# AI-Application-and-Integration-Lab/RDPN6D

Hardware: AMD Instinct MI355X
Metric: RGB-D crops/sec (fwd+PnP) at 256x256 (higher is better)
Workload: dtype f32

## Files before the change

include/rdpn6d.h:

```cpp
#ifndef RDPN6D_H
#define RDPN6D_H

#ifdef __cplusplus
extern "C" {
#endif

#define RDPN6D_OK 0
#define RDPN6D_EINVAL -1
#define RDPN6D_EHIP -2
#define RDPN6D_ENOMEM -3

const char* rdpn6d_last_error(void);
int rdpn6d_version(void);
int rdpn6d_device_count(void);

void farthest_point_sampling(float* pts, int* idxs, int pn, int sn);
void farthest_point_sampling_init_center(float* pts, int* idxs, int pn, int sn);
int rdpn6d_fps_host(const float* pts, int* idxs, int pn, int sn, int start);
int rdpn6d_fps_device(const float* d_pts, const int* d_offsets, int nobj, int max_pn, int sn, int start,
                      int* d_idxs, float* d_mindist, void* stream);
long long rdpn6d_fps_workspace_bytes(int nobj);
int rdpn6d_fps_device_ws(const float* d_pts, const int* d_offsets, int nobj, int max_pn, int sn, int start, int* d_idxs,
                         float* d_mindist, void* workspace, long long workspace_bytes, void* stream);

typedef struct {
    const float* x;
    const float* w;
    const float* scale;
    const float* shift;
    const float* res;
    float* y;
    int B, H, W;
    int Cin;
    int in_cs, in_co;
    int Ho, Wo;
    int stride;
    int ntaps;
    int dy[9], dx[9];
    int N, Npad;
    int OH, OW;
    int osy, osx, ooy, oox;
    int out_cs, out_co;
    int res_cs, res_co;
    int act;
    float slope;
} rdpn6d_conv_desc;
int rdpn6d_conv2d_f32(const rdpn6d_conv_desc* d, void* stream);
long long rdpn6d_conv_splitk_ws_floats(const rdpn6d_conv_desc* d, int ksplit);
int rdpn6d_conv2d_splitk_f32(const rdpn6d_conv_desc* d, int ksplit, float* workspace, void* stream);
int rdpn6d_conv_tile_for(const rdpn6d_conv_desc* d, int* bm, int* bn);
void rdpn6d_conv_force_tile(int bm, int bn);
void rdpn6d_conv_set_tap_inner(int v);

int rdpn6d_conv2d_bf16(const rdpn6d_conv_desc* d, int out_f32, void* stream);
int rdpn6d_conv2d_splitk_bf16(const rdpn6d_conv_desc* d, int out_f32, int ksplit, float* workspace, void* stream);
int rdpn6d_conv2d_bf16_bnstats(const rdpn6d_conv_desc* d, double* stats, int stats_row0, int* stats_rows, void* stream);
int rdpn6d_conv2d_bf16_bnbwd(const rdpn6d_conv_desc* d, const void* bn_x, int bn_cs, int bn_co, const float* mean, const float* invstd,
                             const float* gamma, const float* beta, double* partial, int* rows, void* stream);
int rdpn6d_bn_relu_backward_apply_bf16(const void* x, int xcs, int xco, const void* dy, int dcs, int dco, const float* mean,
                                       const float* invstd, const float* gamma, const float* beta, float* dgamma, float* dbeta, void* dx,
                                       int xgcs, int xgco, long long M, int C, const double* partial, int S, void* stream);
int rdpn6d_conv2d_bf16_bnbwd_y(const rdpn6d_conv_desc* d, const void* bn_x, int bn_cs, int bn_co, const void* bn_y, int y_cs, int y_co,
                               const float* mean, const float* invstd, double* partial, int* rows, void* stream);
int rdpn6d_bn_backward_apply_bf16(const void* x, int xcs, int xco, const void* dy, int dcs, int dco, const void* y, int ycs, int yco,
                                  const float* mean, const float* invstd, const float* gamma, float* dgamma, float* dbeta, void* dx,
                                  int xgcs, int xgco, void* dres, int rcs, int rco, long long M, int C, const double* partial, int S,
                                  void* stream);
void rdpn6d_conv_bf16_force_tile(int bm, int bn);
void rdpn6d_conv_bf16_force_stages(int nst);
int rdpn6d_conv_bf16_tile_for(const rdpn6d_conv_desc* d, int* bm, int* bn);
int rdpn6d_conv_bf16_uses_pingpong(const rdpn6d_conv_desc* d, int out_f32);
int rdpn6d_split_bf16x3(const float* x, long long n, void* planes, long long plane_elems, void* stream);
int rdpn6d_conv_bf16x3_eligible(const rdpn6d_conv_desc* d);
int rdpn6d_conv_bf16x3_kernel_for(const rdpn6d_conv_desc* d);
int rdpn6d_conv2d_bf16x3(const rdpn6d_conv_desc* d, long long x_plane_elems, long long w_plane_elems, void* y_planes,
                         long long y_plane_elems, void* stream);
int rdpn6d_conv2d_bf16x3_ex(const rdpn6d_conv_desc* d, long long x_plane_elems, long long w_plane_elems, void* y_planes,
                            long long y_plane_elems, const void* res_planes, long long res_plane_elems, void* stream);
int rdpn6d_split_h2(const float* x, int src_cs, int src_co, int C, void* dst, long long npix, int* overflow_flag, void* stream);
int rdpn6d_conv_h2_kernel_for(const rdpn6d_conv_desc* d);
int rdpn6d_conv2d_h2(const rdpn6d_conv_desc* d, void* y_h2, const void* res_h2, int* overflow_flag, void* stream);
int rdpn6d_conv2d_h2_cb(const rdpn6d_conv_desc* d, void* y_h2, const void* res_h2, int* overflow_flag, const float* crop_bias,
                        void* stream);
long long rdpn6d_conv_h2_workspace_bytes(const rdpn6d_conv_desc* d);
void rdpn6d_conv_h2_set_clock_probe(unsigned long long* buf);
void rdpn6d_conv_h2_set_wfrag(int mode);
int rdpn6d_conv_h2_colmax_ok(const rdpn6d_conv_desc* d, int rows_per_group);
int rdpn6d_conv2d_h2_colmax(const rdpn6d_conv_desc* d, unsigned long long* keys, int rows_per_group, int* overflow_flag, void* stream);
int rdpn6d_h2_colmax_decode(unsigned long long* keys, int groups, int N, int Npad, void* out_h2, void* stream);
int rdpn6d_conv_h2_wfrag_wanted(const rdpn6d_conv_desc* d);
int rdpn6d_h2_weight_frag(const void* w_h2, int Npad, int ntaps, int cchunks, void* w_frag, void* stream);
int rdpn6d_conv2d_h2_wf(const rdpn6d_conv_desc* d, void* y_h2, const void* res_h2, int* overflow_flag, const void* w_frag, void* stream);
int rdpn6d_conv2d_h2_ws(const rdpn6d_conv_desc* d, void* y_h2, const void* res_h2, int* overflow_flag, const float* crop_bias,
                        void* workspace, long long workspace_bytes, void* stream);
int rdpn6d_conv_h2_fuse1x1_ok(const rdpn6d_conv_desc* d);
int rdpn6d_conv2d_h2_fuse1x1(const rdpn6d_conv_desc* d, const void* res_h2, int* overflow_flag, const float* crop_bias,
                             const void* w1_h2, const float* scale1, const float* bias1, float* out, int out_cs, int n_out,
                             void* stream);
int rdpn6d_upsample_bilinear_h2(const void* x, int B, int H, int W, int C, int factor, void* y, int* overflow_flag, void* stream);
int rdpn6d_upsample_bilinear_h2_ex(const void* x, int B, int H, int W, int C, int factor, void* y, int out_cs, int out_co, int relu,
                                   int* overflow_flag, void* stream);
int rdpn6d_xyz_subsample_h2(const float* x, int B, int xc, int R, int step, void* y, int out_cs, int out_co, int* overflow_flag,
                            void* stream);
int rdpn6d_global_max_concat_h2(void* buf, int B, int HW, int C, int cs, void* stream);
int rdpn6d_global_max_h2(const void* x_h2, int B, int HW, int C, int cs, void* gmax_h2, void* stream);
int rdpn6d_convt3x3s2_const_bias_f32(const float* V, const float* scale, int B, int F, float* out , void* stream);
int rdpn6d_stem_pool_h2(const float* x, int B, int xc, int R, const void* w_h2, const float* scale, const float* shift, void* y,
                        int* overflow_flag, void* stream);
int rdpn6d_stem_pool_h2_ex(const float* x, int B, int xc, int R, const void* w_h2, const float* scale, const float* shift, void* y,
                           int out_fmt, int* overflow_flag, void* stream);
int rdpn6d_stem_pack_h2(const float* w_oihw, void* w_h2, float* inv_scale, void* stream);
void rdpn6d_conv_bf16_force_chunk(int row_bytes);
int rdpn6d_stem_conv7x7_bf16(const float* x, int B, int xc, int R, const float* w, const float* scale,
                             const float* shift, void* y, void* stream);
int rdpn6d_maxpool3x3s2_bf16(const void* x, int B, int H, int W, int C, void* y, void* stream);
int rdpn6d_upsample_bilinear_bf16(const void* x, int B, int H, int W, int C, int factor, void* y, void* stream);
int rdpn6d_xyz_subsample_bf16(const float* x, int B, int xc, int R, int step, void* y, int out_cs, int out_co,
                              void* stream);
int rdpn6d_global_max_concat_bf16(void* buf, int B, int HW, int C, int cs, void* stream);
int rdpn6d_cast_f32_bf16(const float* src, int src_cs, int src_co, int C, void* dst, int dst_cs, long long npix,
                         void* stream);

int rdpn6d_stem_conv7x7_f32(const float* x, int B, int xc, int R, const float* w, const float* scale,
                            const float* shift, float* y, void* stream);
int rdpn6d_maxpool3x3s2_f32(const float* x, int B, int H, int W, int C, float* y, void* stream);
int rdpn6d_upsample_bilinear_f32(const float* x, int B, int H, int W, int C, int factor, float* y, void* stream);
int rdpn6d_xyz_subsample_f32(const float* x, int B, int xc, int R, int step, float* y, int out_cs, int out_co,
                             void* stream);
int rdpn6d_global_max_concat_f32(float* buf, int B, int HW, int C, int cs, void* stream);
int rdpn6d_groupnorm_relu_f32(float* x, int B, int HW, int C, int G, const float* gamma, const float* beta,
                              void* stream);
int rdpn6d_groupnorm_relu_h2(const float* x, int B, int HW, int C, int G, const float* gamma, const float* beta, void* y_h2,
                             int* overflow_flag, void* stream);

int rdpn6d_dense_glue_f32(const float* head, int head_cs, const float* coord2d, const float* fps, int B, int HW,
                          int K, int mask_attention, float* minmax_scratch, float* out_nchw, float* pnp_in,
                          int pnp_cs, int* argmax_out, void* stream);
int rdpn6d_dense_glue_h2(const float* head, int head_cs, const float* coord2d, const float* fps, int B, int HW, int K,
                         int mask_attention, float* minmax_scratch, float* out_nchw, void* pnp_in_h2, int pnp_cs,
                         int* argmax_out, int* overflow_flag, void* stream);
int rdpn6d_dense_glue_mt_f32(const float* head, int head_cs, const float* coord2d, const float* fps, int B, int HW, int K,
                             int mask_attention, int mask_type, float* minmax_scratch, float* out_nchw, float* pnp_in, int pnp_cs,
                             int* argmax_out, void* stream);
int rdpn6d_dense_glue_mt_h2(const float* head, int head_cs, const float* coord2d, const float* fps, int B, int HW, int K,
                            int mask_attention, int mask_type, float* minmax_scratch, float* out_nchw, void* pnp_in_h2, int pnp_cs,
                            int* argmax_out, int* overflow_flag, void* stream);

int rdpn6d_pose_decode_f32(const float* rt, int rt_stride, const float* roi_cams, const float* roi_centers,
                           const float* roi_whs, const float* resize_ratios, int B, int is_allo, int train_variant,
                           float* rot, float* trans, void* stream);

int rdpn6d_ransac_kabsch_f32(const float* out_nchw, const float* coord2d, const float* fps, const float* extents,
                             const float* resize_ratios, const int* region_argmax, int B, int HW, int K,
                             float mask_thr, float inlier_thr, int iters, float confidence, unsigned seed,
                             float* pose_out, int* n_inliers, unsigned char* inlier_mask, void* stream);
int rdpn6d_ransac_kabsch_ex(const float* out_nchw, const float* coord2d, const float* fps, const float* extents,
                            const float* resize_ratios, const int* region_argmax, int B, int HW, int K,
                            float mask_thr, float inlier_thr, int iters, float confidence, unsigned seed,
                            float* pose_out, int* n_inliers, unsigned char* inlier_mask, int* best_hyp, void* stream);
int rdpn6d_ransac_kabsch_net_f32(const float* out_nchw, const float* coord2d, const float* fps, const float* extents,
                                 const float* resize_ratios, const int* region_argmax, const float* net_pose, int B,
                                 int HW, int K, float mask_thr, float inlier_thr, int iters, float confidence,
                                 unsigned seed, int mode, float max_t_diff, float* pose_out, int* n_inliers,
                                 unsigned char* inlier_mask, int* best_hyp, void* stream);
long long rdpn6d_ransac_workspace_bytes(int B);
int rdpn6d_ransac_kabsch_ws(const float* out_nchw, const float* coord2d, const float* fps, const float* extents,
                            const float* resize_ratios, const int* region_argmax, const float* net_pose, int B, int HW, int K,
                            float mask_thr, float inlier_thr, int iters, float confidence, unsigned seed, int mode,
                            float max_t_diff, float* pose_out, int* n_inliers, unsigned char* inlier_mask, int* best_hyp,
                            void* workspace, long long workspace_bytes, void* stream);
int rdpn6d_ransac_kabsch_ws_mt(const float* out_nchw, const float* coord2d, const float* fps, const float* extents,
                               const float* resize_ratios, const int* region_argmax, const float* net_pose, int B, int HW, int K,
                               float mask_thr, int mask_type, float inlier_thr, int iters, float confidence, unsigned seed, int mode,
                               float max_t_diff, float* pose_out, int* n_inliers, unsigned char* inlier_mask, int* best_hyp,
                               void* workspace, long long workspace_bytes, void* stream);



int rdpn6d_stem_conv7x7_raw_f32(const float* x, int B, int xc, int R, const float* w, float* y, void* stream);
int rdpn6d_bn_train_stats_f32(const float* x, long long M, int C, int cs, int co, float eps, float momentum, float* mean,
                              float* invstd, float* running_mean, float* running_var, double* scratch, void* stream);
int rdpn6d_bn_stats_finalize(const double* partial, int S, int C, long long M, float eps, float momentum, float* mean, float* invstd,
                             float* running_mean, float* running_var, void* stream);
int rdpn6d_bn_apply_f32(const float* x, int xcs, int xco, const float* mean, const float* invstd, const float* gamma,
                        const float* beta, const float* res, int rcs, int rco, float* y, int ycs, int yco, long long M, int C,
                        int relu, void* stream);
int rdpn6d_bn_backward_f32(const float* x, int xcs, int xco, const float* dy, int dcs, int dco, const float* y, int ycs,
                           int yco, const float* mean, const float* invstd, const float* gamma, float* dgamma, float* dbeta,
                           float* dx, int xgcs, int xgco, float* dres, int rcs, int rco, long long M, int C, int relu,
                           double* scratch, void* stream);
int rdpn6d_bn_relu_backward_f32(const float* x, int xcs, int xco, const float* dy, int dcs, int dco, const float* mean,
                                const float* invstd, const float* gamma, const float* beta, float* dgamma, float* dbeta, float* dx,
                                int xgcs, int xgco, long long M, int C, double* scratch, void* stream);
int rdpn6d_channel_sum_f32(const float* x, long long M, int C, int cs, int co, float* out, int accumulate, double* scratch,
                           void* stream);
int rdpn6d_groupnorm_relu_train_f32(const float* x, float* y, int B, int HW, int C, int G, const float* gamma,
                                    const float* beta, float* stats, void* stream);
int rdpn6d_groupnorm_relu_backward_f32(const float* x, const float* y, const float* dy, const float* gamma, const float* stats,
                                       float* dx, float* dgamma, float* dbeta, float* dgb_scratch, double* scratch, int B,
                                       int HW, int C, int G, void* stream);
long long rdpn6d_wgrad_scratch_floats(int Bn, int Ha, int Wa, int Ca, int Cb, int ntaps);
int rdpn6d_wgrad_f32(const float* A, int a_cs, int a_co, int Ca, const float* Bg, int b_cs, int b_co, int Cb, int Bn, int Ha,
                     int Wa, int Hb, int Wb, int stride, int ntaps, const int* dy, const int* dx, float* out, float* partial,
                     void* stream);
int rdpn6d_wgrad_bf16(const void* A, int a_cs, int a_co, int Ca, int Ca_ld, const void* Bg, int b_cs, int b_co, int Cb,
                      int Cb_ld, int Bn, int Ha, int Wa, int Hb, int Wb, int stride, int ntaps, const int* dy, const int* dx,
                      float* out, float* partial, void* stream);
int rdpn6d_wgrad_f32_strided(const float* A, int a_cs, int a_co, int Ca, const float* Bg, int b_cs, int b_co, int Cb, int Bn,
                             int Ha, int Wa, int Hb, int Wb, int stride, int ntaps, const int* dy, const int* dx, float* out,
                             long long sa, long long st, long long sb, int Ca_out, int Cb_out, float* partial, void* stream);
int rdpn6d_wgrad_bf16_strided(const void* A, int a_cs, int a_co, int Ca, int Ca_ld, const void* Bg, int b_cs, int b_co, int Cb,
                              int Cb_ld, int Bn, int Ha, int Wa, int Hb, int Wb, int stride, int ntaps, const int* dy,
                              const int* dx, float* out, long long sa, long long st, long long sb, int Ca_out, int Cb_out,
                              float* partial, void* stream);
long long rdpn6d_wgrad_group_scratch_floats(int G, int Bn, int Ha, int Wa, int Ca, int Cb, int ntaps);
int rdpn6d_wgrad_bf16_group(int G, const void* const* A_list, int a_cs, int a_co, int Ca, int Ca_ld, const void* const* B_list, int b_cs,
                            int b_co, int Cb, int Cb_ld, int Bn, int Ha, int Wa, int Hb, int Wb, int stride, int ntaps, const int* dy,
                            const int* dx, float* const* out_list, long long sa, long long st, long long sb, int Ca_out, int Cb_out,
                            float* partial, long long partial_floats, void* stream);
int rdpn6d_wgrad_bf16x3_strided(const void* A, long long a_plane_elems, int a_cs, int a_co, int Ca, int Ca_ld, const void* Bg,
                                long long b_plane_elems, int b_cs, int b_co, int Cb, int Cb_ld, int Bn, int Ha, int Wa, int Hb,
                                int Wb, int stride, int ntaps, const int* dy, const int* dx, float* out, long long sa,
                                long long st, long long sb, int Ca_out, int Cb_out, float* partial, void* stream);
int rdpn6d_maxpool3x3s2_backward_f32(const float* x, const float* dy, int B, int H, int W, int C, float* dx, void* stream);
int rdpn6d_upsample_bilinear_backward_f32(const float* dy, int B, int H, int W, int C, int factor, float* dx, void* stream);
int rdpn6d_global_max_concat_backward_f32(const float* feat, const float* dfeat, int B, int HW, int C, int cs, float* dl3,
                                          void* stream);
int rdpn6d_dense_losses_f32(const float* head, int head_cs, const float* gt_xyz, const float* mask_visib,
                            const float* mask_trunc, const long long* gt_region, int B, int HW, int K, float xyz_lw,
                            float mask_lw, float region_lw, float* dhead, float* losses, double* scratch, void* stream);
int rdpn6d_dense_glue_backward_f32(const float* head, int head_cs, const float* coord2d, const float* fps, const int* argmax,
                                   const float* dpnp, int pnp_cs, int B, int HW, int K, int mask_attention,
                                   const float* minmax, float* dhead, float* datt_scratch, void* stream);
int rdpn6d_dense_losses_mt_f32(const float* head, int head_cs, const float* gt_xyz, const float* mask_visib, const float* mask_trunc,
                               const long long* gt_region, int B, int HW, int K, float xyz_lw, float mask_lw, float region_lw,
                               int mask_type, float* dhead, float* losses, double* scratch, void* stream);
int rdpn6d_dense_glue_backward_mt_f32(const float* head, int head_cs, const float* coord2d, const float* fps, const int* argmax,
                                      const float* dpnp, int pnp_cs, int B, int HW, int K, int mask_attention, int mask_type,
                                      const float* minmax, float* dhead, float* datt_scratch, void* stream);
int rdpn6d_pose_train_f32(const float* rt, int rt_stride, const float* roi_cams, const float* roi_centers,
                          const float* roi_whs, const float* resize_ratios, const float* roi_extents, const float* gt_rot,
                          const float* gt_trans_ratio, const float* points, int npts, int B, int is_allo, float pm_lw,
                          int pm_norm_by_extent, float centroid_lw, float z_lw, float* rot, float* trans, float* d_rt,
// ... 156 lines not shown
```

rdpn6d_amd/_lib.py:

```python
import ctypes
import os

HERE = os.path.dirname(os.path.abspath(__file__))
LIB_PATH = os.environ.get("RDPN6D_LIB") or os.path.join(HERE, "librdpn6d_hip.so")

_ll = ctypes.c_longlong
c_float_p = ctypes.c_void_p
c_int_p = ctypes.c_void_p
_vp, _i, _f, _u = ctypes.c_void_p, ctypes.c_int, ctypes.c_float, ctypes.c_uint


class ConvDesc(ctypes.Structure):

    _fields_ = [
        ("x", _vp), ("w", _vp), ("scale", _vp), ("shift", _vp), ("res", _vp), ("y", _vp),
        ("B", _i), ("H", _i), ("W", _i), ("Cin", _i), ("in_cs", _i), ("in_co", _i), ("Ho", _i), ("Wo", _i),
        ("stride", _i), ("ntaps", _i), ("dy", _i * 9), ("dx", _i * 9), ("N", _i), ("Npad", _i), ("OH", _i), ("OW", _i),
        ("osy", _i), ("osx", _i), ("ooy", _i), ("oox", _i), ("out_cs", _i), ("out_co", _i), ("res_cs", _i),
        ("res_co", _i), ("act", _i), ("slope", _f),
    ]


SIGNATURES = {
    "rdpn6d_last_error": (ctypes.c_char_p, []),
    "rdpn6d_version": (_i, []),
    "rdpn6d_device_count": (_i, []),
    "farthest_point_sampling": (None, [_vp, _vp, _i, _i]),
    "farthest_point_sampling_init_center": (None, [_vp, _vp, _i, _i]),
    "rdpn6d_fps_host": (_i, [_vp, _vp, _i, _i, _i]),
    "rdpn6d_fps_device": (_i, [_vp, _vp, _i, _i, _i, _i, _vp, _vp, _vp]),
    "rdpn6d_fps_workspace_bytes": (_ll, [_i]),
    "rdpn6d_fps_device_ws": (_i, [_vp, _vp, _i, _i, _i, _i, _vp, _vp, _vp, _ll, _vp]),
    "rdpn6d_conv2d_f32": (_i, [ctypes.POINTER(ConvDesc), _vp]),
    "rdpn6d_conv_tile_for": (_i, [ctypes.POINTER(ConvDesc), _vp, _vp]),
    "rdpn6d_conv_force_tile": (None, [_i, _i]),
    "rdpn6d_conv_set_tap_inner": (None, [_i]),
    "rdpn6d_conv_splitk_ws_floats": (ctypes.c_longlong, [ctypes.POINTER(ConvDesc), _i]),
    "rdpn6d_conv2d_splitk_f32": (_i, [ctypes.POINTER(ConvDesc), _i, _vp, _vp]),
    "rdpn6d_conv2d_bf16": (_i, [ctypes.POINTER(ConvDesc), _i, _vp]),
    "rdpn6d_conv2d_splitk_bf16": (_i, [ctypes.POINTER(ConvDesc), _i, _i, _vp, _vp]),
    "rdpn6d_conv_bf16_force_tile": (None, [_i, _i]),
    "rdpn6d_conv_bf16_uses_pingpong": (_i, [ctypes.POINTER(ConvDesc), _i]),
    "rdpn6d_conv2d_bf16_bnstats": (_i, [ctypes.POINTER(ConvDesc), _vp, _i, _vp, _vp]),
    "rdpn6d_conv2d_bf16_bnbwd": (_i, [ctypes.POINTER(ConvDesc), _vp, _i, _i, _vp, _vp, _vp, _vp, _vp, _vp, _vp]),
    "rdpn6d_bn_relu_backward_apply_bf16": (_i, [_vp, _i, _i, _vp, _i, _i, _vp, _vp, _vp, _vp, _vp, _vp, _vp, _i, _i, _ll, _i, _vp, _i, _vp]),
    "rdpn6d_conv2d_bf16_bnbwd_y": (_i, [ctypes.POINTER(ConvDesc), _vp, _i, _i, _vp, _i, _i, _vp, _vp, _vp, _vp, _vp]),
    "rdpn6d_bn_backward_apply_bf16": (_i, [_vp, _i, _i, _vp, _i, _i, _vp, _i, _i, _vp, _vp, _vp, _vp, _vp, _vp, _i, _i, _vp, _i, _i, _ll, _i,
                                           _vp, _i, _vp]),
    "rdpn6d_bn_stats_finalize": (_i, [_vp, _i, _i, _ll, _f, _f, _vp, _vp, _vp, _vp, _vp]),
    "rdpn6d_conv_bf16_tile_for": (_i, [ctypes.POINTER(ConvDesc), _vp, _vp]),
    "rdpn6d_split_bf16x3": (_i, [_vp, _ll, _vp, _ll, _vp]),
    "rdpn6d_conv_bf16x3_eligible": (_i, [ctypes.POINTER(ConvDesc)]),
    "rdpn6d_conv2d_bf16x3": (_i, [ctypes.POINTER(ConvDesc), _ll, _ll, _vp, _ll, _vp]),
    "rdpn6d_conv_bf16x3_kernel_for": (_i, [ctypes.POINTER(ConvDesc)]),
    "rdpn6d_conv2d_bf16x3_ex": (_i, [ctypes.POINTER(ConvDesc), _ll, _ll, _vp, _ll, _vp, _ll, _vp]),
    "rdpn6d_conv_bf16_force_chunk": (None, [_i]),
    "rdpn6d_conv_bf16_force_stages": (None, [_i]),
    "rdpn6d_stem_conv7x7_bf16": (_i, [_vp, _i, _i, _i, _vp, _vp, _vp, _vp, _vp]),
    "rdpn6d_maxpool3x3s2_bf16": (_i, [_vp, _i, _i, _i, _i, _vp, _vp]),
    "rdpn6d_upsample_bilinear_bf16": (_i, [_vp, _i, _i, _i, _i, _i, _vp, _vp]),
    "rdpn6d_xyz_subsample_bf16": (_i, [_vp, _i, _i, _i, _i, _vp, _i, _i, _vp]),
    "rdpn6d_global_max_concat_bf16": (_i, [_vp, _i, _i, _i, _i, _vp]),
    "rdpn6d_cast_f32_bf16": (_i, [_vp, _i, _i, _i, _vp, _i, ctypes.c_longlong, _vp]),
    "rdpn6d_stem_conv7x7_f32": (_i, [_vp, _i, _i, _i, _vp, _vp, _vp, _vp, _vp]),
    "rdpn6d_maxpool3x3s2_f32": (_i, [_vp, _i, _i, _i, _i, _vp, _vp]),
    "rdpn6d_upsample_bilinear_f32": (_i, [_vp, _i, _i, _i, _i, _i, _vp, _vp]),
    "rdpn6d_xyz_subsample_f32": (_i, [_vp, _i, _i, _i, _i, _vp, _i, _i, _vp]),
    "rdpn6d_global_max_concat_f32": (_i, [_vp, _i, _i, _i, _i, _vp]),
    "rdpn6d_groupnorm_relu_f32": (_i, [_vp, _i, _i, _i, _i, _vp, _vp, _vp]),
    "rdpn6d_groupnorm_relu_h2": (_i, [_vp, _i, _i, _i, _i, _vp, _vp, _vp, _vp, _vp]),
    "rdpn6d_dense_glue_f32": (_i, [_vp, _i, _vp, _vp, _i, _i, _i, _i, _vp, _vp, _vp, _i, _vp, _vp]),
    "rdpn6d_dense_glue_h2": (_i, [_vp, _i, _vp, _vp, _i, _i, _i, _i, _vp, _vp, _vp, _i, _vp, _vp, _vp]),
    "rdpn6d_dense_glue_mt_f32": (_i, [_vp, _i, _vp, _vp, _i, _i, _i, _i, _i, _vp, _vp, _vp, _i, _vp, _vp]),
    "rdpn6d_dense_glue_mt_h2": (_i, [_vp, _i, _vp, _vp, _i, _i, _i, _i, _i, _vp, _vp, _vp, _i, _vp, _vp, _vp]),
    "rdpn6d_pose_decode_f32": (_i, [_vp, _i, _vp, _vp, _vp, _vp, _i, _i, _i, _vp, _vp, _vp]),
    "rdpn6d_ransac_kabsch_f32": (_i, [_vp, _vp, _vp, _vp, _vp, _vp, _i, _i, _i, _f, _f, _i, _f, _u, _vp, _vp, _vp, _vp]),
    "rdpn6d_ransac_kabsch_ex": (_i, [_vp, _vp, _vp, _vp, _vp, _vp, _i, _i, _i, _f, _f, _i, _f, _u, _vp, _vp, _vp, _vp, _vp]),
    "rdpn6d_ransac_kabsch_net_f32": (_i, [_vp, _vp, _vp, _vp, _vp, _vp, _vp, _i, _i, _i, _f, _f, _i, _f, _u, _i, _f, _vp, _vp, _vp,
                                          _vp, _vp]),
    "rdpn6d_ransac_workspace_bytes": (ctypes.c_longlong, [_i]),
    "rdpn6d_ransac_kabsch_ws": (_i, [_vp, _vp, _vp, _vp, _vp, _vp, _vp, _i, _i, _i, _f, _f, _i, _f, _u, _i, _f, _vp, _vp, _vp, _vp, _vp, _ll, _vp]),
    "rdpn6d_ransac_kabsch_ws_mt": (_i, [_vp, _vp, _vp, _vp, _vp, _vp, _vp, _i, _i, _i, _f, _i, _f, _i, _f, _u, _i, _f, _vp, _vp, _vp, _vp, _vp, _ll, _vp]),
    "rdpn6d_stem_conv7x7_raw_f32": (_i, [_vp, _i, _i, _i, _vp, _vp, _vp]),
    "rdpn6d_bn_train_stats_f32": (_i, [_vp, _ll, _i, _i, _i, _f, _f, _vp, _vp, _vp, _vp, _vp, _vp]),
    "rdpn6d_bn_apply_f32": (_i, [_vp, _i, _i, _vp, _vp, _vp, _vp, _vp, _i, _i, _vp, _i, _i, _ll, _i, _i, _vp]),
    "rdpn6d_bn_backward_f32": (_i, [_vp, _i, _i, _vp, _i, _i, _vp, _i, _i, _vp, _vp, _vp, _vp, _vp, _vp, _i, _i, _vp, _i, _i,
                                    _ll, _i, _i, _vp, _vp]),
    "rdpn6d_bn_relu_backward_f32": (_i, [_vp, _i, _i, _vp, _i, _i, _vp, _vp, _vp, _vp, _vp, _vp, _vp, _i, _i, _ll, _i, _vp, _vp]),
    "rdpn6d_channel_sum_f32": (_i, [_vp, _ll, _i, _i, _i, _vp, _i, _vp, _vp]),
    "rdpn6d_groupnorm_relu_train_f32": (_i, [_vp, _vp, _i, _i, _i, _i, _vp, _vp, _vp, _vp]),
    "rdpn6d_groupnorm_relu_backward_f32": (_i, [_vp, _vp, _vp, _vp, _vp, _vp, _vp, _vp, _vp, _vp, _i, _i, _i, _i, _vp]),
    "rdpn6d_wgrad_scratch_floats": (_ll, [_i, _i, _i, _i, _i, _i]),
    "rdpn6d_wgrad_f32": (_i, [_vp, _i, _i, _i, _vp, _i, _i, _i, _i, _i, _i, _i, _i, _i, _i, _vp, _vp, _vp, _vp, _vp]),
    "rdpn6d_wgrad_bf16": (_i, [_vp, _i, _i, _i, _i, _vp, _i, _i, _i, _i, _i, _i, _i, _i, _i, _i, _i, _vp, _vp, _vp, _vp, _vp]),
    "rdpn6d_wgrad_f32_strided": (_i, [_vp, _i, _i, _i, _vp, _i, _i, _i, _i, _i, _i, _i, _i, _i, _i, _vp, _vp, _vp, _ll, _ll, _ll, _i, _i,
                                      _vp, _vp]),
    "rdpn6d_wgrad_bf16_strided": (_i, [_vp, _i, _i, _i, _i, _vp, _i, _i, _i, _i, _i, _i, _i, _i, _i, _i, _i, _vp, _vp, _vp, _ll, _ll, _ll,
                                       _i, _i, _vp, _vp]),
    "rdpn6d_wgrad_group_scratch_floats": (_ll, [_i, _i, _i, _i, _i, _i, _i]),
    "rdpn6d_wgrad_bf16_group": (_i, [_i, _vp, _i, _i, _i, _i, _vp, _i, _i, _i, _i, _i, _i, _i, _i, _i, _i, _i, _vp, _vp, _vp, _ll, _ll, _ll,
                                     _i, _i, _vp, _ll, _vp]),
    "rdpn6d_wgrad_bf16x3_strided": (_i, [_vp, _ll, _i, _i, _i, _i, _vp, _ll, _i, _i, _i, _i, _i, _i, _i, _i, _i, _i, _i, _vp, _vp, _vp,
                                         _ll, _ll, _ll, _i, _i, _vp, _vp]),
    "rdpn6d_maxpool3x3s2_backward_f32": (_i, [_vp, _vp, _i, _i, _i, _i, _vp, _vp]),
    "rdpn6d_upsample_bilinear_backward_f32": (_i, [_vp, _i, _i, _i, _i, _i, _vp, _vp]),
    "rdpn6d_global_max_concat_backward_f32": (_i, [_vp, _vp, _i, _i, _i, _i, _vp, _vp]),
    "rdpn6d_dense_losses_f32": (_i, [_vp, _i, _vp, _vp, _vp, _vp, _i, _i, _i, _f, _f, _f, _vp, _vp, _vp, _vp]),
    "rdpn6d_dense_glue_backward_f32": (_i, [_vp, _i, _vp, _vp, _vp, _vp, _i, _i, _i, _i, _i, _vp, _vp, _vp, _vp]),
    "rdpn6d_dense_losses_mt_f32": (_i, [_vp, _i, _vp, _vp, _vp, _vp, _i, _i, _i, _f, _f, _f, _i, _vp, _vp, _vp, _vp]),
    "rdpn6d_dense_glue_backward_mt_f32": (_i, [_vp, _i, _vp, _vp, _vp, _vp, _i, _i, _i, _i, _i, _i, _vp, _vp, _vp, _vp]),
    "rdpn6d_pose_train_f32": (_i, [_vp, _i, _vp, _vp, _vp, _vp, _vp, _vp, _vp, _vp, _i, _i, _i, _f, _i, _f, _f, _vp, _vp, _vp,
                                   _vp, _vp, _vp]),
    "rdpn6d_pose_train_sym_f32": (_i, [_vp, _i, _vp, _vp, _vp, _vp, _vp, _vp, _vp, _vp, _i, _i, _i, _f, _i, _f, _f, _vp, _vp, _i,
                                       _vp, _vp, _vp, _vp, _vp, _vp, _vp]),
    "rdpn6d_ranger_step_f32": (_i, [_vp, _vp, _vp, _vp, _vp, _vp, _i, _vp, _vp, _i, _vp, _f, _f, _f, _f, _f, _i, _i, _f, _vp]),
    "rdpn6d_ranger_step_scaled_f32": (_i, [_vp, _vp, _vp, _vp, _vp, _vp, _i, _vp, _vp, _i, _vp, _f, _f, _f, _f, _f, _i, _i, _f, _f, _vp, _vp]),
    "rdpn6d_grad_nonfinite_f32": (_i, [_vp, _ll, _vp, _vp]),
    "rdpn6d_region_targets_f32": (_i, [_vp, _vp, _vp, _vp, _i, _i, _i, _vp, _vp, _vp]),
    "rdpn6d_pose_errors_f64": (_i, [_vp, _vp, _vp, _i, _i, _i, _vp, _vp, _vp]),
    "rdpn6d_crop_builder_f32": (_i, [_vp, _vp, _i, _i, _i, _vp, _vp, _vp, _vp, _vp, _i, _i, _vp, _vp, _vp]),
    "rdpn6d_act_backward_f32": (_i, [_vp, _vp, _ll, _f, _vp]),
    "rdpn6d_transpose_rc_f32": (_i, [_vp, _i, _i, _i, _vp, _vp]),
    "rdpn6d_train_vis_scalars_f32": (_i, [_vp, _vp, _vp, _vp, _vp, _i, _vp, _i, _vp, _vp]),
    "rdpn6d_rgb_to_nhwc4_f32": (_i, [_vp, _i, _i, _i, _vp, _vp]),
    "rdpn6d_stem_im2col_f32": (_i, [_vp, _i, _i, _i, _vp, _vp]),
    "rdpn6d_stem_rowpatch_f32": (_i, [_vp, _i, _i, _i, _vp, _vp]),
    "rdpn6d_stem_conv7x7_raw_bf16": (_i, [_vp, _i, _i, _i, _vp, _vp, _vp]),
    "rdpn6d_bn_train_stats_bf16": (_i, [_vp, _ll, _i, _i, _i, _f, _f, _vp, _vp, _vp, _vp, _vp, _vp]),
    "rdpn6d_bn_apply_bf16": (_i, [_vp, _i, _i, _vp, _vp, _vp, _vp, _vp, _i, _i, _vp, _i, _i, _ll, _i, _i, _vp]),
    "rdpn6d_bn_backward_bf16": (_i, [_vp, _i, _i, _vp, _i, _i, _vp, _i, _i, _vp, _vp, _vp, _vp, _vp, _vp, _i, _i, _vp, _i, _i,
                                     _ll, _i, _i, _vp, _vp]),
    "rdpn6d_bn_relu_backward_bf16": (_i, [_vp, _i, _i, _vp, _i, _i, _vp, _vp, _vp, _vp, _vp, _vp, _vp, _i, _i, _ll, _i, _vp, _vp]),
    "rdpn6d_channel_sum_bf16": (_i, [_vp, _ll, _i, _i, _i, _vp, _i, _vp, _vp]),
    "rdpn6d_maxpool3x3s2_backward_bf16": (_i, [_vp, _vp, _i, _i, _i, _i, _vp, _vp]),
    "rdpn6d_upsample_bilinear_backward_bf16": (_i, [_vp, _i, _i, _i, _i, _i, _vp, _vp]),
    "rdpn6d_global_max_concat_backward_bf16": (_i, [_vp, _vp, _i, _i, _i, _i, _vp, _vp]),
    "rdpn6d_stem_im2col_bf16": (_i, [_vp, _i, _i, _i, _vp, _vp]),
    "rdpn6d_stem_rowpatch_bf16": (_i, [_vp, _i, _i, _i, _vp, _vp]),
    "rdpn6d_repack_f32": (_i, [_vp, _vp, _vp, _i, _vp]),
    "rdpn6d_split_h2": (_i, [_vp, _i, _i, _i, _vp, _ll, _vp, _vp]),
    "rdpn6d_conv_h2_kernel_for": (_i, [_vp]),
    "rdpn6d_conv2d_h2": (_i, [_vp, _vp, _vp, _vp, _vp]),
    "rdpn6d_upsample_bilinear_h2": (_i, [_vp, _i, _i, _i, _i, _i, _vp, _vp, _vp]),
    "rdpn6d_xyz_subsample_h2": (_i, [_vp, _i, _i, _i, _i, _vp, _i, _i, _vp, _vp]),
    "rdpn6d_stem_pool_h2": (_i, [_vp, _i, _i, _i, _vp, _vp, _vp, _vp, _vp, _vp]),
    "rdpn6d_stem_pool_h2_ex": (_i, [_vp, _i, _i, _i, _vp, _vp, _vp, _vp, _i, _vp, _vp]),
    "rdpn6d_stem_pack_h2": (_i, [_vp, _vp, _vp, _vp]),
    "rdpn6d_global_max_concat_h2": (_i, [_vp, _i, _i, _i, _i, _vp]),
    "rdpn6d_upsample_bilinear_h2_ex": (_i, [_vp, _i, _i, _i, _i, _i, _vp, _i, _i, _i, _vp, _vp]),
    "rdpn6d_global_max_h2": (_i, [_vp, _i, _i, _i, _i, _vp, _vp]),
    "rdpn6d_convt3x3s2_const_bias_f32": (_i, [_vp, _vp, _i, _i, _vp, _vp]),
    "rdpn6d_conv2d_h2_cb": (_i, [_vp, _vp, _vp, _vp, _vp, _vp]),
    "rdpn6d_conv2d_h2_ws": (_i, [_vp, _vp, _vp, _vp, _vp, _vp, ctypes.c_longlong, _vp]),
    "rdpn6d_conv_h2_fuse1x1_ok": (_i, [ctypes.POINTER(ConvDesc)]),
    "rdpn6d_conv2d_h2_fuse1x1": (_i, [ctypes.POINTER(ConvDesc), _vp, _vp, _vp, _vp, _vp, _vp, _vp, _i, _i, _vp]),
    "rdpn6d_conv_h2_workspace_bytes": (ctypes.c_longlong, [_vp]),
    "rdpn6d_conv_h2_colmax_ok": (_i, [ctypes.POINTER(ConvDesc), _i]),
    "rdpn6d_conv2d_h2_colmax": (_i, [ctypes.POINTER(ConvDesc), _vp, _i, _vp, _vp]),
    "rdpn6d_h2_colmax_decode": (_i, [_vp, _i, _i, _i, _vp, _vp]),
    "rdpn6d_conv_h2_set_wfrag": (None, [_i]),
    "rdpn6d_conv_h2_set_clock_probe": (None, [_vp]),
    "rdpn6d_conv_h2_wfrag_wanted": (_i, [ctypes.POINTER(ConvDesc)]),
    "rdpn6d_h2_weight_frag": (_i, [_vp, _i, _i, _i, _vp, _vp]),
    "rdpn6d_conv2d_h2_wf": (_i, [ctypes.POINTER(ConvDesc), _vp, _vp, _vp, _vp, _vp]),
    "rdpn6d_ransac_pnp_f32": (_i, [_vp, _vp, _vp, _vp, _vp, _i, _i, _f, _i, _f, ctypes.c_uint, _i, _f, _vp, _vp, _vp, _vp, _vp]),
    "rdpn6d_ransac_pnp_ex": (_i, [_vp, _vp, _vp, _vp, _vp, _i, _i, _f, _i, _f, ctypes.c_uint, _i, _f, _i, _vp, _vp, _vp, _vp, _vp]),
    "rdpn6d_ransac_pnp_workspace_bytes": (_ll, [_i]),
    "rdpn6d_ransac_pnp_ws": (_i, [_vp, _vp, _vp, _vp, _vp, _i, _i, _f, _i, _f, ctypes.c_uint, _i, _f, _i, _vp, _vp, _vp, _vp, _vp, _ll, _vp]),
    "rdpn6d_select_correspondences_f32": (_i, [_vp, _i, _vp, _i, _i, _i, _vp, _vp, _i, _i, _i, _i, _f, _vp, _vp, _vp, _vp, _vp, _vp]),
    "rdpn6d_select_correspondences_mt_f32": (_i, [_vp, _i, _vp, _i, _i, _i, _vp, _vp, _i, _i, _i, _i, _f, _i, _vp, _vp, _vp, _vp, _vp, _vp]),
}

for _k in [k for k in list(SIGNATURES) if "_bf16" in k and "bf16x3" not in k]:
    SIGNATURES[_k.replace("_bf16", "_fp16")] = SIGNATURES[_k]
SIGNATURES["rdpn6d_repack_fp16"] = SIGNATURES["rdpn6d_repack_f32"]

_lib = None


def load():
    global _lib
    if _lib is None:
        if not os.path.exists(LIB_PATH):
            raise RuntimeError(
                f"{LIB_PATH} is missing: build the HIP extension first (python -m rdpn6d_amd.build). "
                "rdpn6d_amd has no CPU fallback."
            )
        import torch

        if torch.cuda.device_count() > 0:
            torch.cuda.init()
        lib = ctypes.CDLL(LIB_PATH)
        for name, (res, args) in SIGNATURES.items():
            fn = getattr(lib, name)
            fn.restype = res
            fn.argtypes = args
        _lib = lib
    return _lib


def check(rc, what=""):
    if rc != 0:
        msg = load().rdpn6d_last_error()
        raise RuntimeError(f"rdpn6d HIP call failed ({what}, rc={rc}): {msg.decode() if msg else '?'}")
```

rdpn6d_amd/csrc/conv_igemm_h2.hip:

```cpp
#include "conv_h2_common.h"

#include <cstdio>
#include <cstdlib>

#ifdef RDPN6D_PROBE
__device__ unsigned long long* g_h2_probe = nullptr;
extern "C" int rdpn6d_debug_h2_probe(void* buf)
{
    RD_CHECK_HIP(hipMemcpyToSymbol(HIP_SYMBOL(g_h2_probe), &buf, sizeof(buf)));
    return RDPN6D_OK;
}
#endif

namespace {

constexpr int HT_BYTES = 16384;
constexpr int LDS_8PH = 2 * 4 * HT_BYTES;
constexpr int LDS_8PH_FUSED = 8 * (32 * 72 * 4 + 32 * 272);
static_assert(LDS_8PH_FUSED >= LDS_8PH && LDS_8PH_FUSED <= 160 * 1024, "LDS");

template <bool FUSE, bool CMAX>
__device__ __forceinline__ void conv_h2_8ph_body(const ConvH2Args& ax)
{
    extern __shared__ __attribute__((aligned(1024))) unsigned char smem[];
// ... 292 lines not shown
            f32x16 oacc[2];
#pragma unroll
            for (int jn = 0; jn < 2; ++jn)
#pragma unroll
                for (int e = 0; e < 16; ++e) oacc[jn][e] = 0.f;
            {
                H2_PAIRS;
#pragma unroll
                for (int cch = 0; cch < 2; ++cch) {
                    u32x4 af[4];
#pragma unroll
                    for (int j = 0; j < 4; ++j) af[j] = *reinterpret_cast<const u32x4*>(ast + frow * AST + cch * 128 + ((2 * j + half) << 4));
#pragma unroll
                    for (int pr = 0; pr < 6; ++pr)
#pragma unroll
                        for (int jn = 0; jn < 2; ++jn) oacc[jn] = h2_mfma(af[H2_PA[pr]], fw[jn][cch][H2_PB[pr]], oacc[jn]);
                }
            }
#pragma unroll
            for (int jn = 0; jn < 2; ++jn)
#pragma unroll
                for (int e = 0; e < 16; ++e) cst[((e & 3) + 8 * (e >> 2) + 4 * hi) * CS + jn * 32 + frow] = oacc[jn][e];
            asm volatile("s_waitcnt lgkmcnt(0)" ::: "memory");
            __builtin_amdgcn_s_barrier();
            asm volatile("" ::: "memory");
            {
                const int row = lane >> 1, n8 = wc * 16 + (lane & 1) * 8;
                float r[8] = {0.f, 0.f, 0.f, 0.f, 0.f, 0.f, 0.f, 0.f};
#pragma unroll
                for (int w4 = 0; w4 < 4; ++w4) {
                    const float* ps = reinterpret_cast<const float*>(smem + (wr * 4 + w4) * SLICE) + row * CS + n8;
                    const f32x4 p0 = *reinterpret_cast<const f32x4*>(ps), p1 = *reinterpret_cast<const f32x4*>(ps + 4);
#pragma unroll
                    for (int q = 0; q < 4; ++q) {
                        r[q] += p0[q];
                        r[4 + q] += p1[q];
                    }
                }
                const long long mrow = m0 + wr * 128 + i * 32 + row;
                if (mrow < a.M && n8 < ax.fuse_cs) {
                    float* op = ax.fuse_out + h2_pixel_of(a, mrow) * ax.fuse_cs + n8;
                    f32x4 o0, o1;
#pragma unroll
                    for (int q = 0; q < 4; ++q) {
                        o0[q] = r[q] * ax.fuse_scale[n8 + q] + ax.fuse_bias[n8 + q];
                        o1[q] = r[4 + q] * ax.fuse_scale[n8 + 4 + q] + ax.fuse_bias[n8 + 4 + q];
                    }
                    *reinterpret_cast<f32x4*>(op) = o0;
                    *reinterpret_cast<f32x4*>(op + 4) = o1;
                }
            }
            asm volatile("s_waitcnt lgkmcnt(0)" ::: "memory");
            __builtin_amdgcn_s_barrier();
            asm volatile("" ::: "memory");
        }
        return;
    }
    if constexpr (CMAX) {
        unsigned long long* keys = reinterpret_cast<unsigned long long*>(ax.fuse_out);
        const int hi = lane >> 5;
        const long long rbase = m0 + wr * 128 + 4 * hi;
        const bool full = m0 + 256 <= a.M;
        unsigned mbits = 0;
#pragma unroll
        for (int j = 0; j < 2; ++j) {
            float vmax = -__builtin_huge_valf();
#pragma unroll
            for (int i = 0; i < 4; ++i)
#pragma unroll
                for (int e = 0; e < 16; ++e) {
                    const float v = acc[i][j][e] * scj[j] + shj[j];
                    const bool valid = full || rbase + i * 32 + (e & 3) + 8 * (e >> 2) < a.M;
                    const unsigned ub = __float_as_uint(v) & 0x7fffffffu;
                    mbits = (valid && ub > mbits) ? ub : mbits;
                    vmax = valid ? __builtin_fmaxf(vmax, v) : vmax;
                }
            const float vo = __shfl_xor(vmax, 32, 64);
            vmax = __builtin_fmaxf(vmax, vo);
            const int n = nb + j * 32 + frow;
            if (hi == 0 && n < d.N && vmax > -__builtin_huge_valf()) {
                _Float16 hq, lq;
                h2_split(vmax * H2_SCALE, hq, lq);
                const float r = (float)hq + (float)lq;
                const unsigned u = __float_as_uint(r);
                const unsigned ord = (u & 0x80000000u) ? ~u : (u | 0x80000000u);
                const unsigned pay = ((unsigned)__builtin_bit_cast(unsigned short, hq) << 16) | (unsigned)__builtin_bit_cast(unsigned short, lq);
                atomicMax(keys + (m0 / ax.fuse_cs) * d.Npad + n, ((unsigned long long)ord << 32) | pay);
            }
        }
        if (mbits > 0x457fe000u && ax.overflow_flag) *ax.overflow_flag = 1;
        return;
    }
    {
        const int hi = lane >> 5;
        constexpr int CS = 64 + 8;
        __builtin_amdgcn_s_barrier();
        asm volatile("" ::: "memory");
        float* cst = reinterpret_cast<float*>(smem) + wave * (32 * CS);
        const int rrow = lane >> 3, c8 = (lane & 7) * 8;
#pragma unroll
        for (int i = 0; i < 4; ++i) {
#pragma unroll
            for (int j = 0; j < 2; ++j)
#pragma unroll
                for (int e = 0; e < 16; ++e)
                    cst[((e & 3) + 8 * (e >> 2) + 4 * hi) * CS + j * 32 + frow] = acc[i][j][e] * scj[j] + shj[j];
#pragma unroll
            for (int rr = 0; rr < 4; ++rr) {
                const int row = rr * 8 + rrow;
                const long long mrow = m0 + wr * 128 + i * 32 + row;
                if (mrow >= a.M) continue;
                const f32x4 lo = *reinterpret_cast<const f32x4*>(cst + row * CS + c8);
                const f32x4 hi4 = *reinterpret_cast<const f32x4*>(cst + row * CS + c8 + 4);
                float v[8] = {lo[0], lo[1], lo[2], lo[3], hi4[0], hi4[1], hi4[2], hi4[3]};
                h2_finish_row8(ax, v, h2_pixel_of(a, mrow), nb + c8);
            }
        }
    }
#ifdef RDPN6D_PROBE
    {
        const unsigned long long t_issued = __builtin_readcyclecounter();
        asm volatile("s_waitcnt vmcnt(0)" ::: "memory");
        const unsigned long long t_done = __builtin_readcyclecounter();
        if (g_h2_probe && lane == 0) {
            unsigned long long* o = g_h2_probe + ((size_t)blockIdx.x * 8 + wave) * 8;
            o[0] = pq_loop0 - pq_start;
            o[1] = pq_loop1 - pq_loop0;
            o[2] = t_issued - pq_loop1;
            o[3] = t_done - t_issued;
            o[4] = pq_rt0;
            o[5] = __builtin_amdgcn_s_memrealtime();
            o[6] = (unsigned long long)nk;
        }
    }
#endif
}

template <bool FUSE>
__global__ __launch_bounds__(512) void conv_h2_8ph_kernel_t(const ConvH2Args ax)
{
    const bool probe = ax.clk_probe != nullptr && blockIdx.x == 0 && blockIdx.y == 0;
    unsigned long long t0 = 0, r0 = 0;
    if (probe) { t0 = __builtin_readcyclecounter(); r0 = __builtin_amdgcn_s_memrealtime(); }
    conv_h2_8ph_body<FUSE, false>(ax);
    if (probe && threadIdx.x == 0) {
        ax.clk_probe[0] = t0; ax.clk_probe[1] = r0;
        ax.clk_probe[2] = __builtin_readcyclecounter(); ax.clk_probe[3] = __builtin_amdgcn_s_memrealtime();
    }
}
__global__ __launch_bounds__(512) void conv_h2_8ph_colmax_kernel(const ConvH2Args ax) { conv_h2_8ph_body<false, true>(ax); }

constexpr auto conv_h2_8ph_kernel = conv_h2_8ph_kernel_t<false>;

template <int BM, int BN, int NST, int SCHED = 0>
__global__ __launch_bounds__(256, 2) void conv_h2_tile_kernel(const ConvH2Args ax)
{
    constexpr int NW = 4, RB = 128;
    constexpr int RPP = 1024 / RB;
    constexpr int WGN = 2, WTM = BM / 2, WTN = BN / 2;
    constexpr int TM = WTM / 32, TN = WTN / 32;
    constexpr int AG = BM / RPP / NW, BG = BN / RPP / NW;
    constexpr int NDMA = AG + BG;
    static_assert(TM >= 1 && TN >= 1 && AG >= 1 && BG >= 1, "tile / wave layout");
    extern __shared__ __attribute__((aligned(1024))) unsigned char smem[];
    unsigned char* As = smem;
    unsigned char* Bs = smem + NST * BM * RB;

    const ConvBArgs& a = ax.b;
    const rdpn6d_conv_desc& d = a.d;
    const int nblk = a.mtiles * a.ntiles;
    const int bid = blockIdx.x;
    const int q8 = nblk >> 3, r8 = nblk & 7, xcd = bid & 7, kk = bid >> 3;
    const int logical = (xcd < r8 ? xcd * (q8 + 1) : r8 * (q8 + 1) + (xcd - r8) * q8) + kk;
    const int nt = logical % a.ntiles;
    const int mt = logical / a.ntiles;
    const long long m0 = (long long)mt * BM;
    const int n0 = nt * BN;

    const int tid = threadIdx.x;
    const int lane = tid & 63;
    const int wave = __builtin_amdgcn_readfirstlane(tid >> 6);

    const int prow = lane >> 3, pslot = lane & 7;
    const unsigned px_bytes = (unsigned)d.in_cs * 4u;
    unsigned a_base[AG], a_mask[AG];
#pragma unroll
    for (int i = 0; i < AG; ++i) {
        const int row = (wave + NW * i) * RPP + prow;
        const long long m = m0 + row;
        const bool ok = m < a.M;
        const int mm = ok ? (int)m : 0;
        const int b = mm / a.HoWo;
        const int rem = mm - b * a.HoWo;
        const int oy = rem / d.Wo;
        const int ox = rem - oy * d.Wo;
        const int iy = oy * d.stride, ix = ox * d.stride;
        const int lslot = pslot ^ ((row >> 1) & 7);
        a_base[i] = (unsigned)((b * d.H + iy) * d.W + ix) * px_bytes + (unsigned)d.in_co * 4u + (unsigned)lslot * 16u;
        unsigned mask = 0;
        for (int t = 0; t < d.ntaps; ++t) {
            const int dy = (int)((a.dy_pack >> (4 * t)) & 15ull) - 8, dx = (int)((a.dx_pack >> (4 * t)) & 15ull) - 8;
            mask |= (ok && (unsigned)(iy + dy) < (unsigned)d.H && (unsigned)(ix + dx) < (unsigned)d.W) ? (1u << t) : 0u;
        }
        a_mask[i] = mask;
    }
    unsigned w_off[BG];
#pragma unroll
    for (int i = 0; i < BG; ++i) {
        const int row = (wave + NW * i) * RPP + prow;
        const int lslot = pslot ^ ((row >> 1) & 7);
        w_off[i] = (unsigned)(n0 + row) * (unsigned)a.Ktot * 4u + (unsigned)lslot * 16u;
    }
    const __amdgpu_buffer_rsrc_t xsrc = __builtin_amdgcn_make_buffer_rsrc(const_cast<float*>(d.x), 0, a.x_bytes, 0x00020000);
    const __amdgpu_buffer_rsrc_t wsrc = __builtin_amdgcn_make_buffer_rsrc(const_cast<float*>(d.w), 0, a.w_bytes, 0x00020000);

    auto stage_chunk = [&](const int tap, const int cc, const int st) {
        const int dy = (int)((a.dy_pack >> (4 * tap)) & 15ull) - 8, dx = (int)((a.dx_pack >> (4 * tap)) & 15ull) - 8;
        const unsigned toff = (unsigned)((dy * d.W + dx) * (int)px_bytes + cc * RB);
#pragma unroll
        for (int i = 0; i < AG; ++i) {
            const unsigned kill = ((a_mask[i] >> tap) & 1u) - 1u;
            unsigned char* dst = As + ((st * BM) + (wave + NW * i) * RPP) * RB;
            __builtin_amdgcn_raw_ptr_buffer_load_lds(xsrc, (lds_ptr_t)dst, 16, (int)((a_base[i] + toff) | kill), 0, 0, 0);
        }
        const unsigned wk = (unsigned)tap * (unsigned)d.Cin * 4u + (unsigned)cc * (unsigned)RB;
#pragma unroll
        for (int i = 0; i < BG; ++i) {
            unsigned char* dst = Bs + ((st * BN) + (wave + NW * i) * RPP) * RB;
            __builtin_amdgcn_raw_ptr_buffer_load_lds(wsrc, (lds_ptr_t)dst, 16, (int)(w_off[i] + wk), 0, 0, 0);
        }
    };
    const int nk = a.kper;
    const int kt0 = (int)blockIdx.y * a.kper;
    int ld_cc = kt0 / d.ntaps, ld_tap = kt0 - (kt0 / d.ntaps) * d.ntaps, ld_left = nk - 1;
    auto next_chunk = [](int& tap, int& cc, int& left, const int ntaps) {
        const int go = left > 0 ? 1 : 0;
        left -= go;
        tap += go;
        const int wrap = tap == ntaps ? 1 : 0;
        tap = wrap ? 0 : tap;
        cc += wrap;
    };

    const int wm = wave / WGN, wn = wave % WGN;
    const int frow = lane & 31;
    const int half = lane >> 5;

    auto read_frags = [&](int st, u32x4 (&fa)[TM][4], u32x4 (&fb)[TN][4]) {
#pragma unroll
        for (int i = 0; i < TM; ++i) {
            const int R = wm * WTM + i * 32 + frow;
            const int sw = (R >> 1) & 7;
            const unsigned char* q = As + ((st * BM) + R) * RB;
#pragma unroll
            for (int j = 0; j < 4; ++j) fa[i][j] = *reinterpret_cast<const u32x4*>(q + (((2 * j + half) ^ sw) << 4));
        }
#pragma unroll
        for (int jn = 0; jn < TN; ++jn) {
            const int R = wn * WTN + jn * 32 + frow;
            const int sw = (R >> 1) & 7;
            const unsigned char* q = Bs + ((st * BN) + R) * RB;
#pragma unroll
            for (int j = 0; j < 4; ++j) fb[jn][j] = *reinterpret_cast<const u32x4*>(q + (((2 * j + half) ^ sw) << 4));
        }
    };

    constexpr int WC = WTN, CS = WC + 8, LPR = WC / 8, RPI = 64 / LPR, NRR = 32 / RPI;
    const int nb = n0 + wn * WC;
    const int rrow = lane / LPR, c8 = (lane % LPR) * 8;
    f16x8 rh[TM][NRR], rl[TM][NRR];
    long long pixs[TM][NRR];
    const bool res_pre = ax.res_h2 != nullptr && d.res == nullptr && ax.partial == nullptr;
#pragma unroll
    for (int i = 0; i < TM; ++i)
#pragma unroll
        for (int rr = 0; rr < NRR; ++rr) {
            const long long mrow = m0 + wm * WTM + i * 32 + rr * RPI + rrow;
            const bool ok = mrow < a.M && nb + c8 < d.N;
            pixs[i][rr] = ok ? h2_pixel_of(a, mrow) : -1;
            if (res_pre && ok) {
                const int c = d.res_co + nb + c8;
                const _Float16* rp = reinterpret_cast<const _Float16*>(ax.res_h2) + pixs[i][rr] * (2 * d.res_cs) + (c >> 5) * 64 + (c & 31);
                rh[i][rr] = *reinterpret_cast<const f16x8*>(rp);
                rl[i][rr] = *reinterpret_cast<const f16x8*>(rp + 32);
            } else {
                rh[i][rr] = f16x8{};
                rl[i][rr] = f16x8{};
            }
        }
    float scj[TN], shj[TN];
#pragma unroll
    for (int j = 0; j < TN; ++j) {
        const int n = nb + j * 32 + frow;
        scj[j] = (d.scale && !ax.partial) ? d.scale[n] : 1.f;
        shj[j] = (d.shift && !ax.partial) ? d.shift[n] : 0.f;
    }

    f32x16 acc[TM][TN];
#pragma unroll
    for (int i = 0; i < TM; ++i)
#pragma unroll
        for (int j = 0; j < TN; ++j)
#pragma unroll
            for (int e = 0; e < 16; ++e) acc[i][j][e] = 0.f;

    auto mma = [&](const u32x4 (&fa)[TM][4], const u32x4 (&fb)[TN][4]) {
        H2_PAIRS;
#pragma unroll
        for (int pr = 0; pr < 6; ++pr)
#pragma unroll
            for (int i = 0; i < TM; ++i)
#pragma unroll
                for (int jn = 0; jn < TN; ++jn) acc[i][jn] = h2_mfma(fa[i][H2_PA[pr]], fb[jn][H2_PB[pr]], acc[i][jn]);
    };

    u32x4 fa0[TM][4], fb0[TN][4], fa1[TM][4], fb1[TN][4];
    [[maybe_unused]] unsigned long long pr_sum[5] = {0, 0, 0, 0, 0};
    [[maybe_unused]] const unsigned long long pr_start = SCHED == 9 ? __builtin_readcyclecounter() : 0ull;
    [[maybe_unused]] const unsigned long long pr_rt0 = SCHED == 9 ? (__builtin_amdgcn_s_memrealtime() & 0xffffffffull) : 0ull;
    if constexpr (NST == 2) {
        stage_chunk(ld_tap, ld_cc, 0);
        next_chunk(ld_tap, ld_cc, ld_left, d.ntaps);
        stage_chunk(ld_tap, ld_cc, 1);
        next_chunk(ld_tap, ld_cc, ld_left, d.ntaps);
        __syncthreads();
        read_frags(0, fa0, fb0);
        __syncthreads();
        const int npairs = nk >> 1;
        for (int pr = 0; pr < npairs; ++pr) {
            stage_chunk(ld_tap, ld_cc, 0);
            next_chunk(ld_tap, ld_cc, ld_left, d.ntaps);
            read_frags(1, fa1, fb1);
            mma(fa0, fb0);
            __syncthreads();

            stage_chunk(ld_tap, ld_cc, 1);
            next_chunk(ld_tap, ld_cc, ld_left, d.ntaps);
            read_frags(0, fa0, fb0);
            mma(fa1, fb1);
            __syncthreads();
        }
        if (nk & 1) mma(fa0, fb0);
    } else {
        auto publish = [&]() {
            asm volatile("s_waitcnt vmcnt(%0) lgkmcnt(0)" ::"n"(NDMA) : "memory");
            __builtin_amdgcn_s_barrier();
            asm volatile("" ::: "memory");
        };
        stage_chunk(ld_tap, ld_cc, 0);
        next_chunk(ld_tap, ld_cc, ld_left, d.ntaps);
        stage_chunk(ld_tap, ld_cc, 1);
        next_chunk(ld_tap, ld_cc, ld_left, d.ntaps);
        stage_chunk(ld_tap, ld_cc, 2);
        next_chunk(ld_tap, ld_cc, ld_left, d.ntaps);
        asm volatile("s_waitcnt vmcnt(%0)" ::"n"(2 * NDMA) : "memory");
        __builtin_amdgcn_s_barrier();
        asm volatile("" ::: "memory");
        read_frags(0, fa0, fb0);
        publish();
        int st_free = 0, st_next = 1;
        const int npairs = nk >> 1;
        auto step = [&](const int stf, const int stn, u32x4 (&fcur_a)[TM][4], u32x4 (&fcur_b)[TN][4], u32x4 (&fnxt_a)[TM][4], u32x4 (&fnxt_b)[TN][4]) {
            if constexpr (SCHED == 0) {
                stage_chunk(ld_tap, ld_cc, stf);
                next_chunk(ld_tap, ld_cc, ld_left, d.ntaps);
                read_frags(stn, fnxt_a, fnxt_b);
                mma(fcur_a, fcur_b);
                publish();
            } else if constexpr (SCHED == 9) {
#ifdef RDPN6D_PROBE
                const unsigned long long t0 = __builtin_readcyclecounter();
                __builtin_amdgcn_sched_barrier(0);
                read_frags(stn, fnxt_a, fnxt_b);
                __builtin_amdgcn_sched_barrier(0);
                const unsigned long long t1 = __builtin_readcyclecounter();
                __builtin_amdgcn_sched_barrier(0);
                stage_chunk(ld_tap, ld_cc, stf);
                next_chunk(ld_tap, ld_cc, ld_left, d.ntaps);
                __builtin_amdgcn_sched_barrier(0);
                const unsigned long long t2 = __builtin_readcyclecounter();
                __builtin_amdgcn_sched_barrier(0);
                mma(fcur_a, fcur_b);
                __builtin_amdgcn_sched_barrier(0);
                const unsigned long long t3 = __builtin_readcyclecounter();
                __builtin_amdgcn_sched_barrier(0);
                asm volatile("s_waitcnt vmcnt(%0) lgkmcnt(0)" ::"n"(NDMA) : "memory");
                const unsigned long long t4 = __builtin_readcyclecounter();
                __builtin_amdgcn_sched_barrier(0);
                __builtin_amdgcn_s_barrier();
                asm volatile("" ::: "memory");
                const unsigned long long t5 = __builtin_readcyclecounter();
                pr_sum[0] += t1 - t0;
                pr_sum[1] += t2 - t1;
                pr_sum[2] += t3 - t2;
                pr_sum[3] += t4 - t3;
                pr_sum[4] += t5 - t4;
#endif
            }
        };
        for (int pr = 0; pr < npairs; ++pr) {
            step(st_free, st_next, fa0, fb0, fa1, fb1);
            st_free = st_next;
            st_next = st_next == 2 ? 0 : st_next + 1;
            step(st_free, st_next, fa1, fb1, fa0, fb0);
            st_free = st_next;
            st_next = st_next == 2 ? 0 : st_next + 1;
        }
        if (nk & 1) mma(fa0, fb0);
        asm volatile("s_waitcnt vmcnt(0)" ::: "memory");
    }
#ifdef RDPN6D_PROBE
    [[maybe_unused]] const unsigned long long pr_loop_end = SCHED == 9 ? __builtin_readcyclecounter() : 0ull;
#endif

    {
        const int hi = lane >> 5;
        asm volatile("s_waitcnt vmcnt(0) lgkmcnt(0)" ::: "memory");
        __builtin_amdgcn_s_barrier();
        asm volatile("" ::: "memory");
        float* cst = reinterpret_cast<float*>(smem) + wave * (32 * CS);
        if (ax.partial) {
            float* part = ax.partial + ((size_t)blockIdx.y * ax.mpad + (size_t)m0 + wm * WTM) * d.Npad + nb + c8;
#pragma unroll
            for (int i = 0; i < TM; ++i) {
#pragma unroll
                for (int j = 0; j < TN; ++j)
#pragma unroll
                    for (int e = 0; e < 16; ++e) cst[((e & 3) + 8 * (e >> 2) + 4 * hi) * CS + j * 32 + frow] = acc[i][j][e];
#pragma unroll
                for (int rr = 0; rr < 32 / RPI; ++rr) {
                    const int row = rr * RPI + rrow;
                    float* pp = part + (size_t)(i * 32 + row) * d.Npad;
                    *reinterpret_cast<f32x4*>(pp) = *reinterpret_cast<const f32x4*>(cst + row * CS + c8);
                    *reinterpret_cast<f32x4*>(pp + 4) = *reinterpret_cast<const f32x4*>(cst + row * CS + c8 + 4);
                }
            }
            return;
        }
#pragma unroll
        for (int i = 0; i < TM; ++i) {
#pragma unroll
            for (int j = 0; j < TN; ++j)
#pragma unroll
                for (int e = 0; e < 16; ++e)
                    cst[((e & 3) + 8 * (e >> 2) + 4 * hi) * CS + j * 32 + frow] = acc[i][j][e] * scj[j] + shj[j];
#pragma unroll
            for (int rr = 0; rr < NRR; ++rr) {
                const int row = rr * RPI + rrow;
                if (pixs[i][rr] >= 0) {
                    const f32x4 lo = *reinterpret_cast<const f32x4*>(cst + row * CS + c8);
                    const f32x4 hi4 = *reinterpret_cast<const f32x4*>(cst + row * CS + c8 + 4);
                    float v[8] = {lo[0], lo[1], lo[2], lo[3], hi4[0], hi4[1], hi4[2], hi4[3]};
                    if (res_pre) h2_finish_row8_t<true>(ax, v, pixs[i][rr], nb + c8, rh[i][rr], rl[i][rr]);
                    else h2_finish_row8_t<false>(ax, v, pixs[i][rr], nb + c8, rh[i][rr], rl[i][rr]);
                }
            }
        }
    }
#ifdef RDPN6D_PROBE
    if constexpr (SCHED == 9) {
        if (g_h2_probe && lane == 0) {
            const unsigned long long t_end = __builtin_readcyclecounter();
            unsigned long long* o = g_h2_probe + ((size_t)blockIdx.x * 4 + wave) * 8;
            for (int i = 0; i < 5; ++i) o[i] = pr_sum[i];
            o[5] = pr_loop_end - pr_start;
            o[6] = t_end - pr_loop_end;
            o[7] = pr_rt0 | (__builtin_amdgcn_s_memrealtime() << 32);
        }
    }
#endif
}

__global__ __launch_bounds__(256) void h2_splitk_reduce_kernel(const ConvH2Args ax)
{
    const ConvBArgs& a = ax.b;
    const rdpn6d_conv_desc& d = a.d;
    const int n8 = d.Npad >> 3;
    const long long total = a.M * n8;
    const size_t sstride = (size_t)ax.mpad * d.Npad;
    for (long long i = (long long)blockIdx.x * 256 + threadIdx.x; i < total; i += (long long)gridDim.x * 256) {
        const long long m = i / n8;
        const int ch = (int)(i - m * n8) * 8;
        if (ch >= d.N) continue;
        const float* pp = ax.partial + (size_t)m * d.Npad + ch;
        f32x4 s0 = *reinterpret_cast<const f32x4*>(pp), s1 = *reinterpret_cast<const f32x4*>(pp + 4);
        int sl = 1;
        for (; sl + 3 <= ax.nsplit; sl += 3) {
            const float* q = pp + sl * sstride;
            const f32x4 t0 = *reinterpret_cast<const f32x4*>(q), t1 = *reinterpret_cast<const f32x4*>(q + 4);
            const f32x4 u0 = *reinterpret_cast<const f32x4*>(q + sstride), u1 = *reinterpret_cast<const f32x4*>(q + sstride + 4);
            const f32x4 w0 = *reinterpret_cast<const f32x4*>(q + 2 * sstride), w1 = *reinterpret_cast<const f32x4*>(q + 2 * sstride + 4);
            s0 = ((s0 + t0) + u0) + w0;
            s1 = ((s1 + t1) + u1) + w1;
        }
        for (; sl < ax.nsplit; ++sl) {
            const float* q = pp + sl * sstride;
            s0 += *reinterpret_cast<const f32x4*>(q);
            s1 += *reinterpret_cast<const f32x4*>(q + 4);
        }
        float v[8];
#pragma unroll
        for (int q = 0; q < 4; ++q) {
            v[q] = s0[q] * (d.scale ? d.scale[ch + q] : 1.f) + (d.shift ? d.shift[ch + q] : 0.f);
            v[4 + q] = s1[q] * (d.scale ? d.scale[ch + 4 + q] : 1.f) + (d.shift ? d.shift[ch + 4 + q] : 0.f);
        }
        h2_finish_row8(ax, v, h2_pixel_of(a, m), ch);
    }
}

template <int BM, int BN, int NST, int SCHED = 0>
int launch_h2_tile_s(const ConvH2Args& ax, hipStream_t s);
template <int BM, int BN, int NST>
int launch_h2_tile(const ConvH2Args& ax, hipStream_t s)
{
#ifdef RDPN6D_PROBE
    static const int sched = getenv("RDPN6D_H2_SCHED") ? atoi(getenv("RDPN6D_H2_SCHED")) : 0;
    if (sched == 9) return launch_h2_tile_s<BM, BN, NST, 9>(ax, s);
#endif
    return launch_h2_tile_s<BM, BN, NST, 0>(ax, s);
}
template <int BM, int BN, int NST, int SCHED>
int launch_h2_tile_s(const ConvH2Args& ax, hipStream_t s)
{
    constexpr int lds_stage = NST * (BM + BN) * 128;
    constexpr int lds_epi = 4 * 32 * (BN / 2 + 8) * 4;
    constexpr int lds = lds_stage > lds_epi ? lds_stage : lds_epi;
    static_assert(lds <= 80 * 1024 || (BM == 128 && BN == 128 && NST == 3), "two workgroups per CU (128x128 with three stages: one)");
    auto kern = conv_h2_tile_kernel<BM, BN, NST, SCHED>;
    if (lds > 64 * 1024) {
        RD_LDS_OPT_IN(kern, lds);
    }
    hipLaunchKernelGGL(kern, dim3((unsigned)(ax.b.mtiles * ax.b.ntiles), (unsigned)ax.nsplit), dim3(256), lds, s, ax);
    return RDPN6D_OK;
}

__global__ void split_h2_kernel(const float* __restrict__ x, int src_cs, int src_co, int C, _Float16* __restrict__ dst, long long npix,
                                int* __restrict__ overflow_flag)
{
    const int c8n = C >> 3;
    const long long total = npix * c8n;
    bool over = false;
    for (long long i = (long long)blockIdx.x * blockDim.x + threadIdx.x; i < total; i += (long long)gridDim.x * blockDim.x) {
        const long long p = i / c8n;
        const int c = (int)(i - p * c8n) * 8;
        const float* sp = x + p * src_cs + src_co + c;
        const f32x4 v0 = *reinterpret_cast<const f32x4*>(sp), v1 = *reinterpret_cast<const f32x4*>(sp + 4);
        const float v[8] = {v0[0], v0[1], v0[2], v0[3], v1[0], v1[1], v1[2], v1[3]};
        f16x8 hi, lo;
        float sv[8];
#pragma unroll
        for (int q = 0; q < 8; ++q) sv[q] = v[q] * H2_SCALE;
        over |= h2_split8(sv, hi, lo);
        _Float16* pp = dst + p * (2 * (long long)C) + (c >> 5) * 64 + (c & 31);
        *reinterpret_cast<f16x8*>(pp) = hi;
        *reinterpret_cast<f16x8*>(pp + 32) = lo;
    }
    if (over && overflow_flag) *overflow_flag = 1;
}

bool h2_common_ok(const rdpn6d_conv_desc* d)
{
    return d->Cin % 32 == 0 && d->in_cs % 32 == 0 && d->in_co % 32 == 0 && d->out_cs % 8 == 0 && d->out_co % 8 == 0 && d->N % 8 == 0 &&
           d->Npad % 64 == 0 && (!d->res || (d->res_cs % 4 == 0 && d->res_co % 4 == 0));
}
bool h2_big_ok(const rdpn6d_conv_desc* d)
{
    const int nk = d->ntaps * (d->Cin / 32);
    return h2_common_ok(d) && d->Npad % 256 == 0 && d->N == d->Npad && nk >= 2 && (nk & 1) == 0;
}
bool h2_big_pays(const rdpn6d_conv_desc* d, long long M)
{
    const long long tiles = (long long)rd_cdiv(M, 256) * (d->Npad / 256);
    const long long rounds = (tiles + 255) / 256;
    return tiles >= 160 && (double)tiles >= 0.62 * 256.0 * (double)rounds;
}
void h2_pick_tile(const rdpn6d_conv_desc* d, long long M, int* pbm, int* pbn)
{
    int bn = (d->Npad % 128 == 0) ? 128 : 64;
    int bm = 128;
    if ((long long)rd_cdiv(M, 128) * (d->Npad / bn) < 512) bm = 64;
    if (bm == 64 && bn == 128 && (long long)rd_cdiv(M, 64) * (d->Npad / 128) < 512) bn = 64;
    if (const char* f = getenv("RDPN6D_H2_TILE")) {
        int fbm = 0, fbn = 0;
        if (sscanf(f, "%d,%d", &fbm, &fbn) == 2 && (fbm == 64 || fbm == 128) && (fbn == 64 || fbn == 128) && d->Npad % fbn == 0) {
            bm = fbm;
            bn = fbn;
        }
    }
    *pbm = bm;
    *pbn = bn;
}

}

extern "C" int rdpn6d_split_h2(const float* x, int src_cs, int src_co, int C, void* dst, long long npix, int* overflow_flag, void* stream)
{
    RD_REQUIRE(x && dst && npix > 0 && C > 0 && C % 32 == 0 && src_cs % 4 == 0 && src_co % 4 == 0 && src_co + C <= src_cs, "h2 split: C % 32, aligned slice");
    const long long blocks = (npix * (C / 8) + 255) / 256;
    hipLaunchKernelGGL(split_h2_kernel, dim3((unsigned)(blocks > 16384 ? 16384 : blocks)), dim3(256), 0, (hipStream_t)stream, x, src_cs,
                       src_co, C, (_Float16*)dst, npix, overflow_flag);
    RD_LAUNCH_CHECK();
    return RDPN6D_OK;
}

int conv_h2_launch_pp(ConvH2Args& ax, int shape, hipStream_t s);

static int h2_pp_plan(const rdpn6d_conv_desc* d, long long M, int* pbm, int* pbn)
{
    static const int on = getenv("RDPN6D_H2_PP") ? atoi(getenv("RDPN6D_H2_PP")) : 1;
    static const int force = getenv("RDPN6D_H2_PP_SHAPE") ? atoi(getenv("RDPN6D_H2_PP_SHAPE")) : -1;
    if (!on || d->Npad % 128 != 0 || d->ntaps * (d->Cin / 32) < 8) return -1;
    int shape = 0;
    if ((long long)rd_cdiv(M, 256) * (d->Npad / 128) >= 224 && (long long)rd_cdiv(M, 128) * (d->Npad / 128) > 288) shape = 2;
    if (force == 0 || force == 2) shape = force;
    const int bm = shape == 0 ? 128 : 256;
    if ((long long)rd_cdiv(M, bm) * (d->Npad / 128) < 224) return -1;
    *pbm = bm;
    *pbn = 128;
    return shape;
}

static int h2_tile_ksplit(const rdpn6d_conv_desc* d, long long M, int bm, int bn)
{
    static const int off = getenv("RDPN6D_H2_NO_SPLITK") ? 1 : 0;
    const long long tiles = (long long)rd_cdiv(M, bm) * (d->Npad / bn);
    static const int tmax = getenv("RDPN6D_H2_SPLIT_TILES") ? atoi(getenv("RDPN6D_H2_SPLIT_TILES")) : 128;
    if (off || tiles >= tmax) return 0;
    const int nk = d->ntaps * (d->Cin / 32);
    int best = 0;
    for (int sl = 2; sl <= 32; sl *= 2)
        if (tiles * sl <= 512 && nk % sl == 0 && nk / sl >= 4) best = sl;
    return best;
}

static int g_h2_wfrag_mode = getenv("RDPN6D_H2_BFG") ? atoi(getenv("RDPN6D_H2_BFG")) : 0;
extern "C" void rdpn6d_conv_h2_set_wfrag(int mode) { g_h2_wfrag_mode = mode; }
static unsigned long long* g_h2_clk_probe = nullptr;
extern "C" void rdpn6d_conv_h2_set_clock_probe(unsigned long long* buf) { g_h2_clk_probe = buf; }
static bool h2_wfrag_shape_ok(int shape)
{
    const int mode = g_h2_wfrag_mode;
    return mode >= 1 && (shape == 0 || (mode >= 2 && shape == 2));
}

extern "C" int rdpn6d_conv_h2_kernel_for(const rdpn6d_conv_desc* d)
{
    if (!d || !h2_common_ok(d)) return 0;
    const long long M = (long long)d->B * d->Ho * d->Wo;
    return (h2_big_ok(d) && h2_big_pays(d, M)) ? 2 : 1;
}

extern "C" int rdpn6d_conv2d_h2_cb(const rdpn6d_conv_desc* d, void* y_h2, const void* res_h2, int* overflow_flag, const float* crop_bias,
                                   void* stream);
extern "C" int rdpn6d_conv2d_h2(const rdpn6d_conv_desc* d, void* y_h2, const void* res_h2, int* overflow_flag, void* stream)
{
    return rdpn6d_conv2d_h2_cb(d, y_h2, res_h2, overflow_flag, nullptr, stream);
}

extern "C" long long rdpn6d_conv_h2_workspace_bytes(const rdpn6d_conv_desc* d)
{
    if (!d || rdpn6d_conv_h2_kernel_for(d) != 1) return 0;
    const long long M = (long long)d->B * d->Ho * d->Wo;
    int bm, bn;
    if (h2_pp_plan(d, M, &bm, &bn) >= 0) return 0;
    h2_pick_tile(d, M, &bm, &bn);
    return (long long)h2_tile_ksplit(d, M, bm, bn) * rd_cdiv(M, bm) * bm * d->Npad * 4;
}

extern "C" int rdpn6d_conv2d_h2_ws(const rdpn6d_conv_desc* d, void* y_h2, const void* res_h2, int* overflow_flag, const float* crop_bias,
                                   void* workspace, long long workspace_bytes, void* stream);
extern "C" int rdpn6d_conv2d_h2_cb(const rdpn6d_conv_desc* d, void* y_h2, const void* res_h2, int* overflow_flag, const float* crop_bias,
                                   void* stream)
{
    return rdpn6d_conv2d_h2_ws(d, y_h2, res_h2, overflow_flag, crop_bias, nullptr, 0, stream);
}

struct H2Fuse {
    const void* w;
    const float *scale, *bias;
    float* out;
    int cs, n;
};
static int conv2d_h2_impl(const rdpn6d_conv_desc* d, void* y_h2, const void* res_h2, int* overflow_flag, const float* crop_bias,
                          void* workspace, long long workspace_bytes, const H2Fuse* fuse, void* stream, const void* w_frag = nullptr);

extern "C" int rdpn6d_conv2d_h2_ws(const rdpn6d_conv_desc* d, void* y_h2, const void* res_h2, int* overflow_flag, const float* crop_bias,
                                   void* workspace, long long workspace_bytes, void* stream)
{
    return conv2d_h2_impl(d, y_h2, res_h2, overflow_flag, crop_bias, workspace, workspace_bytes, nullptr, stream);
}

extern "C" int rdpn6d_conv_h2_wfrag_wanted(const rdpn6d_conv_desc* d)
{
    if (!d || rdpn6d_conv_h2_kernel_for(d) != 1) return 0;
    int bm, bn;
    const int shape = h2_pp_plan(d, (long long)d->B * d->Ho * d->Wo, &bm, &bn);
    return shape >= 0 && h2_wfrag_shape_ok(shape) ? 1 : 0;
}

extern "C" int rdpn6d_conv2d_h2_wf(const rdpn6d_conv_desc* d, void* y_h2, const void* res_h2, int* overflow_flag, const void* w_frag,
                                   void* stream)
{
    return conv2d_h2_impl(d, y_h2, res_h2, overflow_flag, nullptr, nullptr, 0, nullptr, stream, w_frag);
}

__global__ void h2_weight_frag_kernel(const uint4* __restrict__ w, uint4* __restrict__ out, int ntaps, int cchunks, long long nslots)
{
    const long long i = (long long)blockIdx.x * blockDim.x + threadIdx.x;
    if (i >= nslots) return;
    const int r = (int)(i & 31), sl = (int)((i >> 5) & 7);
    const long long blk = i >> 8;
    const int cc = (int)(blk % cchunks);
    const long long t2 = blk / cchunks;
    const int tap = (int)(t2 % ntaps);
    const long long n32 = t2 / ntaps;
    out[i] = w[(((n32 * 32 + r) * ntaps + tap) * cchunks + cc) * 8 + sl];
}

extern "C" int rdpn6d_h2_weight_frag(const void* w_h2, int Npad, int ntaps, int cchunks, void* w_frag, void* stream)
{
    RD_REQUIRE(w_h2 && w_frag && w_h2 != w_frag, "null pointer / in place");
    RD_REQUIRE(Npad > 0 && Npad % 32 == 0 && ntaps >= 1 && cchunks >= 1, "shape (Npad % 32)");
    const long long nslots = (long long)Npad * ntaps * cchunks * 8;
    hipLaunchKernelGGL(h2_weight_frag_kernel, dim3((unsigned)((nslots + 255) / 256)), dim3(256), 0, (hipStream_t)stream,
                       (const uint4*)w_h2, (uint4*)w_frag, ntaps, cchunks, nslots);
    RD_LAUNCH_CHECK();
    return RDPN6D_OK;
}

extern "C" int rdpn6d_conv_h2_fuse1x1_ok(const rdpn6d_conv_desc* d)
{
    return d && rdpn6d_conv_h2_kernel_for(d) == 2 && d->Npad == 256 && d->N == 256;
}
extern "C" int rdpn6d_conv2d_h2_fuse1x1(const rdpn6d_conv_desc* d, const void* res_h2, int* overflow_flag, const float* crop_bias,
                                        const void* w1_h2, const float* scale1, const float* bias1, float* out, int out_cs, int n_out,
                                        void* stream)
{
    RD_REQUIRE(d && w1_h2 && scale1 && bias1 && out, "null pointer");
    RD_REQUIRE(rdpn6d_conv_h2_fuse1x1_ok(d), "fused 1x1 output convolution: needs the 256x256 kernel with N == Npad == 256");
    RD_REQUIRE(n_out >= 1 && n_out <= out_cs && out_cs <= 64 && out_cs % 8 == 0, "n_out <= out_cs <= 64, out_cs % 8 == 0");
    RD_REQUIRE(d->y == nullptr, "the fused form does not write the activation (desc.y must be null)");
    RD_REQUIRE(!res_h2 && !crop_bias && !d->res, "the fused 1x1 form takes no residual and no per-crop bias");
    const H2Fuse f = {w1_h2, scale1, bias1, out, out_cs, n_out};
    return conv2d_h2_impl(d, nullptr, res_h2, overflow_flag, crop_bias, nullptr, 0, &f, stream);
}

extern "C" int rdpn6d_conv_h2_colmax_ok(const rdpn6d_conv_desc* d, int rows_per_group)
{
    return d && rdpn6d_conv_h2_kernel_for(d) == 2 && rows_per_group > 0 && rows_per_group % 256 == 0 && d->act == 0 && !d->res &&
           ((long long)d->B * d->Ho * d->Wo) % rows_per_group == 0 && d->osy == 1 && d->osx == 1 && d->ooy == 0 && d->oox == 0 && d->OH == d->Ho && d->OW == d->Wo;
}
extern "C" int rdpn6d_conv2d_h2_colmax(const rdpn6d_conv_desc* d, unsigned long long* keys, int rows_per_group, int* overflow_flag,
                                       void* stream)
{
    RD_REQUIRE(d && keys, "null pointer");
    RD_REQUIRE(rdpn6d_conv_h2_colmax_ok(d, rows_per_group), "column-max form: 256x256 kernel, rows_per_group % 256 == 0, linear output, no activation / residual");
    RD_REQUIRE(d->y == nullptr, "the column-max form does not write the activation (desc.y must be null)");
    const long long groups = (long long)d->B * d->Ho * d->Wo / rows_per_group;
    RD_CHECK_HIP(hipMemsetAsync(keys, 0, (size_t)groups * d->Npad * sizeof(unsigned long long), (hipStream_t)stream));
    const H2Fuse f = {nullptr, nullptr, nullptr, reinterpret_cast<float*>(keys), rows_per_group, 0};
    return conv2d_h2_impl(d, nullptr, nullptr, overflow_flag, nullptr, nullptr, 0, &f, stream);
}

__global__ void h2_colmax_decode_kernel(unsigned long long* __restrict__ keys, int groups, int N, int Npad, _Float16* __restrict__ out)
{
    const int i = blockIdx.x * blockDim.x + threadIdx.x;
    if (i >= groups * N) return;
    const int g = i / N, n = i - g * N;
    const unsigned long long k = keys[(size_t)g * Npad + n];
    keys[(size_t)g * Npad + n] = 0ull;
    const unsigned pay = (unsigned)(k & 0xffffffffull);
    _Float16* o = out + ((size_t)g * (N / 32) + (n >> 5)) * 64 + (n & 31);
    o[0] = __builtin_bit_cast(_Float16, (unsigned short)(pay >> 16));
    o[32] = __builtin_bit_cast(_Float16, (unsigned short)(pay & 0xffffu));
}
extern "C" int rdpn6d_h2_colmax_decode(unsigned long long* keys, int groups, int N, int Npad, void* out_h2, void* stream)
{
    RD_REQUIRE(keys && out_h2 && groups > 0 && N > 0 && N % 32 == 0 && Npad >= N, "shape (N % 32)");
    hipLaunchKernelGGL(h2_colmax_decode_kernel, dim3((unsigned)((groups * N + 255) / 256)), dim3(256), 0, (hipStream_t)stream, keys, groups, N,
                       Npad, (_Float16*)out_h2);
    RD_LAUNCH_CHECK();
    return RDPN6D_OK;
}

static int conv2d_h2_impl(const rdpn6d_conv_desc* d, void* y_h2, const void* res_h2, int* overflow_flag, const float* crop_bias,
                          void* workspace, long long workspace_bytes, const H2Fuse* fuse, void* stream, const void* w_frag)
{
    RD_REQUIRE(d && d->x && d->w && (d->y || y_h2 || fuse), "null pointer");
    const int which = rdpn6d_conv_h2_kernel_for(d);
    RD_REQUIRE(which != 0, "h2 needs Cin, in_cs, in_co % 32 == 0, N % 8 == 0, Npad % 64 == 0, 16-byte aligned output slices");
    RD_REQUIRE(d->B > 0 && d->H > 0 && d->W > 0 && d->Ho > 0 && d->Wo > 0 && d->ntaps >= 1 && d->ntaps <= 9, "shape");
    RD_REQUIRE(d->in_co + d->Cin <= d->in_cs && d->out_co + d->N <= d->out_cs, "channel slices");
    RD_REQUIRE((d->Ho - 1) * d->osy + d->ooy < d->OH && (d->Wo - 1) * d->osx + d->oox < d->OW, "output geometry");
    RD_REQUIRE(!(d->res && res_h2), "residual either as an fp32 tensor or as an h2 tensor");
    RD_REQUIRE(!res_h2 || (d->res_cs % 32 == 0 && d->res_co % 8 == 0 && d->res_co + d->N <= d->res_cs), "h2 residual slice");
    RD_REQUIRE(!y_h2 || (d->out_cs % 32 == 0), "h2 output: channel stride % 32");
    ConvH2Args ax;
    ConvBArgs& a = ax.b;
    a.d = *d;
    a.M = (long long)d->B * d->Ho * d->Wo;
    RD_REQUIRE(a.M < (1LL << 31), "B*Ho*Wo must fit 31 bits");
    a.HoWo = d->Ho * d->Wo;
    a.cchunks = d->Cin / 32;
    a.nk = d->ntaps * a.cchunks;
    a.Ktot = d->ntaps * d->Cin;
    a.linear_out = (d->osy == 1 && d->osx == 1 && d->ooy == 0 && d->oox == 0 && d->OH == d->Ho && d->OW == d->Wo);
    a.out_f32 = 1;
    a.vec_out = 1;
    const long long x_bytes = (long long)d->B * d->H * d->W * d->in_cs * 4, w_bytes = (long long)d->Npad * d->ntaps * d->Cin * 4;
    RD_REQUIRE(x_bytes < (1LL << 32) - 64 && w_bytes < (1LL << 32) - 64, "h2 tensors are addressed with 32-bit offsets (< 4 GiB each)");
    a.x_bytes = (unsigned)x_bytes;
    a.w_bytes = (unsigned)w_bytes;
    ax.y_h2 = y_h2;
    ax.res_h2 = res_h2;
    ax.overflow_flag = overflow_flag;
    ax.crop_bias = crop_bias;
    ax.partial = nullptr;
    ax.fuse_w = fuse ? fuse->w : nullptr;
    ax.fuse_scale = fuse ? fuse->scale : nullptr;
    ax.fuse_bias = fuse ? fuse->bias : nullptr;
    ax.fuse_out = fuse ? fuse->out : nullptr;
    ax.fuse_cs = fuse ? fuse->cs : 0;
    ax.fuse_n = fuse ? fuse->n : 0;
    ax.w_frag = nullptr;
    ax.clk_probe = g_h2_clk_probe;
    ax.nsplit = 1;
    ax.mpad = 0;
    a.dy_pack = a.dx_pack = 0;
    for (int t = 0; t < d->ntaps; ++t) {
        RD_REQUIRE(d->dy[t] >= -8 && d->dy[t] <= 7 && d->dx[t] >= -8 && d->dx[t] <= 7, "tap offsets must be in -8..7");
        a.dy_pack |= (unsigned long long)(d->dy[t] + 8) << (4 * t);
        a.dx_pack |= (unsigned long long)(d->dx[t] + 8) << (4 * t);
    }
    a.kper = a.nk;
    a.partial = nullptr;
    hipStream_t s = (hipStream_t)stream;
    if (which == 1) {
        int bm, bn;
        const int shape = h2_pp_plan(d, a.M, &bm, &bn);
        if (shape >= 0) {
            a.mtiles = rd_cdiv(a.M, bm);
            a.ntiles = d->Npad / bn;
            ax.w_frag = h2_wfrag_shape_ok(shape) ? w_frag : nullptr;
            const int rc = conv_h2_launch_pp(ax, shape, s);
            if (rc != RDPN6D_OK) return rc;
            RD_LAUNCH_CHECK();
            return RDPN6D_OK;
        }
        h2_pick_tile(d, a.M, &bm, &bn);
        a.mtiles = rd_cdiv(a.M, bm);
        a.ntiles = d->Npad / bn;
        const int ks = h2_tile_ksplit(d, a.M, bm, bn);
        if (ks && workspace && workspace_bytes >= (long long)ks * a.mtiles * bm * d->Npad * 4) {
            ax.nsplit = ks;
            ax.mpad = a.mtiles * bm;
            ax.partial = reinterpret_cast<float*>(workspace);
            a.kper = a.nk / ks;
        }
        int rc;
        static const int nst_env = getenv("RDPN6D_H2_NST") ? atoi(getenv("RDPN6D_H2_NST")) : 0;
        const bool three = nst_env ? nst_env == 3 : a.kper >= 32;
        if (bm == 128 && bn == 128) rc = (nst_env == 3) ? launch_h2_tile<128, 128, 3>(ax, s) : launch_h2_tile<128, 128, 2>(ax, s);
        else if (bm == 128) rc = three ? launch_h2_tile<128, 64, 3>(ax, s) : launch_h2_tile<128, 64, 2>(ax, s);
        else if (bn == 128) rc = three ? launch_h2_tile<64, 128, 3>(ax, s) : launch_h2_tile<64, 128, 2>(ax, s);
        else rc = three ? launch_h2_tile<64, 64, 3>(ax, s) : launch_h2_tile<64, 64, 2>(ax, s);
        if (rc != RDPN6D_OK) return rc;
        RD_LAUNCH_CHECK();
        if (ax.partial) {
            const long long items = a.M * (d->Npad / 8);
            hipLaunchKernelGGL(h2_splitk_reduce_kernel, dim3((unsigned)((items + 255) / 256 < 4096 ? (items + 255) / 256 : 4096)), dim3(256), 0, s, ax);
            RD_LAUNCH_CHECK();
        }
        return RDPN6D_OK;
    }
    a.mtiles = rd_cdiv(a.M, 256);
    a.ntiles = d->Npad / 256;
    if (fuse && !fuse->w) {
        RD_LDS_OPT_IN(conv_h2_8ph_colmax_kernel, LDS_8PH);
        hipLaunchKernelGGL(conv_h2_8ph_colmax_kernel, dim3((unsigned)(a.mtiles * a.ntiles)), dim3(512), LDS_8PH, s, ax);
        RD_LAUNCH_CHECK();
        return RDPN6D_OK;
    }
    if (fuse) {
        RD_LDS_OPT_IN(conv_h2_8ph_kernel_t<true>, LDS_8PH_FUSED);
        hipLaunchKernelGGL(conv_h2_8ph_kernel_t<true>, dim3((unsigned)(a.mtiles * a.ntiles)), dim3(512), LDS_8PH_FUSED, s, ax);
        RD_LAUNCH_CHECK();
        return RDPN6D_OK;
    }
    RD_LDS_OPT_IN(conv_h2_8ph_kernel, LDS_8PH);
#ifdef RDPN6D_PROBE
    if (const char* e = getenv("RDPN6D_H2_ABL_A")) ax.nsplit = 100 + atoi(e);
#endif
    hipLaunchKernelGGL(conv_h2_8ph_kernel, dim3((unsigned)(a.mtiles * a.ntiles)), dim3(512), LDS_8PH, s, ax);
    RD_LAUNCH_CHECK();
    return RDPN6D_OK;
}
```

rdpn6d_amd/csrc/conv_igemm_h2_pp.hip:

```cpp
#include "conv_h2_common.h"

#include <cstdio>
#include <cstdlib>

#ifdef RDPN6D_PROBE
__device__ unsigned long long* g_h2pp_probe = nullptr;
extern "C" int rdpn6d_debug_h2pp_probe(void* buf)
{
    RD_CHECK_HIP(hipMemcpyToSymbol(HIP_SYMBOL(g_h2pp_probe), &buf, sizeof(buf)));
    return RDPN6D_OK;
}
#define PP_T(i) const unsigned long long pt##i = __builtin_readcyclecounter(); __builtin_amdgcn_sched_barrier(0)
#define PP_ACC(j, a, b) pp_sum[j] += pt##b - pt##a
#else
#define PP_T(i)
#define PP_ACC(j, a, b)
#endif

namespace {

template <int BM, int BN, int WM, int WN, int NST, int PM, bool BFG = false>
__global__ __launch_bounds__(512) void conv_h2_pp_kernel(const ConvH2Args ax)
{
    constexpr int RB = 128, RPP = 8, NW = 8;
    constexpr int WTM = BM / WM, WTN = BN / WN, TM = WTM / 32, TN = WTN / 32;
    constexpr int AG = BM / RPP / NW, BG = BFG ? 0 : BN / RPP / NW;
    constexpr int NB = BFG ? 4 * TN : 0;
    constexpr int P = AG + BG, PL = P - PM, D = NST - 1;
    constexpr int Q = P + NB;
    static_assert(WM * WN == NW && WM == 2 && TM >= 1 && TN >= 1 && AG >= 1 && (BFG || BG >= 1), "wave grid / tile");
    static_assert(PM >= 0 && PM <= 2 && PL >= 1 && D >= 2, "pieces in the MFMA part; at least three stages");
    extern __shared__ __attribute__((aligned(1024))) unsigned char smem[];
    unsigned char* As = smem;
    unsigned char* Bs = smem + NST * BM * RB;
#ifdef RDPN6D_PROBE
    const unsigned long long pp_start = __builtin_readcyclecounter();
    unsigned long long pp_e[6] = {0, 0, 0, 0, 0, 0};
#endif

    const ConvBArgs& a = ax.b;
    const rdpn6d_conv_desc& d = a.d;
    const int nblk = a.mtiles * a.ntiles;
    const int bid = blockIdx.x;
    const int q8 = nblk >> 3, r8 = nblk & 7, xcd = bid & 7, kk = bid >> 3;
    const int logical = (xcd < r8 ? xcd * (q8 + 1) : r8 * (q8 + 1) + (xcd - r8) * q8) + kk;
    const int nt = logical % a.ntiles;
    const int mt = logical / a.ntiles;
    const long long m0 = (long long)mt * BM;
    const int n0 = nt * BN;

    const int tid = threadIdx.x;
    const int lane = tid & 63;
    const int wave = __builtin_amdgcn_readfirstlane(tid >> 6);
    const int grp = wave >> 2, wq = wave & 3;
    const int wm = grp, wn = wq;

    const int prow = lane >> 3, pslot = lane & 7;
    const unsigned px_bytes = (unsigned)d.in_cs * 4u;
    unsigned a_base[AG], a_mask[AG];
#pragma unroll
    for (int i = 0; i < AG; ++i) {
        const int row = (wave + NW * i) * RPP + prow;
        const long long m = m0 + row;
        const bool ok = m < a.M;
        const int mm = ok ? (int)m : 0;
        const int b = mm / a.HoWo;
        const int rem = mm - b * a.HoWo;
        const int oy = rem / d.Wo;
        const int ox = rem - oy * d.Wo;
        const int iy = oy * d.stride, ix = ox * d.stride;
        const int lslot = pslot ^ ((row >> 1) & 7);
        a_base[i] = (unsigned)((b * d.H + iy) * d.W + ix) * px_bytes + (unsigned)d.in_co * 4u + (unsigned)lslot * 16u;
        unsigned mask = 0;
        for (int t = 0; t < d.ntaps; ++t) {
            const int dy = (int)((a.dy_pack >> (4 * t)) & 15ull) - 8, dx = (int)((a.dx_pack >> (4 * t)) & 15ull) - 8;
            mask |= (ok && (unsigned)(iy + dy) < (unsigned)d.H && (unsigned)(ix + dx) < (unsigned)d.W) ? (1u << t) : 0u;
        }
        a_mask[i] = mask;
    }
    unsigned w_off[BG > 0 ? BG : 1];
#pragma unroll
    for (int i = 0; i < BG; ++i) {
        const int row = (wave + NW * i) * RPP + prow;
        const int lslot = pslot ^ ((row >> 1) & 7);
        w_off[i] = (unsigned)(n0 + row) * (unsigned)a.Ktot * 4u + (unsigned)lslot * 16u;
    }
    const __amdgpu_buffer_rsrc_t xsrc = __builtin_amdgcn_make_buffer_rsrc(const_cast<float*>(d.x), 0, a.x_bytes, 0x00020000);
    const __amdgpu_buffer_rsrc_t wsrc = __builtin_amdgcn_make_buffer_rsrc(const_cast<void*>(BFG ? ax.w_frag : (const void*)d.w), 0, a.w_bytes, 0x00020000);

    unsigned dma_off[P];
    auto stage_addr = [&](const int tap, const int cc, const bool valid) {
        const int dy = (int)((a.dy_pack >> (4 * tap)) & 15ull) - 8, dx = (int)((a.dx_pack >> (4 * tap)) & 15ull) - 8;
        const unsigned toff = (unsigned)((dy * d.W + dx) * (int)px_bytes + cc * RB);
        const unsigned sel = valid ? 0u : 0xFFFFFFFFu;
#pragma unroll
        for (int i = 0; i < AG; ++i) dma_off[i] = (a_base[i] + toff) | (((a_mask[i] >> tap) & 1u) - 1u) | sel;
        const unsigned wk = (unsigned)tap * (unsigned)d.Cin * 4u + (unsigned)cc * (unsigned)RB;
#pragma unroll
        for (int i = 0; i < BG; ++i) dma_off[AG + i] = (w_off[i] + wk) | sel;
    };
    auto stage_piece = [&](auto ic_, const int st) {
        constexpr int i = decltype(ic_)::value;
        if constexpr (i < AG) {
            unsigned char* dst = As + ((st * BM) + (wave + NW * i) * RPP) * RB;
            __builtin_amdgcn_raw_ptr_buffer_load_lds(xsrc, (lds_ptr_t)dst, 16, (int)dma_off[i], 0, 0, 0);
        } else {
            unsigned char* dst = Bs + ((st * BN) + (wave + NW * (i - AG)) * RPP) * RB;
            __builtin_amdgcn_raw_ptr_buffer_load_lds(wsrc, (lds_ptr_t)dst, 16, (int)dma_off[i], 0, 0, 0);
        }
    };
    auto stage_pieces = [&](auto firstc, auto lastc, const int st) {
        constexpr int first = decltype(firstc)::value, last = decltype(lastc)::value;
        if constexpr (first + 0 < last) stage_piece(ic<first + 0>{}, st);
        if constexpr (first + 1 < last) stage_piece(ic<first + 1>{}, st);
        if constexpr (first + 2 < last) stage_piece(ic<first + 2>{}, st);
        if constexpr (first + 3 < last) stage_piece(ic<first + 3>{}, st);
        if constexpr (first + 4 < last) stage_piece(ic<first + 4>{}, st);
        if constexpr (first + 5 < last) stage_piece(ic<first + 5>{}, st);
        if constexpr (first + 6 < last) stage_piece(ic<first + 6>{}, st);
        if constexpr (first + 7 < last) stage_piece(ic<first + 7>{}, st);
        static_assert(last - first <= 8, "pieces per wave and chunk");
    };

    constexpr int CS = WTN + 8, LPR = WTN / 8, RPI = 64 / LPR, NRR = 32 / RPI;
    const int frow = lane & 31;
    const int nb = n0 + wn * WTN;
    const int rrow = lane / LPR, c8 = (lane % LPR) * 8;
    const long long mbase = m0 + wm * WTM;
    f16x8 rh[TM][NRR], rl[TM][NRR];
    long long pixs[TM][NRR];
    const bool res_pre = ax.res_h2 != nullptr && d.res == nullptr;
#pragma unroll
    for (int i = 0; i < TM; ++i)
#pragma unroll
        for (int rr = 0; rr < NRR; ++rr) {
            const long long mrow = mbase + i * 32 + rr * RPI + rrow;
            const bool ok = mrow < a.M && nb + c8 < d.N;
            pixs[i][rr] = ok ? h2_pixel_of(a, mrow) : -1;
            if (res_pre && ok) {
                const int c = d.res_co + nb + c8;
                const _Float16* rp = reinterpret_cast<const _Float16*>(ax.res_h2) + pixs[i][rr] * (2 * d.res_cs) + (c >> 5) * 64 + (c & 31);
                rh[i][rr] = *reinterpret_cast<const f16x8*>(rp);
                rl[i][rr] = *reinterpret_cast<const f16x8*>(rp + 32);
            } else {
                rh[i][rr] = f16x8{};
                rl[i][rr] = f16x8{};
            }
        }
    float scj[TN], shj[TN];
#pragma unroll
    for (int j = 0; j < TN; ++j) {
        const int n = nb + j * 32 + frow;
        scj[j] = d.scale ? d.scale[n] : 1.f;
        shj[j] = d.shift ? d.shift[n] : 0.f;
    }

    const int nk = a.nk;
    int ld_cc = 0, ld_tap = 0, ld_idx = 0;
    auto next_chunk = [&]() {
        ++ld_idx;
        ++ld_tap;
        const int wrap = ld_tap == d.ntaps ? 1 : 0;
        ld_tap = wrap ? 0 : ld_tap;
        ld_cc += wrap;
    };

    const int half = lane >> 5;
    u32x4 fa[TM][4], fb[BFG ? 3 * TN : TN][4];
    const unsigned wf_lane = (unsigned)lane * 16u;
    const unsigned wf_n32 = (unsigned)(n0 + wn * WTN) / 32u;
    auto load_bfrags = [&](auto slotc, const int tap, const int cc, const bool valid) {
        constexpr int slot = decltype(slotc)::value;
        if constexpr (BFG) {
#pragma unroll
            for (int jn = 0; jn < TN; ++jn) {
                const unsigned base = (((wf_n32 + (unsigned)jn) * (unsigned)d.ntaps + (unsigned)tap) * (unsigned)a.cchunks + (unsigned)cc) * 4096u;
                const unsigned so = valid ? base : 0xFFFFF000u;
#pragma unroll
                for (int j = 0; j < 4; ++j)
                    fb[slot * TN + jn][j] = __builtin_bit_cast(u32x4, __builtin_amdgcn_raw_buffer_load_b128(wsrc, (int)wf_lane, (int)(so + j * 1024u), 0));
            }
        }
    };
    auto read_frags = [&](const int st) {
#pragma unroll
        for (int i = 0; i < TM; ++i) {
            const int R = wm * WTM + i * 32 + frow;
            const int sw = (R >> 1) & 7;
            const unsigned char* q = As + ((st * BM) + R) * RB;
#pragma unroll
            for (int j = 0; j < 4; ++j) fa[i][j] = *reinterpret_cast<const u32x4*>(q + (((2 * j + half) ^ sw) << 4));
        }
        if constexpr (!BFG) {
#pragma unroll
            for (int jn = 0; jn < TN; ++jn) {
                const int R = wn * WTN + jn * 32 + frow;
                const int sw = (R >> 1) & 7;
                const unsigned char* q = Bs + ((st * BN) + R) * RB;
#pragma unroll
                for (int j = 0; j < 4; ++j) fb[jn][j] = *reinterpret_cast<const u32x4*>(q + (((2 * j + half) ^ sw) << 4));
            }
        }
    };

    f32x16 acc[TM][TN];
#pragma unroll
    for (int i = 0; i < TM; ++i)
#pragma unroll
        for (int j = 0; j < TN; ++j)
#pragma unroll
            for (int e = 0; e < 16; ++e) acc[i][j][e] = 0.f;

    auto mma_group = [&](auto prc, auto slotc) {
        constexpr int pr = decltype(prc)::value, slot = decltype(slotc)::value;
        H2_PAIRS;
#pragma unroll
        for (int i = 0; i < TM; ++i)
#pragma unroll
            for (int jn = 0; jn < TN; ++jn) acc[i][jn] = h2_mfma(fa[i][H2_PA[pr]], fb[slot * TN + jn][H2_PB[pr]], acc[i][jn]);
    };

    int lb_cc = 0, lb_tap = 0, lb_idx = 0;
    auto next_b = [&]() {
        ++lb_idx;
        ++lb_tap;
        const int wrap = lb_tap == d.ntaps ? 1 : 0;
        lb_tap = wrap ? 0 : lb_tap;
        lb_cc += wrap;
    };
    static_assert(!BFG || D <= 3, "BFG: the counted waits below assume the weight stream (2 chunks ahead) is not behind the DMA ring");

    auto pro_step = [&](auto cc_) {
        constexpr int c = decltype(cc_)::value;
        if constexpr (c < D) {
            stage_addr(ld_tap, ld_cc, ld_idx < nk);
            stage_pieces(ic<0>{}, ic<PL>{}, c);
            if constexpr (BFG && c - D + 2 >= 0) {
                load_bfrags(ic<c - D + 2>{}, lb_tap, lb_cc, lb_idx < nk);
                next_b();
            }
            stage_pieces(ic<PL>{}, ic<P>{}, c);
            next_chunk();
        }
    };
    pro_step(ic<0>{});
    pro_step(ic<1>{});
    pro_step(ic<2>{});
    pro_step(ic<3>{});
    static_assert(D <= 4, "prologue steps");
    stage_addr(ld_tap, ld_cc, ld_idx < nk);
    asm volatile("s_waitcnt vmcnt(%0)" ::"n"((D - 1) * Q) : "memory");
    __builtin_amdgcn_s_barrier();
    asm volatile("" ::: "memory");
    if (grp == 1) __builtin_amdgcn_s_barrier();

    int st_rd = 0, st_wr = D;
#ifdef RDPN6D_PROBE
    unsigned long long pp_sum[6] = {0, 0, 0, 0, 0, 0};
    const unsigned long long pp_t0 = __builtin_readcyclecounter();
#endif
    constexpr int N1a = (D - 2) * Q + PL + NB, N1 = (BFG && N1a > 2 * Q) ? 2 * Q : N1a, N3 = (D - 1) * Q;
    static_assert(N1 <= 63 && N3 <= 63, "vmcnt is a 6-bit counter");
    auto step = [&](auto slotc) {
        constexpr int slot = decltype(slotc)::value;
        __builtin_amdgcn_sched_barrier(0);
        PP_T(0);
        read_frags(st_rd);
        __builtin_amdgcn_sched_barrier(0);
        stage_pieces(ic<0>{}, ic<PL>{}, st_wr);
        if constexpr (BFG) {
            load_bfrags(ic<(slot + 2) % 3>{}, lb_tap, lb_cc, lb_idx < nk);
            next_b();
        }
        __builtin_amdgcn_sched_barrier(0);
        PP_T(1);
        asm volatile("s_waitcnt vmcnt(%0) lgkmcnt(0)" ::"n"(N1) : "memory");
        PP_T(2);
        __builtin_amdgcn_s_barrier();
        asm volatile("" ::: "memory");
        __builtin_amdgcn_sched_barrier(0);
        PP_T(3);
        __builtin_amdgcn_s_setprio(1);
        mma_group(ic<0>{}, slotc);
        mma_group(ic<1>{}, slotc);
        __builtin_amdgcn_sched_barrier(0);
        if constexpr (PM >= 1) stage_piece(ic<PL>{}, st_wr);
        __builtin_amdgcn_sched_barrier(0);
        mma_group(ic<2>{}, slotc);
        mma_group(ic<3>{}, slotc);
        __builtin_amdgcn_sched_barrier(0);
        if constexpr (PM >= 2) stage_piece(ic<PL + 1>{}, st_wr);
        __builtin_amdgcn_sched_barrier(0);
        next_chunk();
        stage_addr(ld_tap, ld_cc, ld_idx < nk);
        mma_group(ic<4>{}, slotc);
        mma_group(ic<5>{}, slotc);
        __builtin_amdgcn_s_setprio(0);
        __builtin_amdgcn_sched_barrier(0);
        PP_T(4);
        st_rd = st_rd == NST - 1 ? 0 : st_rd + 1;
        st_wr = st_wr == NST - 1 ? 0 : st_wr + 1;
        asm volatile("s_waitcnt vmcnt(%0)" ::"n"(N3) : "memory");
        PP_T(5);
        __builtin_amdgcn_s_barrier();
        asm volatile("" ::: "memory");
        PP_T(6);
        PP_ACC(0, 0, 1);
        PP_ACC(1, 1, 2);
        PP_ACC(2, 2, 3);
        PP_ACC(3, 3, 4);
        PP_ACC(4, 4, 5);
        PP_ACC(5, 5, 6);
    };
    if constexpr (BFG) {
        int k = 0;
        for (; k + 3 <= nk; k += 3) {
            step(ic<0>{});
            step(ic<1>{});
            step(ic<2>{});
        }
        if (k < nk) step(ic<0>{});
        if (k + 1 < nk) step(ic<1>{});
    } else {
        for (int k = 0; k < nk; ++k) step(ic<0>{});
    }
#ifdef RDPN6D_PROBE
    const unsigned long long pp_loop_end = __builtin_readcyclecounter();
#endif
    asm volatile("s_waitcnt vmcnt(0)" ::: "memory");
    if (grp == 0) __builtin_amdgcn_s_barrier();
#ifdef RDPN6D_PROBE
    pp_e[0] = __builtin_readcyclecounter();
#endif

    {
        const int hi = lane >> 5;
        __builtin_amdgcn_s_barrier();
        asm volatile("" ::: "memory");
#ifdef RDPN6D_PROBE
        pp_e[1] = __builtin_readcyclecounter();
#endif
        float* cst = reinterpret_cast<float*>(smem) + wave * (32 * CS);
#pragma unroll
        for (int i = 0; i < TM; ++i) {
#pragma unroll
            for (int j = 0; j < TN; ++j)
#pragma unroll
                for (int e = 0; e < 16; ++e)
                    cst[((e & 3) + 8 * (e >> 2) + 4 * hi) * CS + j * 32 + frow] = acc[i][j][e] * scj[j] + shj[j];
#pragma unroll
            for (int rr = 0; rr < NRR; ++rr) {
                const int row = rr * RPI + rrow;
                if (pixs[i][rr] >= 0) {
                    const f32x4 lo = *reinterpret_cast<const f32x4*>(cst + row * CS + c8);
                    const f32x4 hi4 = *reinterpret_cast<const f32x4*>(cst + row * CS + c8 + 4);
                    float v[8] = {lo[0], lo[1], lo[2], lo[3], hi4[0], hi4[1], hi4[2], hi4[3]};
                    if (res_pre) h2_finish_row8_t<true>(ax, v, pixs[i][rr], nb + c8, rh[i][rr], rl[i][rr]);
                    else h2_finish_row8_t<false>(ax, v, pixs[i][rr], nb + c8, rh[i][rr], rl[i][rr]);
                }
            }
        }
    }
#ifdef RDPN6D_PROBE
    pp_e[2] = __builtin_readcyclecounter();
    asm volatile("s_waitcnt vmcnt(0)" ::: "memory");
    pp_e[3] = __builtin_readcyclecounter();
    if (g_h2pp_probe && lane == 0) {
        unsigned long long* o = g_h2pp_probe + ((size_t)blockIdx.x * 8 + wave) * 16;
        for (int i = 0; i < 6; ++i) o[i] = pp_sum[i];
        o[6] = pp_loop_end - pp_t0;
        o[7] = (unsigned long long)nk;
        o[8] = pp_t0 - pp_start;
        o[9] = pp_e[0] - pp_loop_end;
        o[10] = pp_e[1] - pp_e[0];
        o[11] = pp_e[2] - pp_e[1];
        o[12] = pp_e[3] - pp_e[2];
    }
#endif
}

template <int BM, int BN, int WM, int WN, int NST, int PM, bool BFG = false>
int launch_pp(const ConvH2Args& ax, hipStream_t s)
{
    constexpr int lds_stage = NST * (BM + (BFG ? 0 : BN)) * 128;
    constexpr int lds_epi = 8 * 32 * (BN / WN + 8) * 4;
    constexpr int lds = lds_stage > lds_epi ? lds_stage : lds_epi;
    static_assert(lds <= 160 * 1024, "LDS");
    auto kern = conv_h2_pp_kernel<BM, BN, WM, WN, NST, PM, BFG>;
    RD_LDS_OPT_IN(kern, lds);
    hipLaunchKernelGGL(kern, dim3((unsigned)(ax.b.mtiles * ax.b.ntiles)), dim3(512), lds, s, ax);
    return RDPN6D_OK;
}

}

int conv_h2_launch_pp(ConvH2Args& ax, int shape, hipStream_t s)
{
    static const int pm = getenv("RDPN6D_H2_PP_PM") ? atoi(getenv("RDPN6D_H2_PP_PM")) : 2;
    if (ax.w_frag) {
        static const int bpm = getenv("RDPN6D_H2_BFG_PM") ? atoi(getenv("RDPN6D_H2_BFG_PM")) : 1;
        if (shape == 0) return bpm == 0 ? launch_pp<128, 128, 2, 4, 4, 0, true>(ax, s) : launch_pp<128, 128, 2, 4, 4, 1, true>(ax, s);
        if (shape == 2) return bpm == 0 ? launch_pp<256, 128, 2, 4, 4, 0, true>(ax, s) : bpm == 1 ? launch_pp<256, 128, 2, 4, 4, 1, true>(ax, s) : launch_pp<256, 128, 2, 4, 4, 2, true>(ax, s);
    }
    if (shape == 0) return pm == 0 ? launch_pp<128, 128, 2, 4, 4, 0>(ax, s) : pm == 1 ? launch_pp<128, 128, 2, 4, 4, 1>(ax, s) : launch_pp<128, 128, 2, 4, 4, 2>(ax, s);
    if (shape == 2) return pm == 0 ? launch_pp<256, 128, 2, 4, 3, 0>(ax, s) : pm == 1 ? launch_pp<256, 128, 2, 4, 3, 1>(ax, s) : launch_pp<256, 128, 2, 4, 3, 2>(ax, s);
    rdpn6d_set_error("conv_h2_launch_pp: unknown tile shape %d", shape);
    return RDPN6D_EINVAL;
}
```

rdpn6d_amd/gdrn.py:

```python
import ctypes
import os

import torch
import torch.nn as nn

from . import _lib

import weakref

_MODELS = weakref.WeakSet()


def bump_weights_epoch(tensors=None):
    if isinstance(tensors, nn.Module):
        tensors._weights_epoch += 1
        return
    ids = None if tensors is None else {id(t) for t in tensors}
    for m in list(_MODELS):
        if ids is None or not ids.isdisjoint(m._tensor_ids()):
            m._weights_epoch += 1


RESNET_SPEC = {18: (1, (2, 2, 2, 2)), 34: (1, (3, 4, 6, 3)), 50: (4, (3, 4, 6, 3)), 101: (4, (3, 4, 23, 3)),
               152: (4, (3, 8, 36, 3))}
# ... 144 lines not shown
                ds = bi == 0 and (s != 1 or cin != cout)
                blocks.append(BlockP(cin, planes, s, ds) if exp == 1 else BottleneckP(cin, planes, s, ds))
                cin = cout
            setattr(self, f"layer{li + 1}", _HolderSeq(*blocks))


class RotHeadP(_Holder):
    def __init__(self, num_regions, num_filters=256, num_layers=3, in_channels=1024, mask_out_dim=1):
        super().__init__()
        f = [ConvP(in_channels, num_filters, 3, 2, 1, transposed=True), BNP(num_filters), Slot()]
        for _ in range(2 * num_layers):
            f += [ConvP(num_filters, num_filters, 3, 1, 1), BNP(num_filters), Slot()]
        f.append(ConvP(num_filters, mask_out_dim + 3 + num_regions + 1, 1, bias=True))
        self.features = _HolderList(f)


class ConvPnPP(_Holder):
    def __init__(self, n_in, featdim=128, rot_dim=6, out_res=64):
        super().__init__()
        f = []
        for i in range(3):
            f += [ConvP(n_in if i == 0 else featdim, featdim, 3, 2, 1), GNP(32, featdim), Slot()]
        self.features = _HolderList(f)
        self.fc1 = LinearP(featdim * (out_res // 8) ** 2, 1024)
        self.fc2 = LinearP(1024, 256)
        self.fc_r = LinearP(256, rot_dim, std=0.01)
        self.fc_t = LinearP(256, 3, std=0.01)


def _pad_to(n, m):
    return (n + m - 1) // m * m


def _ptr(t):
    return ctypes.c_void_p(t.data_ptr()) if t is not None else None


def pack_conv_weight(w, cin_pad=None, perm=None):
    cout, cin, kh, kw = w.shape
    if perm is not None:
        w = w[:, perm]
    cin_pad = cin_pad or _pad_to(cin, 16)
    npad = _pad_to(cout, 64)
    out = torch.zeros(npad, kh * kw, cin_pad, dtype=torch.float32, device=w.device)
    out[:cout, :, :cin] = w.permute(0, 2, 3, 1).reshape(cout, kh * kw, cin)
    return out.contiguous()


H2_ACT_SCALE = 16.0


def pack_h2_weight(w32):
    npad, taps, cin = w32.shape
    assert cin % 32 == 0, cin
    mx = w32.abs().amax(dim=(1, 2))
    e = torch.floor(13.0 - torch.log2(mx.clamp_min(1e-30)))
    sw = torch.where(mx > 0, torch.exp2(e), torch.ones_like(mx))
    ws = w32 * sw[:, None, None]
    hi = ws.half()
    lo = (ws - hi.float()).half()
    out = torch.stack([hi.view(npad, taps, cin // 32, 32), lo.view(npad, taps, cin // 32, 32)], dim=3).contiguous()
    assert torch.isfinite(out.float()).all()
    return out, (1.0 / (sw * H2_ACT_SCALE)).float().contiguous()


def pack_stem_h2_weight(w_oihw):
    w = w_oihw.detach().float()
    wk = torch.zeros(64, 24, 8, dtype=torch.float32, device=w.device)
    wk[:, :21, :7] = w.reshape(64, 21, 7)
    return pack_h2_weight(wk.reshape(64, 1, 192))


def fold_bn(bn, conv_bias=None, npad=None):
    g, b = bn.weight.detach().double(), bn.bias.detach().double()
    m, v = bn.running_mean.double(), bn.running_var.double()
    scale = g / torch.sqrt(v + bn.eps)
    shift = b - m * scale
    if conv_bias is not None:
        shift = shift + conv_bias.detach().double() * scale
    return _pad_vec(scale.float(), npad, 1.0), _pad_vec(shift.float(), npad, 0.0)


def _pad_vec(v, npad, fill):
    npad = npad or _pad_to(v.numel(), 64)
    out = torch.full((npad,), fill, dtype=torch.float32, device=v.device)
    out[: v.numel()] = v
    return out


def pick_ksplit(M, npad, nk):
    blocks = ((M + 63) // 64) * (npad // 64)
    ks = min(nk // 8, max(1, 768 // blocks))
    return ks if ks >= 2 else 1


class _Launch:

    __slots__ = ("fn", "args", "name", "keep")

    def __init__(self, name, fn, args, keep=()):
        self.name, self.fn, self.args, self.keep = name, fn, args, keep


_SIGMA_MAX_CACHE = {}


def _sigma_max_upper_bound(w):
    import hashlib
    import math

    wh = w.detach().to("cpu", torch.float32).contiguous()
    key = (tuple(wh.shape), hashlib.blake2b(wh.numpy().tobytes(), digest_size=16).hexdigest())
    hit = _SIGMA_MAX_CACHE.get(key)
    if hit is not None:
        return hit
    a = wh.double()
    g = a @ a.t() if a.shape[0] <= a.shape[1] else a.t() @ a
    if not bool(torch.isfinite(g).all()):
        return float("inf")
    log_scale, k = 0.0, 1
    for _ in range(7):
        tr = float(g.diagonal().sum())
        if tr <= 0.0:
            return 0.0
        g = g / tr
        g = g @ g
        log_scale, k = 2.0 * (log_scale + math.log(tr)), 2 * k
    lam = math.exp((log_scale + math.log(max(float(g.diagonal().sum()), 1e-300))) / k)
    out = math.sqrt(lam) * (1.0 + 1e-9)
    if len(_SIGMA_MAX_CACHE) > 64:
        _SIGMA_MAX_CACHE.clear()
    _SIGMA_MAX_CACHE[key] = out
    return out


class InferencePlan:

    def __init__(self, model, B, device, bf16=False):
        self.lib = _lib.load()
        self.lp = None if not bf16 else ("bf16" if bf16 is True else str(bf16))
        if self.lp not in (None, "bf16", "fp16"):
            raise ValueError(f"16-bit format {self.lp!r}: bf16 | fp16")
        self.lp_dtype = torch.float16 if self.lp == "fp16" else torch.bfloat16
        self.B, self.device, self.bf16 = B, device, self.lp is not None
        self.launches = []
        self._graphs = {}
        self.bufs = {}
        self.keep = []
        cfg = model.cfg
        self.fused_gmax = False
        self.h2_wfrag = bool(cfg.get("TEST", {}).get("H2_WFRAG", False))
        if self.h2_wfrag:
            self.lib.rdpn6d_conv_h2_set_wfrag(1)
        self.R = int(cfg.MODEL.CDPN.BACKBONE.INPUT_RES)
        self.K = int(cfg.MODEL.CDPN.ROT_HEAD.NUM_REGIONS)
        self.mask_attention = cfg.MODEL.CDPN.PNP_NET.MASK_ATTENTION
        if self.mask_attention not in ("none", "mul"):
            raise ValueError(f"MASK_ATTENTION={self.mask_attention!r} is not implemented (none | mul)")
        self.mask_type = MASK_TYPES[str(cfg.MODEL.CDPN.ROT_HEAD.MASK_LOSS_TYPE)]
        self.mask_channels = 2 if self.mask_type == 2 else 1
        if self.mask_attention != "none" and self.mask_type == 2:
            raise NotImplementedError("MASK_ATTENTION with ROT_HEAD.MASK_LOSS_TYPE='CE': get_mask_prob's CE branch raises in the reference "
                                      "itself (torch.softmax has no keepdim argument, models/model_utils.py:39)")
        tcfg = cfg.get("TEST", {})
        self.fast = None if (self.bf16 or not tcfg.get("BF16X3", True)) else ("h2" if tcfg.get("FP16X2", True) else "x3")
        self.x3 = self.fast is not None
        self.x3_launches = 0
        self.h2_flag = model.h2_range_flag(device)
        self._exp_table = dict(model.h2_exponents(device))
        self._slots, self._texp, self._tvar = [], {}, {}
        self._h2_out, self._probe = {}, None
        self._tile_min_rows = int(os.environ.get("RDPN6D_TILE_MIN_ROWS", 1024 if self.fast == "h2" else 8192))
        self._side_stream = None
        self._build(model)

    def exp(self, var):
        return int(self._exp_table.get(var, 4)) if var is not None else 4

    def flag_ptr(self, var):
        n = self.h2_flag.numel()
        if len(self._slots) >= n - 1:
            if len(self._slots) == n - 1:
                self._slots.append(None)
            return ctypes.c_void_p(self.h2_flag.data_ptr() + 4 * (n - 1))
        self._slots.append(var)
        return ctypes.c_void_p(self.h2_flag.data_ptr() + 4 * (len(self._slots) - 1))

    def tag(self, t, e, var):
        if t is not None:
            self._texp[t.data_ptr()], self._tvar[t.data_ptr()] = int(e), var

    def exp_of(self, t):
        return self._texp.get(t.data_ptr(), 4) if t is not None else 4

    def buf(self, name, *shape, dtype=torch.float32, zero=False):
        if name not in self.bufs:
            fn = torch.zeros if zero else torch.empty
            self.bufs[name] = fn(*shape, dtype=dtype, device=self.device)
        return self.bufs[name]

    def conv(self, name, x, xshape, w, scale, shift, y, yshape, *, cin, in_cs, in_co=0, k=1, stride=1, pad=0, N,
             out_cs, out_co=0, res=None, res_cs=0, res_co=0, act=0, slope=0.0, taps=None, phase=None, lowp=False,
             out_f32=False, ksplit=False):
        d = _lib.ConvDesc()
        d.x, d.w, d.scale, d.shift, d.res, d.y = _ptr(x), _ptr(w), _ptr(scale), _ptr(shift), _ptr(res), _ptr(y)
        d.B, d.H, d.W = self.B, xshape[0], xshape[1]
        d.Cin, d.in_cs, d.in_co = cin, in_cs, in_co
        if taps is None:
            taps = [(ky - pad, kx - pad) for ky in range(k) for kx in range(k)]
        d.ntaps = len(taps)
        for t, (dy, dx) in enumerate(taps):
            d.dy[t], d.dx[t] = dy, dx
        d.stride = stride
        d.N, d.Npad = N, w.shape[0]
        d.OH, d.OW = yshape
        if phase is None:
            d.Ho, d.Wo, d.osy, d.osx, d.ooy, d.oox = yshape[0], yshape[1], 1, 1, 0, 0
        else:
            d.Ho, d.Wo, d.osy, d.osx, d.ooy, d.oox = phase
        d.out_cs, d.out_co, d.res_cs, d.res_co = out_cs, out_co, res_cs, res_co
        d.act, d.slope = act, slope
        assert w.shape[1] == d.ntaps and w.shape[2] == cin, (name, tuple(w.shape), d.ntaps, cin)
        self.keep += [w, scale, shift]
        nk = d.ntaps * cin // (64 if (lowp and cin % 64 == 0) else (32 if lowp else 16))
        ks = pick_ksplit(self.B * d.Ho * d.Wo, d.Npad, nk) if phase is None else 1
        if ks > 1:
            ws = self.buf("splitk_ws:" + name, int(self.lib.rdpn6d_conv_splitk_ws_floats(ctypes.byref(d), ks)))
            if lowp:
                self.launches.append(_Launch(name, getattr(self.lib, f"rdpn6d_conv2d_splitk_{self.lp}"), (ctypes.byref(d), 1 if out_f32 else 0, ks, _ptr(ws)),
                                             keep=(d,)))
            else:
                self.launches.append(_Launch(name, self.lib.rdpn6d_conv2d_splitk_f32, (ctypes.byref(d), ks, _ptr(ws)), keep=(d,)))
        elif lowp:
            assert w.dtype == self.lp_dtype, name
            self.launches.append(_Launch(name, getattr(self.lib, f"rdpn6d_conv2d_{self.lp}"), (ctypes.byref(d), 1 if out_f32 else 0), keep=(d,)))
        else:
            assert w.dtype == torch.float32, name
            self.launches.append(_Launch(name, self.lib.rdpn6d_conv2d_f32, (ctypes.byref(d),), keep=(d,)))

    def x3_ok(self, M, N, cin, ntaps):
        kc = 32 if self.fast == "h2" else 16
        if not self.x3 or N % 256 or cin % kc or (ntaps * (cin // kc)) % 2:
            return False
        if self._fast_bytes(M, max(N, cin)) >= (1 << 32) - 64:
            self._x3_limit_warning(M, max(N, cin))
            return False
        tiles = ((M + 255) // 256) * (N // 256)
        rounds = (tiles + 255) // 256
        return tiles >= 160 and tiles / (256.0 * rounds) >= 0.62

    def x3_tile_ok(self, M, N, cin):
        if self.x3 and N % 64 == 0 and cin % 32 == 0 and M >= self._tile_min_rows and self._fast_bytes(M, max(N, cin)) >= (1 << 32) - 64:
            self._x3_limit_warning(M, max(N, cin))
        return self.x3 and N % 64 == 0 and cin % 32 == 0 and M >= self._tile_min_rows and self._fast_bytes(M, max(N, cin)) < (1 << 32) - 64

    def _fast_bytes(self, M, C):
        return (4 if self.fast == "h2" else 6) * M * C

    def planes_buf(self, name, npix, C):
        if self.fast == "h2":
            return self.buf(name, npix * C * 2, dtype=torch.float16)
        return self.buf(name, 3, npix * C, dtype=torch.bfloat16)

    def _x3_limit_warning(self, M, C):
        if not getattr(self, "_x3_warned", False):
            self._x3_warned = True
            import warnings

            warnings.warn(f"rdpn6d_amd: batch {self.B}: an activation of {M} x {C} elements needs {self._fast_bytes(M, C) / 2**30:.1f} GiB in "
                          "plane form (> 4 GiB buffer-descriptor range): those layers run on the fp32 MFMA kernel instead "
                          "(about 1.5x slower per layer); split the batch (<= 256 crops per call at 256x256) to stay on the fast path",
                          RuntimeWarning, stacklevel=3)

    def split3(self, name, x, planes):
        if self.fast == "h2":
            C = x.shape[-1]
            self.launches.append(_Launch(name, self.lib.rdpn6d_split_h2, (_ptr(x), C, 0, C, _ptr(planes), x.numel() // C, self.flag_ptr(None))))
            return
        self.launches.append(_Launch(name, self.lib.rdpn6d_split_bf16x3, (_ptr(x), x.numel(), _ptr(planes), planes.shape[1])))

    def weight_planes(self, w32):
        n = w32.numel()
        wp = torch.empty(3, _pad_to(n, 8), dtype=torch.bfloat16, device=self.device)
        _lib.check(self.lib.rdpn6d_split_bf16x3(_ptr(w32.contiguous()), n, _ptr(wp), wp.shape[1], None), "split weights")
        torch.cuda.synchronize(self.device)
        return wp

    def h2_workspace(self, nbytes):
        cur = self.bufs.get("h2_workspace")
        if cur is None or cur.numel() < nbytes:
            self.bufs["h2_workspace"] = cur = torch.empty(max(nbytes, 8 << 20), dtype=torch.uint8, device=self.device)
            for L in list(self.launches) + list(getattr(self, "_main_launches", ())):
                if L.fn is self.lib.rdpn6d_conv2d_h2_ws:
                    L.args = L.args[:5] + (_ptr(cur), cur.numel())
        return cur

    def conv_x3(self, name, xp, xshape, w32, scale, shift, y, yp, yshape, *, cin, in_cs, k=1, stride=1, pad=0, N, out_cs, act=0,
                slope=0.0, taps=None, phase=None, res_planes=None, res_cs=0, crop_bias=None, fuse=None, evar=None):
        fptr = None
        if self.fast == "h2":
            wp, inv = pack_h2_weight(w32.contiguous())
            e_in = self.exp_of(xp)
            if yp is None and fuse is None:
                evar, e_out = None, 4
                if res_planes is not None and self.exp_of(res_planes) != 4:
                    raise NotImplementedError(f"{name}: fp32 output with a residual stored at 2^{self.exp_of(res_planes)} (h2 exponents other "
# ... 399 lines not shown
                    self.fused_out = True
                    pa, pb = pb, pa
                    continue
                self.conv_x3(f"rot_head.features.{i}", pa, (R4, R4), w32, sch, shh, b if is_last else None,
                             None if is_last else pb, (R4, R4), cin=F, in_cs=F, k=3, pad=1, N=F, out_cs=F, act=1, evar=f"rot_head.features.{i}")
                pa, pb = pb, pa
            else:
                wh = pw(head.features[i].weight.detach().float())
                sch, shh = fold_bn(head.features[i + 1], npad=wh.shape[0])
                self.conv(f"rot_head.features.{i}", a, (R4, R4), wh, sch, shh, b, (R4, R4), cin=F, in_cs=F, k=3, stride=1,
                          pad=1, N=F, out_cs=F, act=1, lowp=lp)
            a, b = b, a
        wl = pw(last.weight.detach().float())
        bl = _pad_vec(last.bias.detach().float(), wl.shape[0], 0.0)
        if self.fused_out:
            pass
        elif h2_pw and x3_head and self.head_cs % 8 == 0:
            self.conv_x3("rot_head.out", pa, (R4, R4), wl, None, bl, ho, None, (R4, R4), cin=F, in_cs=F, k=1, N=self.head_cs,
                         out_cs=self.head_cs, act=0)
        else:
            if h2_pw:
                raise NotImplementedError("h2 point-wise mode needs a head output width that pads to a multiple of 8")
            self.conv("rot_head.out", a, (R4, R4), wl, None, bl, ho, (R4, R4), cin=F, in_cs=F, N=nout, out_cs=self.head_cs,
                      lowp=lp, out_f32=True)

        HW = R4 * R4
        self.pnp_h2 = bool(h2_pw and x3_head and self.fast == "h2" and model.cfg.get("TEST", {}).get("PNP_H2", True)
                           and pnp.features[0].weight.shape[0] % 32 == 0 and (B * R4 * R4) % 256 == 0 and self._pnp_h2_range_ok(pnp, R4))
        self.pnp_cs = _pad_to(11 + K, 32 if self.pnp_h2 else 16)
        self.out_nchw = self.buf("out_nchw", B, nout, R4, R4)
        pnp_in = self.planes_buf("pnp_in_planes", B * HW * self.pnp_cs, 1) if self.pnp_h2 else self.buf("pnp_in", B, HW, self.pnp_cs)
        self.argmax = self.buf("argmax", B, HW, dtype=torch.int32)
        minmax = self.buf("minmax", B, 2)
        self.glue_fn = lib.rdpn6d_dense_glue_mt_h2 if self.pnp_h2 else lib.rdpn6d_dense_glue_mt_f32
        self.glue_args = lambda coord2d, fps: (_ptr(ho), self.head_cs, _ptr(coord2d), _ptr(fps), B, HW, K,
                                               1 if self.mask_attention == "mul" else 0, self.mask_type, _ptr(minmax),
                                               _ptr(self.out_nchw), _ptr(pnp_in), self.pnp_cs, _ptr(self.argmax)) + (
                                                   (self.flag_ptr(None),) if self.pnp_h2 else ())
        self.post = []
        main, self.launches = self.launches, self.post
        self._main_launches = main

        x, hw, cin = pnp_in, R4, self.pnp_cs
        for i in range(0, 9, 3):
            conv, gn = pnp.features[i], pnp.features[i + 1]
            fd = conv.weight.shape[0]
            wpn = pack_conv_weight(conv.weight.detach().float(), cin_pad=cin)
            y = self.buf(f"pnp_c{i}", B, hw // 2, hw // 2, fd)
            g, bta = gn.weight.detach().float().contiguous(), gn.bias.detach().float().contiguous()
            self.keep += [g, bta]
            if self.pnp_h2:
                self.conv_x3(f"pnp_net.features.{i}", x, (hw, hw), wpn, None, None, y, None, (hw // 2, hw // 2), cin=cin, in_cs=cin, k=3,
                             stride=2, pad=1, N=fd, out_cs=fd, act=0)
                yh = self.planes_buf(f"pnp_c{i}_planes", B * (hw // 2) ** 2 * fd, 1)
                self.call(f"pnp_net.features.{i + 1}", lib.rdpn6d_groupnorm_relu_h2, _ptr(y), B, (hw // 2) ** 2, fd, gn.groups, _ptr(g),
                          _ptr(bta), _ptr(yh), self.flag_ptr(None))
                x, hw, cin = yh, hw // 2, fd
                continue
            self.conv(f"pnp_net.features.{i}", x, (hw, hw), wpn, None, None, y, (hw // 2, hw // 2), cin=cin, in_cs=cin,
                      k=3, stride=2, pad=1, N=fd, out_cs=fd)
            self.call(f"pnp_net.features.{i + 1}", lib.rdpn6d_groupnorm_relu_f32, _ptr(y), B, (hw // 2) ** 2, fd, gn.groups,
                      _ptr(g), _ptr(bta))
            x, hw, cin = y, hw // 2, fd
        kin = cin * hw * hw
        w1 = pnp.fc1.weight.detach().float().view(-1, cin, hw, hw).permute(0, 2, 3, 1).reshape(-1, kin)
        w1p = torch.zeros(_pad_to(w1.shape[0], 64), 1, kin, **f32)
        w1p[: w1.shape[0], 0] = w1
        w2 = pnp.fc2.weight.detach().float()
        w2p = torch.zeros(_pad_to(w2.shape[0], 64), 1, w2.shape[1], **f32)
        w2p[: w2.shape[0], 0] = w2
        wrt = torch.cat([pnp.fc_r.weight.detach().float(), pnp.fc_t.weight.detach().float()], 0)
        brt = torch.cat([pnp.fc_r.bias.detach().float(), pnp.fc_t.bias.detach().float()], 0)
        if wrt.shape[0] != 9:
            raise ValueError("only ROT_TYPE *_rot6d (rot_dim 6) is implemented")
        wrtp = torch.zeros(64, 1, wrt.shape[1], **f32)
        wrtp[:9, 0] = wrt
        self.rt = self.buf("rt", B, 16, zero=True)
        if self.pnp_h2:
            n1, n2 = w1.shape[0], w2.shape[0]
            f1, f2 = self.planes_buf("fc1_planes", B * n1, 1), self.planes_buf("fc2_planes", B * n2, 1)
            b1 = _pad_vec(pnp.fc1.bias.detach().float(), w1p.shape[0], 0.0)
            b2 = _pad_vec(pnp.fc2.bias.detach().float(), w2p.shape[0], 0.0)
            b3 = _pad_vec(brt, 64, 0.0)
            self.conv_x3("pnp_net.fc1", x, (1, 1), w1p, None, b1, None, f1, (1, 1), cin=kin, in_cs=kin, N=n1, out_cs=n1, act=2, slope=0.1)
            self.conv_x3("pnp_net.fc2", f1, (1, 1), w2p, None, b2, None, f2, (1, 1), cin=n1, in_cs=n1, N=n2, out_cs=n2, act=2, slope=0.1)
            self.conv_x3("pnp_net.fc_r|fc_t", f2, (1, 1), wrtp, None, b3, self.rt, None, (1, 1), cin=n2, in_cs=n2, N=16, out_cs=16, act=0)
        else:
            f1 = self.buf("fc1", B, w1.shape[0])
            self._fc("pnp_net.fc1", x, kin, w1p, pnp.fc1.bias, f1, w1.shape[0], act=2)
            f2 = self.buf("fc2", B, w2.shape[0])
            self._fc("pnp_net.fc2", f1, w2.shape[1], w2p, pnp.fc2.bias, f2, w2.shape[0], act=2)
            self._fc("pnp_net.fc_r|fc_t", f2, wrt.shape[1], wrtp, brt, self.rt, 9, act=0, out_cs=16)
        segs = (("rot", (B, 3, 3), torch.float32), ("trans", (B, 3), torch.float32),
                ("pnp_pose", (B, 12), torch.float32), ("pnp_ninl", (B,), torch.int32), ("pnp_mask", (B, HW), torch.uint8))
        self._small_layout, off = [], 0
        for nm, shp, dt in segs:
            nb = int(torch.Size(shp).numel()) * torch.empty((), dtype=dt).element_size()
            self._small_layout.append((nm, off, nb, shp, dt))
            off += _pad_to(nb, 16)
        self._small = self.buf("small_outputs", off, dtype=torch.uint8)
        for nm, t in self.small_views(self._small).items():
            setattr(self, nm, t)
        self.pnp_best = self.buf("pnp_best", B, dtype=torch.int32)
        self.launches = main

    @staticmethod
    def _pnp_h2_range_ok(pnp, R4, limit=4000.0):
        hw = R4
        gn = None
        with torch.no_grad():
            for i in (0, 3, 6):
                gn, hw = pnp.features[i + 1], hw // 2
                n = (gn.weight.numel() // gn.groups) * hw * hw
                if float(gn.weight.abs().max()) * n ** 0.5 + float(gn.bias.abs().max()) >= limit:
                    return False
            C = gn.weight.numel()
            n = (C // gn.groups) * hw * hw
            w1 = pnp.fc1.weight.double()
            if w1.shape[1] != C * hw * hw:
                return False
            gam = gn.weight.double().repeat_interleave(hw * hw)
            bet = gn.bias.double().repeat_interleave(hw * hw)
            b1 = (w1 * gam).view(w1.shape[0], gn.groups, n).norm(dim=2).sum(1) * n ** 0.5 + (w1 * bet).abs().sum(1) + pnp.fc1.bias.double().abs()
            if float(b1.max()) >= limit:
                return False
            smax = _sigma_max_upper_bound(pnp.fc1.weight)
            pre = smax * (float(gn.weight.abs().max()) * float(w1.shape[1]) ** 0.5 + float(bet.norm())) + float(pnp.fc1.bias.double().norm())
            pre = min(pre, float(b1.norm()))
            b2 = pnp.fc2.weight.double().norm(dim=1) * pre + pnp.fc2.bias.double().abs()
            return bool(float(b2.max()) < limit)

    def bind_outputs(self, fresh):
        if fresh:
            self.out_nchw = torch.empty_like(self.bufs["out_nchw"])
            self._small = torch.empty_like(self.bufs["small_outputs"])
        else:
            self.out_nchw, self._small = self.bufs["out_nchw"], self.bufs["small_outputs"]
        for nm, t in self.small_views(self._small).items():
            setattr(self, nm, t)

    def small_views(self, buf):
        return {nm: buf[o:o + nb].view(dt).view(*shp) for nm, o, nb, shp, dt in self._small_layout}

    def _fc(self, name, x, kin, wp, bias, y, nout, act, out_cs=None):
        b = _pad_vec(bias.detach().float(), wp.shape[0], 0.0)
        self.conv(name, x, (1, 1), wp, None, b, y, (1, 1), cin=kin, in_cs=kin, N=nout, out_cs=out_cs or nout, act=act,
                  slope=0.1, ksplit=True)

    def run(self, x, roi_coord_2d, fps, roi_cams, roi_centers, roi_whs, resize_ratios, is_allo=True, train_pose=False, after_glue=None,
            after_h2=None):
        lib = self.lib
        st = ctypes.c_void_p(torch.cuda.current_stream().cuda_stream)
        B = self.B
        _lib.check(self.stem_fn(_ptr(x), self.stem_args[0], x.shape[1], *self.stem_args[2:], st), "stem")
        _lib.check(self.xyz_fn(_ptr(x), self.xyz_args[0], x.shape[1], *self.xyz_args[2:], st), "xyz")
        probe = self._probe
        if probe is not None:
            probe(("stem", self.stem_args))
        for L in self.launches:
            _lib.check(L.fn(*L.args, st), L.name)
            if probe is not None:
                probe(L)
        self.flag_read_queued = False
        if not self.pnp_h2 and after_h2 is not None and not torch.cuda.is_current_stream_capturing():
            after_h2()
            self.flag_read_queued = True
        _lib.check(self.glue_fn(*self.glue_args(roi_coord_2d, fps), st), "dense_glue")
        if self.pnp_h2 and after_h2 is not None and not torch.cuda.is_current_stream_capturing():
            after_h2()
            self.flag_read_queued = True
        side = None
        if after_glue is not None:
            if self._side_stream is None:
                self._side_stream = torch.cuda.Stream(device=self.device)
            side = self._side_stream
            side.wait_stream(torch.cuda.current_stream())
            with torch.cuda.stream(side):
                after_glue()
        for L in self.post:
            _lib.check(L.fn(*L.args, st), L.name)
        _lib.check(lib.rdpn6d_pose_decode_f32(_ptr(self.rt), 16, _ptr(roi_cams), _ptr(roi_centers), _ptr(roi_whs),
                                              _ptr(resize_ratios), B, 1 if is_allo else 0, 1 if train_pose else 0,
                                              _ptr(self.rot), _ptr(self.trans), st), "pose_decode")
        if side is not None:
            torch.cuda.current_stream().wait_stream(side)

    def range_exceeded(self, wait=True):
        if self.fast != "h2":
            return False
        if wait:
            torch.cuda.current_stream().synchronize()
        return bool(int(self.h2_flag.ne(0).any().item()))

    def run_graphed(self, key, launch):
        g = self._graphs.get(key)
        if g is None:
            launch()
            self._graphs[key] = "seen"
            return
        if g == "seen":
            if len([v for v in self._graphs.values() if v != "seen"]) >= 4:
                launch()
                return
            torch.cuda.synchronize()
            g = torch.cuda.CUDAGraph()
            with torch.cuda.graph(g):
                launch()
            self._graphs[key] = g
        g.replay()

    def run_pnp2d(self, roi_coord_2d, roi_extents, roi_cams, im_hw, uv_channels, mask_thr=0.5, reproj_thr=3.0, iters=100, confidence=0.99,
                  seed=0, net_mode=0, max_t_diff=1.0, minimal=0):
        assert im_hw.dtype == torch.int32 and tuple(im_hw.shape) == (self.B, 2) and im_hw.is_cuda and im_hw.is_contiguous()
        st = ctypes.c_void_p(torch.cuda.current_stream().cuda_stream)
        B, C = self.B, self.out_nchw.shape[1]
        HW = self.out_nchw.shape[2] * self.out_nchw.shape[3]
        ip, mp = self.buf("pnp2d_ip", B, HW, 2), self.buf("pnp2d_mp", B, HW, 3)
        cnt = self.buf("pnp2d_cnt", B, dtype=torch.int32)
        _lib.check(self.lib.rdpn6d_select_correspondences_mt_f32(
            _ptr(self.out_nchw), C, _ptr(roi_coord_2d), roi_coord_2d.shape[1], uv_channels[0], uv_channels[1], _ptr(roi_extents), _ptr(im_hw),
            0, 0, B, HW, mask_thr, self.mask_type, _ptr(ip), _ptr(mp), _ptr(cnt), None, None, st), "select_correspondences")
        netp = None
        if net_mode:
            netp = self.buf("net_pose", B, 12)
            netp[:, :9].copy_(self.rot.view(B, 9))
            netp[:, 9:].copy_(self.trans)
        cams = roi_cams.reshape(B, 9)
        ws = self.buf("pnp2d_ws", int(self.lib.rdpn6d_ransac_pnp_workspace_bytes(B)), dtype=torch.uint8)
        _lib.check(self.lib.rdpn6d_ransac_pnp_ws(_ptr(ip), _ptr(mp), _ptr(cnt), _ptr(cams), _ptr(netp), B, HW, reproj_thr, iters, confidence,
                                                 seed, net_mode, max_t_diff, int(minimal), _ptr(self.pnp_pose), _ptr(self.pnp_ninl),
                                                 _ptr(self.pnp_mask), _ptr(self.pnp_best), _ptr(ws), ws.numel(), st), "ransac_pnp")
        self.pnp_counts = cnt

    def run_ransac(self, roi_coord_2d, fps, roi_extents, resize_ratios, mask_thr=0.5, inlier_thr=0.01, iters=100,
                   confidence=0.99, seed=0, net_mode=0, max_t_diff=1.0):
        st = ctypes.c_void_p(torch.cuda.current_stream().cuda_stream)
        HW = self.out_nchw.shape[2] * self.out_nchw.shape[3]
        netp = None
        if net_mode:
            netp = self.buf("net_pose", self.B, 12)
            netp[:, :9].copy_(self.rot.view(self.B, 9))
            netp[:, 9:].copy_(self.trans)
        ws = self.buf("ransac_ws", int(self.lib.rdpn6d_ransac_workspace_bytes(self.B)), dtype=torch.uint8)
        _lib.check(self.lib.rdpn6d_ransac_kabsch_ws_mt(
            _ptr(self.out_nchw), _ptr(roi_coord_2d), _ptr(fps), _ptr(roi_extents), _ptr(resize_ratios), _ptr(self.argmax), _ptr(netp),
            self.B, HW, self.K, mask_thr, self.mask_type, inlier_thr, iters, confidence, seed, net_mode or 1, max_t_diff, _ptr(self.pnp_pose),
            _ptr(self.pnp_ninl), _ptr(self.pnp_mask), _ptr(self.pnp_best), _ptr(ws), ws.numel(), st), "ransac_kabsch")


def get_xyz_mask_region_out_dim(cfg):
    r = cfg.MODEL.CDPN.ROT_HEAD
    if r.XYZ_LOSS_TYPE not in ("MSE", "L1", "L2", "SmoothL1"):
        raise NotImplementedError(f"unknown / unsupported xyz loss type: {r.XYZ_LOSS_TYPE}")
    if r.MASK_LOSS_TYPE not in MASK_TYPES:
        raise NotImplementedError(f"unknown mask loss type: {r.MASK_LOSS_TYPE}")
    region_out_dim = r.NUM_REGIONS + 1
    assert region_out_dim > 2, region_out_dim
    return 3, (2 if r.MASK_LOSS_TYPE == "CE" else 1), region_out_dim


MASK_TYPES = {"L1": 0, "BCE": 1, "CE": 2}


class GDRN(_TreeWatch, nn.Module):
    def __init__(self, cfg, backbone, rot_head_net, trans_head_net=None, pnp_net=None):
        super().__init__()
        assert cfg.MODEL.CDPN.NAME == "GDRN", cfg.MODEL.CDPN.NAME
        self.backbone = backbone
        self.rot_head_net = rot_head_net
        self.pnp_net = pnp_net
        self.trans_head_net = trans_head_net
        self.cfg = cfg
        self._plans = {}
        self._weights_epoch = 0
        self._stamp_tensors = None
        self._stamp_tree_epoch = -1
        _MODELS.add(self)
        self._h2_flags = {}
        self._h2_exp = {}

    NFLAG = 512

    @staticmethod
    def _dev_key(device):
        device = torch.device(device)
        if device.type == "cuda" and device.index is None:
            device = torch.device("cuda", torch.cuda.current_device())
        return str(device)

    def h2_range_flag(self, device):
        key = self._dev_key(device)
        if key not in self._h2_flags:
            self._h2_flags[key] = [torch.zeros(self.NFLAG, dtype=torch.int32, device=device), torch.zeros(self.NFLAG, dtype=torch.int32).pin_memory(), None]
        return self._h2_flags[key][0]

    def h2_exponents(self, device):
        return self._h2_exp.setdefault(self._dev_key(device), {})

    def _lower_h2_exponents(self, plan, device, binades=2, floor=-12):
        ent = self._h2_flags.get(self._dev_key(device))
        if ent is None or ent[2] is None:
            return False
        ent[2].synchronize()
        hit = torch.nonzero(ent[1]).reshape(-1).tolist()
        slots = getattr(plan, "_slots", [])
        names = {slots[i] if i < len(slots) else None for i in hit}
# ... 632 lines not shown
```

rdpn6d_amd/ops.py:

```python
import ctypes

import numpy as np
import torch

from . import _lib
from .gdrn import _pad_to, _pad_vec, _ptr, pack_conv_weight


def _stream():
    return ctypes.c_void_p(torch.cuda.current_stream().cuda_stream)


def _need_gpu(*ts):
    for t in ts:
        if t is not None and not t.is_cuda:
            raise RuntimeError("rdpn6d_amd.ops: tensors must live on the GPU (no CPU fallback)")


def conv2d_nhwc(x, weight, scale=None, shift=None, stride=1, pad=0, residual=None, act=0, slope=0.0, out=None,
                out_co=0, in_co=0, cin=None, out_f32=False):
    _need_gpu(x, weight, scale, shift, residual, out)
    lib = _lib.load()
    B, H, W, cs = x.shape
    N, wcin, k, _ = weight.shape
    cin_real = cin or wcin
    bf = x.dtype == torch.bfloat16
    cin_pad = _pad_to(cin_real, 32 if bf else 16)
    assert in_co + cin_pad <= cs, "input slice must cover the padded reduction width"
    wp = pack_conv_weight(weight.float(), cin_pad=cin_pad)
    if bf:
        wp = wp.to(torch.bfloat16)
        assert residual is None or residual.dtype == (torch.float32 if out_f32 else torch.bfloat16)
    Ho, Wo = (H + 2 * pad - k) // stride + 1, (W + 2 * pad - k) // stride + 1
    if out is None:
        out = torch.empty(B, Ho, Wo, N, dtype=torch.bfloat16 if bf and not out_f32 else torch.float32, device=x.device)
    sc = _pad_vec(scale.float(), wp.shape[0], 1.0) if scale is not None else None
    sh = _pad_vec(shift.float(), wp.shape[0], 0.0) if shift is not None else None
    d = _lib.ConvDesc()
    d.x, d.w, d.scale, d.shift, d.res, d.y = _ptr(x), _ptr(wp), _ptr(sc), _ptr(sh), _ptr(residual), _ptr(out)
    d.B, d.H, d.W, d.Cin, d.in_cs, d.in_co = B, H, W, cin_pad, cs, in_co
    d.Ho, d.Wo, d.stride = Ho, Wo, stride
    taps = [(ky - pad, kx - pad) for ky in range(k) for kx in range(k)]
    d.ntaps = len(taps)
    for t, (dy, dx) in enumerate(taps):
        d.dy[t], d.dx[t] = dy, dx
    d.N, d.Npad, d.OH, d.OW = N, wp.shape[0], Ho, Wo
    d.osy = d.osx = 1
    d.ooy = d.oox = 0
    d.out_cs, d.out_co = out.shape[-1], out_co
    if residual is not None:
        d.res_cs, d.res_co = residual.shape[-1], 0
    d.act, d.slope = act, slope
    if bf:
        assert out.dtype == (torch.float32 if out_f32 else torch.bfloat16)
        _lib.check(lib.rdpn6d_conv2d_bf16(ctypes.byref(d), 1 if out_f32 else 0, _stream()), "conv2d_bf16")
    else:
        _lib.check(lib.rdpn6d_conv2d_f32(ctypes.byref(d), _stream()), "conv2d")
    return out


def split_bf16x3(x):
    _need_gpu(x)
    x = x.contiguous()
    n = x.numel()
    pe = _pad_to(n, 8)
    planes = torch.empty(3, pe, dtype=torch.bfloat16, device=x.device)
    _lib.check(_lib.load().rdpn6d_split_bf16x3(_ptr(x), n, _ptr(planes), pe, _stream()), "split_bf16x3")
    return planes


def conv2d_nhwc_x3(x, weight, scale=None, shift=None, stride=1, pad=0, residual=None, act=0, slope=0.0, want_planes=False,
                   residual_planes=None):
    lib = _lib.load()
    if isinstance(x, tuple):
        xp, (B, H, W, cs) = x
    else:
        B, H, W, cs = x.shape
        xp = split_bf16x3(x)
    _need_gpu(xp, weight, scale, shift, residual)
    N, wcin, k, _ = weight.shape
    cin_pad = _pad_to(wcin, 16)
    assert cin_pad <= cs
    wp32 = pack_conv_weight(weight.float(), cin_pad=cin_pad)
    wp = split_bf16x3(wp32)
    Ho, Wo = (H + 2 * pad - k) // stride + 1, (W + 2 * pad - k) // stride + 1
    out = torch.empty(B, Ho, Wo, N, dtype=torch.float32, device=xp.device)
    npe = _pad_to(out.numel(), 8)
    yp = torch.empty(3, npe, dtype=torch.bfloat16, device=xp.device) if want_planes else None
    sc = _pad_vec(scale.float(), wp32.shape[0], 1.0) if scale is not None else None
    sh = _pad_vec(shift.float(), wp32.shape[0], 0.0) if shift is not None else None
    d = _lib.ConvDesc()
    d.x, d.w, d.scale, d.shift, d.res, d.y = _ptr(xp), _ptr(wp), _ptr(sc), _ptr(sh), _ptr(residual), _ptr(out)
    d.B, d.H, d.W, d.Cin, d.in_cs, d.in_co = B, H, W, cin_pad, cs, 0
    d.Ho, d.Wo, d.stride = Ho, Wo, stride
    taps = [(ky - pad, kx - pad) for ky in range(k) for kx in range(k)]
    d.ntaps = len(taps)
    for t, (dy, dx) in enumerate(taps):
        d.dy[t], d.dx[t] = dy, dx
    d.N, d.Npad, d.OH, d.OW = N, wp32.shape[0], Ho, Wo
    d.osy = d.osx = 1
    d.ooy = d.oox = 0
    d.out_cs, d.out_co = N, 0
    if residual is not None:
        d.res_cs, d.res_co = residual.shape[-1], 0
    d.act, d.slope = act, slope
    rp = None
    if residual_planes is not None:
        rp = residual_planes[0]
        d.res_cs, d.res_co = residual_planes[1][-1], 0
    if not lib.rdpn6d_conv_bf16x3_eligible(ctypes.byref(d)):
        raise ValueError("layer not eligible for the bf16x3 kernels (Cin % 16, N % 8, aligned slices)")
    _lib.check(lib.rdpn6d_conv2d_bf16x3_ex(ctypes.byref(d), xp.shape[1], wp.shape[1], _ptr(yp), npe, _ptr(rp),
                                           rp.shape[1] if rp is not None else 0, _stream()), "conv2d_bf16x3")
    return (out, (yp, tuple(out.shape))) if want_planes else out


def split_h2(x):
    _need_gpu(x)
    x = x.contiguous()
    C = x.shape[-1]
    npix = x.numel() // C
    h2 = torch.empty(npix, C // 32, 2, 32, dtype=torch.float16, device=x.device)
    flag = torch.zeros(1, dtype=torch.int32, device=x.device)
    _lib.check(_lib.load().rdpn6d_split_h2(_ptr(x), C, 0, C, _ptr(h2), npix, _ptr(flag), _stream()), "split_h2")
    return h2, flag


def merge_h2(h2, shape):
    return ((h2[:, :, 0].float() + h2[:, :, 1].float()) / 16.0).reshape(shape)


def conv2d_nhwc_h2(x, weight, scale=None, shift=None, stride=1, pad=0, residual=None, act=0, slope=0.0, want_h2=False, residual_h2=None,
                   split_k=True, wfrag=False):
    from .gdrn import pack_h2_weight

    lib = _lib.load()
    if isinstance(x, tuple):
        xh, (B, H, W, cs) = x
    else:
        B, H, W, cs = x.shape
        xh, _ = split_h2(x)
    _need_gpu(xh, weight, scale, shift, residual)
    N, wcin, k, _ = weight.shape
    assert wcin % 32 == 0 and wcin <= cs
    wp32 = pack_conv_weight(weight.float(), cin_pad=wcin)
    wh, inv = pack_h2_weight(wp32)
    Ho, Wo = (H + 2 * pad - k) // stride + 1, (W + 2 * pad - k) // stride + 1
    out = torch.empty(B, Ho, Wo, N, dtype=torch.float32, device=xh.device)
    yh = torch.empty(B * Ho * Wo, N // 32, 2, 32, dtype=torch.float16, device=xh.device) if want_h2 else None
    flag = torch.zeros(1, dtype=torch.int32, device=xh.device)
    sc = _pad_vec(scale.float(), wp32.shape[0], 1.0) * inv if scale is not None else inv
    sh = _pad_vec(shift.float(), wp32.shape[0], 0.0) if shift is not None else None
    d = _lib.ConvDesc()
    d.x, d.w, d.scale, d.shift, d.res, d.y = _ptr(xh), _ptr(wh), _ptr(sc), _ptr(sh), _ptr(residual), _ptr(out)
    d.B, d.H, d.W, d.Cin, d.in_cs, d.in_co = B, H, W, wcin, cs, 0
    d.Ho, d.Wo, d.stride = Ho, Wo, stride
    taps = [(ky - pad, kx - pad) for ky in range(k) for kx in range(k)]
    d.ntaps = len(taps)
    for t, (dy, dx) in enumerate(taps):
        d.dy[t], d.dx[t] = dy, dx
    d.N, d.Npad, d.OH, d.OW = N, wp32.shape[0], Ho, Wo
    d.osy = d.osx = 1
    d.ooy = d.oox = 0
    d.out_cs, d.out_co = N, 0
    if residual is not None:
        d.res_cs, d.res_co = residual.shape[-1], 0
    d.act, d.slope = act, slope
    rh = None
    if residual_h2 is not None:
        rh = residual_h2[0]
        d.res_cs, d.res_co = residual_h2[1][-1], 0
    if not lib.rdpn6d_conv_h2_kernel_for(ctypes.byref(d)):
        raise ValueError("layer not eligible for the h2 kernels (Cin % 32, N % 8, aligned slices)")
    ws_bytes = int(lib.rdpn6d_conv_h2_workspace_bytes(ctypes.byref(d))) if split_k else 0
    if wfrag:
        if not lib.rdpn6d_conv_h2_wfrag_wanted(ctypes.byref(d)):
            raise ValueError("this layer's kernel has no weights-from-L2 form")
        wf = torch.empty_like(wh)
        _lib.check(lib.rdpn6d_h2_weight_frag(_ptr(wh), wh.shape[0], d.ntaps, wcin // 32, _ptr(wf), _stream()), "h2_weight_frag")
        _lib.check(lib.rdpn6d_conv2d_h2_wf(ctypes.byref(d), _ptr(yh), _ptr(rh), _ptr(flag), _ptr(wf), _stream()), "conv2d_h2_wf")
    elif ws_bytes:
        ws = torch.empty(ws_bytes, dtype=torch.uint8, device=xh.device)
        _lib.check(lib.rdpn6d_conv2d_h2_ws(ctypes.byref(d), _ptr(yh), _ptr(rh), _ptr(flag), None, _ptr(ws), ws_bytes, _stream()), "conv2d_h2")
    else:
        _lib.check(lib.rdpn6d_conv2d_h2(ctypes.byref(d), _ptr(yh), _ptr(rh), _ptr(flag), _stream()), "conv2d_h2")
    return (out, ((yh, tuple(out.shape)), flag)) if want_h2 else out


def conv2d_h2_colmax(x, weight, scale, shift, rows_per_group):
    from .gdrn import pack_h2_weight

    lib = _lib.load()
    B, H, W, cs = x.shape
    xh, _ = split_h2(x)
    N, wcin, k, _ = weight.shape
    wp32 = pack_conv_weight(weight.float(), cin_pad=wcin)
    wh, inv = pack_h2_weight(wp32)
    sc = _pad_vec(scale.float(), wp32.shape[0], 1.0) * inv
    sh = _pad_vec(shift.float(), wp32.shape[0], 0.0)
    d = _lib.ConvDesc()
    d.x, d.w, d.scale, d.shift, d.res, d.y = _ptr(xh), _ptr(wh), _ptr(sc), _ptr(sh), None, None
    d.B, d.H, d.W, d.Cin, d.in_cs, d.in_co = B, H, W, wcin, cs, 0
    d.Ho, d.Wo, d.stride = H, W, 1
    taps = [(ky - k // 2, kx - k // 2) for ky in range(k) for kx in range(k)]
    d.ntaps = len(taps)
    for t, (dy, dx) in enumerate(taps):
        d.dy[t], d.dx[t] = dy, dx
    d.N, d.Npad, d.OH, d.OW = N, wp32.shape[0], H, W
    d.osy = d.osx = 1
    d.ooy = d.oox = 0
    d.out_cs, d.out_co, d.act, d.slope = N, 0, 0, 0.0
    if not lib.rdpn6d_conv_h2_colmax_ok(ctypes.byref(d), rows_per_group):
        raise ValueError("layer not eligible for the column-max form (256x256 kernel, rows_per_group % 256 == 0)")
    groups = B * H * W // rows_per_group
    keys = torch.zeros(groups, d.Npad, dtype=torch.int64, device=x.device)
    out = torch.empty(groups, N // 32, 2, 32, dtype=torch.float16, device=x.device)
    flag = torch.zeros(1, dtype=torch.int32, device=x.device)
    _lib.check(lib.rdpn6d_conv2d_h2_colmax(ctypes.byref(d), _ptr(keys), rows_per_group, _ptr(flag), _stream()), "conv2d_h2_colmax")
    _lib.check(lib.rdpn6d_h2_colmax_decode(_ptr(keys), groups, N, d.Npad, _ptr(out), _stream()), "h2_colmax_decode")
    return out, keys, flag


def stem_conv7x7(x_nchw, weight, scale, shift):
    _need_gpu(x_nchw, weight, scale, shift)
    B, xc, R, _ = x_nchw.shape
    w = weight.float().permute(0, 2, 3, 1).contiguous()
    y = torch.empty(B, R // 2, R // 2, 64, dtype=torch.float32, device=x_nchw.device)
    _lib.check(_lib.load().rdpn6d_stem_conv7x7_f32(_ptr(x_nchw), B, xc, R, _ptr(w), _ptr(scale), _ptr(shift), _ptr(y),
                                                   _stream()), "stem")
    return y


def maxpool3x3s2(x):
    _need_gpu(x)
    B, H, W, C = x.shape
    y = torch.empty(B, (H - 1) // 2 + 1, (W - 1) // 2 + 1, C, dtype=torch.float32, device=x.device)
    _lib.check(_lib.load().rdpn6d_maxpool3x3s2_f32(_ptr(x), B, H, W, C, _ptr(y), _stream()), "maxpool")
    return y


def upsample_bilinear(x, factor):
    _need_gpu(x)
    B, H, W, C = x.shape
    y = torch.empty(B, H * factor, W * factor, C, dtype=torch.float32, device=x.device)
    _lib.check(_lib.load().rdpn6d_upsample_bilinear_f32(_ptr(x), B, H, W, C, factor, _ptr(y), _stream()), "upsample")
    return y


def global_max_concat_(buf, C):
    _need_gpu(buf)
    B, H, W, cs = buf.shape
    _lib.check(_lib.load().rdpn6d_global_max_concat_f32(_ptr(buf), B, H * W, C, cs, _stream()), "global_max_concat")
    return buf


def groupnorm_relu_(x, groups, gamma, beta):
    _need_gpu(x, gamma, beta)
    B, H, W, C = x.shape
    _lib.check(_lib.load().rdpn6d_groupnorm_relu_f32(_ptr(x), B, H * W, C, groups, _ptr(gamma), _ptr(beta), _stream()), "gn")
    return x


def farthest_point_sampling(pts, sn, init_center=False, start=None, return_index=False):
    pts = np.ascontiguousarray(pts, np.float32)
    pn, three = pts.shape
    assert three == 3
    idxs = np.zeros([sn], np.int32)
    lib = _lib.load()
    P = ctypes.c_void_p
    if init_center:
        _lib.check(lib.rdpn6d_fps_host(pts.ctypes.data_as(P), idxs.ctypes.data_as(P), pn, sn, -1), "fps")
    elif start is not None:
        _lib.check(lib.rdpn6d_fps_host(pts.ctypes.data_as(P), idxs.ctypes.data_as(P), pn, sn, int(start)), "fps")
    else:
        lib.farthest_point_sampling(pts.ctypes.data_as(P), idxs.ctypes.data_as(P), pn, sn)
        if (idxs < 0).any():
            raise RuntimeError("farthest_point_sampling failed: " + lib.rdpn6d_last_error().decode())
    return (pts[idxs], idxs) if return_index else pts[idxs]


def ransac_kabsch(out_nchw, coord2d, fps, extents, resize_ratios, region_argmax, mask_thr=0.5, inlier_thr=0.01,
                  iters=100, confidence=0.99, seed=0, net_pose=None, net_mode="ransac", max_t_diff=1.0, split=True):
    _need_gpu(out_nchw, coord2d, fps, extents, resize_ratios, region_argmax)
    B, C = out_nchw.shape[0], out_nchw.shape[1]
    HW = out_nchw[0, 0].numel()
    K = C - 5
    dev = out_nchw.device
    pose = torch.empty(B, 12, dtype=torch.float32, device=dev)
    nin = torch.empty(B, dtype=torch.int32, device=dev)
    mask = torch.empty(B, HW, dtype=torch.uint8, device=dev)
    best = torch.empty(B, dtype=torch.int32, device=dev)
    args = [t.contiguous() for t in (out_nchw, coord2d, fps, extents, resize_ratios, region_argmax)]
    assert args[5].dtype == torch.int32
    lib = _lib.load()
    ws = torch.empty(int(lib.rdpn6d_ransac_workspace_bytes(B)) if split else 1, dtype=torch.uint8, device=dev)
    npz = net_pose.float().contiguous() if net_pose is not None else None
    _lib.check(lib.rdpn6d_ransac_kabsch_ws(*[_ptr(t) for t in args], _ptr(npz), B, HW, K, mask_thr, inlier_thr, iters, confidence, seed,
                                           {"ransac": 1, "iter": 2}[net_mode], max_t_diff, _ptr(pose), _ptr(nin), _ptr(mask), _ptr(best),
                                           _ptr(ws) if split else None, ws.numel() if split else 0, _stream()), "ransac_kabsch")
    return pose, nin, mask, best


def ransac_pnp(image_points, model_points, counts, cams, reproj_thr=3.0, iters=100, confidence=0.99, seed=0, net_pose=None,
               net_mode="ransac", max_t_diff=1.0, minimal="p3p", split=True):
    _need_gpu(image_points, model_points, counts, cams)
    B, HW = image_points.shape[0], image_points.shape[1]
    dev = image_points.device
    pose = torch.empty(B, 12, dtype=torch.float32, device=dev)
    nin = torch.empty(B, dtype=torch.int32, device=dev)
    mask = torch.empty(B, HW, dtype=torch.uint8, device=dev)
    best = torch.empty(B, dtype=torch.int32, device=dev)
    args = [image_points.float().contiguous(), model_points.float().contiguous(), counts.contiguous(), cams.float().reshape(B, 9).contiguous()]
    assert args[2].dtype == torch.int32
    npz = net_pose.float().contiguous() if net_pose is not None else None
    mode = 0 if net_pose is None else {"ransac": 1, "iter": 2}[net_mode]
    lib = _lib.load()
    ws = torch.empty(int(lib.rdpn6d_ransac_pnp_workspace_bytes(B)) if split else 1, dtype=torch.uint8, device=dev)
    _lib.check(lib.rdpn6d_ransac_pnp_ws(*[_ptr(t) for t in args], _ptr(npz), B, HW, float(reproj_thr), int(iters), float(confidence),
                                        int(seed), mode, float(max_t_diff), {"p3p": 0, "epnp": 1}[str(minimal).lower()], _ptr(pose),
                                        _ptr(nin), _ptr(mask), _ptr(best), _ptr(ws) if split else None, ws.numel() if split else 0, _stream()),
               "ransac_pnp")
    return pose, nin, mask, best


def region_targets(xyz_hwc, fps64, rot, extent):
    _need_gpu(xyz_hwc, fps64, rot, extent)
    B, H, W, _ = xyz_hwc.shape
# ... 44 lines not shown
```

Measured before the change: 9656.

## Reuse loaded A fragments across 3x3 column taps via DPP lane shifts

Adds a tap-shift form to the h2 implicit-GEMM conv kernels, both the ping-pong kernel and the 64x64 tile kernel, for 3x3 stride-1 pad-1 layers whose width divides 32. Only the centre-column tap of each kernel row is loaded from global memory into LDS. The left and right taps are produced by shifting the A fragments across lanes with DPP row shifts, with edge columns zeroed. This cuts A-operand DMA and LDS reads to a third for those layers, at the cost of extra VALU shift work, a more intricate vmcnt and stage schedule, and new template instantiations. It is on by default and can be turned off through an environment variable or the config.

New measurement: 9373. -2.9%, worse.

```diff
diff --git a/include/rdpn6d.h b/include/rdpn6d.h
--- a/include/rdpn6d.h
+++ b/include/rdpn6d.h
@@ -89,6 +89,8 @@
 int rdpn6d_conv2d_h2_colmax(const rdpn6d_conv_desc* d, unsigned long long* keys, int rows_per_group, int* overflow_flag, void* stream);
 int rdpn6d_h2_colmax_decode(unsigned long long* keys, int groups, int N, int Npad, void* out_h2, void* stream);
 int rdpn6d_conv_h2_wfrag_wanted(const rdpn6d_conv_desc* d);
+void rdpn6d_conv_h2_set_tapshift(int on);
+int rdpn6d_conv_h2_tapshift_wanted(const rdpn6d_conv_desc* d);
 int rdpn6d_h2_weight_frag(const void* w_h2, int Npad, int ntaps, int cchunks, void* w_frag, void* stream);
 int rdpn6d_conv2d_h2_wf(const rdpn6d_conv_desc* d, void* y_h2, const void* res_h2, int* overflow_flag, const void* w_frag, void* stream);
 int rdpn6d_conv2d_h2_ws(const rdpn6d_conv_desc* d, void* y_h2, const void* res_h2, int* overflow_flag, const float* crop_bias,
diff --git a/rdpn6d_amd/_lib.py b/rdpn6d_amd/_lib.py
--- a/rdpn6d_amd/_lib.py
+++ b/rdpn6d_amd/_lib.py
@@ -161,6 +161,8 @@
     "rdpn6d_conv_h2_set_wfrag": (None, [_i]),
     "rdpn6d_conv_h2_set_clock_probe": (None, [_vp]),
     "rdpn6d_conv_h2_wfrag_wanted": (_i, [ctypes.POINTER(ConvDesc)]),
+    "rdpn6d_conv_h2_set_tapshift": (None, [_i]),
+    "rdpn6d_conv_h2_tapshift_wanted": (_i, [ctypes.POINTER(ConvDesc)]),
     "rdpn6d_h2_weight_frag": (_i, [_vp, _i, _i, _i, _vp, _vp]),
     "rdpn6d_conv2d_h2_wf": (_i, [ctypes.POINTER(ConvDesc), _vp, _vp, _vp, _vp, _vp]),
     "rdpn6d_ransac_pnp_f32": (_i, [_vp, _vp, _vp, _vp, _vp, _i, _i, _f, _i, _f, ctypes.c_uint, _i, _f, _vp, _vp, _vp, _vp, _vp]),
diff --git a/rdpn6d_amd/csrc/conv_igemm_h2.hip b/rdpn6d_amd/csrc/conv_igemm_h2.hip
--- a/rdpn6d_amd/csrc/conv_igemm_h2.hip
+++ b/rdpn6d_amd/csrc/conv_igemm_h2.hip
@@ -468,7 +468,7 @@
 
 constexpr auto conv_h2_8ph_kernel = conv_h2_8ph_kernel_t<false>;
 
-template <int BM, int BN, int NST, int SCHED = 0>
+template <int BM, int BN, int NST, int SCHED = 0, bool TS = false>
 __global__ __launch_bounds__(256, 2) void conv_h2_tile_kernel(const ConvH2Args ax)
 {
     constexpr int NW = 4, RB = 128;
@@ -478,6 +478,7 @@
     constexpr int AG = BM / RPP / NW, BG = BN / RPP / NW;
     constexpr int NDMA = AG + BG;
     static_assert(TM >= 1 && TN >= 1 && AG >= 1 && BG >= 1, "tile / wave layout");
+    static_assert(!TS || (NST == 3 && SCHED == 0), "tap-shift form: three stages");
     extern __shared__ __attribute__((aligned(1024))) unsigned char smem[];
     unsigned char* As = smem;
     unsigned char* Bs = smem + NST * BM * RB;
@@ -634,7 +635,110 @@
     [[maybe_unused]] unsigned long long pr_sum[5] = {0, 0, 0, 0, 0};
     [[maybe_unused]] const unsigned long long pr_start = SCHED == 9 ? __builtin_readcyclecounter() : 0ull;
     [[maybe_unused]] const unsigned long long pr_rt0 = SCHED == 9 ? (__builtin_amdgcn_s_memrealtime() & 0xffffffffull) : 0ull;
-    if constexpr (NST == 2) {
+    if constexpr (TS) {
+        int ts_idx = 0;
+        auto stage_ts = [&](auto posc, const int st) {
+            constexpr int pos = decltype(posc)::value;
+            const unsigned sel = ts_idx < nk ? 0u : 0xFFFFFFFFu;
+            if constexpr (pos == 0) {
+                const int ct = ld_tap + 1;
+                const int dy = (int)((a.dy_pack >> (4 * ct)) & 15ull) - 8, dx = (int)((a.dx_pack >> (4 * ct)) & 15ull) - 8;
+                const unsigned toff = (unsigned)((dy * d.W + dx) * (int)px_bytes + ld_cc * RB);
+#pragma unroll
+                for (int i = 0; i < AG; ++i) {
+                    const unsigned kill = ((a_mask[i] >> ct) & 1u) - 1u;
+                    unsigned char* dst = As + ((st * BM) + (wave + NW * i) * RPP) * RB;
+                    __builtin_amdgcn_raw_ptr_buffer_load_lds(xsrc, (lds_ptr_t)dst, 16, (int)((a_base[i] + toff) | kill | sel), 0, 0, 0);
+                }
+            }
+            const unsigned wk = (unsigned)ld_tap * (unsigned)d.Cin * 4u + (unsigned)ld_cc * (unsigned)RB;
+#pragma unroll
+            for (int i = 0; i < BG; ++i) {
+                unsigned char* dst = Bs + ((st * BN) + (wave + NW * i) * RPP) * RB;
+                __builtin_amdgcn_raw_ptr_buffer_load_lds(wsrc, (lds_ptr_t)dst, 16, (int)((w_off[i] + wk) | sel), 0, 0, 0);
+            }
+            ++ts_idx;
+            ++ld_tap;
+            const int wrap = ld_tap == d.ntaps ? 1 : 0;
+            ld_tap = wrap ? 0 : ld_tap;
+            ld_cc += wrap;
+        };
+        auto read_a = [&](const int st, u32x4 (&fa)[TM][4]) {
+#pragma unroll
+            for (int i = 0; i < TM; ++i) {
+                const int R = wm * WTM + i * 32 + frow;
+                const int sw = (R >> 1) & 7;
+                const unsigned char* q = As + ((st * BM) + R) * RB;
+#pragma unroll
+                for (int j = 0; j < 4; ++j) fa[i][j] = *reinterpret_cast<const u32x4*>(q + (((2 * j + half) ^ sw) << 4));
+            }
+        };
+        auto read_b = [&](const int st, u32x4 (&fb)[TN][4]) {
+#pragma unroll
+            for (int jn = 0; jn < TN; ++jn) {
+                const int R = wn * WTN + jn * 32 + frow;
+                const int sw = (R >> 1) & 7;
+                const unsigned char* q = Bs + ((st * BN) + R) * RB;
+#pragma unroll
+                for (int j = 0; j < 4; ++j) fb[jn][j] = *reinterpret_cast<const u32x4*>(q + (((2 * j + half) ^ sw) << 4));
+            }
+        };
+        const int ts_ox = frow % d.W;
+        const bool ts_first = ts_ox == 0, ts_last = ts_ox == d.W - 1;
+        u32x4 (&fc)[TM][4] = fa0;
+        u32x4 (&fsh)[TM][4] = fa1;
+        auto shift = [&](auto dirc) {
+            constexpr int dir = decltype(dirc)::value;
+#pragma unroll
+            for (int i = 0; i < TM; ++i)
+#pragma unroll
+                for (int j = 0; j < 4; ++j)
+#pragma unroll
+                    for (int e = 0; e < 4; ++e) {
+                        const int v = (int)fc[i][j][e];
+                        const int sh = dir < 0 ? __builtin_amdgcn_update_dpp(0, v, 0x138 , 0xf, 0xf, false)
+                                               : __builtin_amdgcn_update_dpp(0, v, 0x130 , 0xf, 0xf, false);
+                        fsh[i][j][e] = (dir < 0 ? ts_first : ts_last) ? 0u : (unsigned)sh;
+                    }
+        };
+        stage_ts(ic<0>{}, 0);
+        stage_ts(ic<1>{}, 1);
+        stage_ts(ic<2>{}, 2);
+        asm volatile("s_waitcnt vmcnt(%0)" ::"n"(2 * BG) : "memory");
+        __builtin_amdgcn_s_barrier();
+        asm volatile("" ::: "memory");
+        read_a(0, fc);
+        read_b(0, fb0);
+        asm volatile("s_waitcnt vmcnt(%0) lgkmcnt(0)" ::"n"(BG) : "memory");
+        __builtin_amdgcn_s_barrier();
+        asm volatile("" ::: "memory");
+        shift(ic<-1>{});
+        auto step = [&](auto posc, u32x4 (&fcur_b)[TN][4], u32x4 (&fnxt_b)[TN][4]) {
+            constexpr int pos = decltype(posc)::value;
+            stage_ts(posc, pos);
+            if constexpr (pos == 2) read_a(0, fc);
+            read_b((pos + 1) % 3, fnxt_b);
+            if constexpr (pos == 1) {
+                mma(fc, fcur_b);
+                shift(ic<1>{});
+            } else {
+                mma(fsh, fcur_b);
+            }
+            asm volatile("s_waitcnt vmcnt(%0) lgkmcnt(0)" ::"n"(pos == 0 ? AG + BG : BG) : "memory");
+            __builtin_amdgcn_s_barrier();
+            asm volatile("" ::: "memory");
+            if constexpr (pos == 2) shift(ic<-1>{});
+        };
+        for (int kc = 0; kc < nk; kc += 6) {
+            step(ic<0>{}, fb0, fb1);
+            step(ic<1>{}, fb1, fb0);
+            step(ic<2>{}, fb0, fb1);
+            step(ic<0>{}, fb1, fb0);
+            step(ic<1>{}, fb0, fb1);
+            step(ic<2>{}, fb1, fb0);
+        }
+        asm volatile("s_waitcnt vmcnt(0)" ::: "memory");
+    } else if constexpr (NST == 2) {
         stage_chunk(ld_tap, ld_cc, 0);
         next_chunk(ld_tap, ld_cc, ld_left, d.ntaps);
         stage_chunk(ld_tap, ld_cc, 1);
@@ -824,7 +928,7 @@
     }
 }
 
-template <int BM, int BN, int NST, int SCHED = 0>
+template <int BM, int BN, int NST, int SCHED = 0, bool TS = false>
 int launch_h2_tile_s(const ConvH2Args& ax, hipStream_t s);
 template <int BM, int BN, int NST>
 int launch_h2_tile(const ConvH2Args& ax, hipStream_t s)
@@ -835,14 +939,14 @@
 #endif
     return launch_h2_tile_s<BM, BN, NST, 0>(ax, s);
 }
-template <int BM, int BN, int NST, int SCHED>
+template <int BM, int BN, int NST, int SCHED, bool TS>
 int launch_h2_tile_s(const ConvH2Args& ax, hipStream_t s)
 {
     constexpr int lds_stage = NST * (BM + BN) * 128;
     constexpr int lds_epi = 4 * 32 * (BN / 2 + 8) * 4;
     constexpr int lds = lds_stage > lds_epi ? lds_stage : lds_epi;
     static_assert(lds <= 80 * 1024 || (BM == 128 && BN == 128 && NST == 3), "two workgroups per CU (128x128 with three stages: one)");
-    auto kern = conv_h2_tile_kernel<BM, BN, NST, SCHED>;
+    auto kern = conv_h2_tile_kernel<BM, BN, NST, SCHED, TS>;
     if (lds > 64 * 1024) {
         RD_LDS_OPT_IN(kern, lds);
     }
@@ -919,7 +1023,7 @@
     return RDPN6D_OK;
 }
 
-int conv_h2_launch_pp(ConvH2Args& ax, int shape, hipStream_t s);
+int conv_h2_launch_pp(ConvH2Args& ax, int shape, bool tapshift, hipStream_t s);
 
 static int h2_pp_plan(const rdpn6d_conv_desc* d, long long M, int* pbm, int* pbn)
 {
@@ -959,11 +1063,39 @@
     return mode >= 1 && (shape == 0 || (mode >= 2 && shape == 2));
 }
 
+static int g_h2_tapshift = getenv("RDPN6D_H2_TAPSHIFT") ? atoi(getenv("RDPN6D_H2_TAPSHIFT")) : 1;
+static const int g_h2_tapshift_fam = getenv("RDPN6D_H2_TAPSHIFT_FAM") ? atoi(getenv("RDPN6D_H2_TAPSHIFT_FAM")) : 7;
+extern "C" void rdpn6d_conv_h2_set_tapshift(int on) { g_h2_tapshift = on; }
+static bool h2_tapshift_layer_ok(const rdpn6d_conv_desc* d)
+{
+    if (d->ntaps != 9 || d->stride != 1 || d->Ho != d->H || d->Wo != d->W || d->W < 1 || 32 % d->W != 0) return false;
+    for (int t = 0; t < 9; ++t)
+        if (d->dy[t] != t / 3 - 1 || d->dx[t] != t % 3 - 1) return false;
+    return true;
+}
+static int h2_tapshift_plan(const rdpn6d_conv_desc* d, long long M)
+{
+    if (!g_h2_tapshift || !h2_tapshift_layer_ok(d)) return 0;
+    int bm, bn;
+    const int shape = h2_pp_plan(d, M, &bm, &bn);
+    if (shape >= 0) return (g_h2_tapshift_fam & (shape == 0 ? 1 : 2)) ? 1 : 0;
+    if (!(g_h2_tapshift_fam & 4)) return 0;
+    h2_pick_tile(d, M, &bm, &bn);
+    if (bm != 64 || bn != 64 || h2_tile_ksplit(d, M, bm, bn) != 0 || (d->Cin / 32) % 2 != 0) return 0;
+    return 2;
+}
+
 extern "C" int rdpn6d_conv_h2_kernel_for(const rdpn6d_conv_desc* d)
 {
     if (!d || !h2_common_ok(d)) return 0;
     const long long M = (long long)d->B * d->Ho * d->Wo;
     return (h2_big_ok(d) && h2_big_pays(d, M)) ? 2 : 1;
+}
+
+extern "C" int rdpn6d_conv_h2_tapshift_wanted(const rdpn6d_conv_desc* d)
+{
+    if (!d || rdpn6d_conv_h2_kernel_for(d) != 1) return 0;
+    return h2_tapshift_plan(d, (long long)d->B * d->Ho * d->Wo) != 0 ? 1 : 0;
 }
 
 extern "C" int rdpn6d_conv2d_h2_cb(const rdpn6d_conv_desc* d, void* y_h2, const void* res_h2, int* overflow_flag, const float* crop_bias,
@@ -1158,7 +1290,7 @@
             a.mtiles = rd_cdiv(a.M, bm);
             a.ntiles = d->Npad / bn;
             ax.w_frag = h2_wfrag_shape_ok(shape) ? w_frag : nullptr;
-            const int rc = conv_h2_launch_pp(ax, shape, s);
+            const int rc = conv_h2_launch_pp(ax, shape, h2_tapshift_plan(d, a.M) == 1, s);
             if (rc != RDPN6D_OK) return rc;
             RD_LAUNCH_CHECK();
             return RDPN6D_OK;
@@ -1172,6 +1304,12 @@
             ax.mpad = a.mtiles * bm;
             ax.partial = reinterpret_cast<float*>(workspace);
             a.kper = a.nk / ks;
+        }
+        if (h2_tapshift_plan(d, a.M) == 2) {
+            const int rc = launch_h2_tile_s<64, 64, 3, 0, true>(ax, s);
+            if (rc != RDPN6D_OK) return rc;
+            RD_LAUNCH_CHECK();
+            return RDPN6D_OK;
         }
         int rc;
         static const int nst_env = getenv("RDPN6D_H2_NST") ? atoi(getenv("RDPN6D_H2_NST")) : 0;
diff --git a/rdpn6d_amd/csrc/conv_igemm_h2_pp.hip b/rdpn6d_amd/csrc/conv_igemm_h2_pp.hip
--- a/rdpn6d_amd/csrc/conv_igemm_h2_pp.hip
+++ b/rdpn6d_amd/csrc/conv_igemm_h2_pp.hip
@@ -19,7 +19,14 @@
 
 namespace {
 
-template <int BM, int BN, int WM, int WN, int NST, int PM, bool BFG = false>
+constexpr int pp_ts_sum(const int first, const int last, const int AG, const int BG, const int D)
+{
+    int n = 0;
+    for (int j = first; j <= last; ++j) n += BG + ((j + 4 * D) % 3 == 0 ? AG : 0);
+    return n;
+}
+
+template <int BM, int BN, int WM, int WN, int NST, int PM, bool BFG = false, bool TS = false>
 __global__ __launch_bounds__(512) void conv_h2_pp_kernel(const ConvH2Args ax)
 {
     constexpr int RB = 128, RPP = 8, NW = 8;
@@ -30,6 +37,7 @@
     constexpr int Q = P + NB;
     static_assert(WM * WN == NW && WM == 2 && TM >= 1 && TN >= 1 && AG >= 1 && (BFG || BG >= 1), "wave grid / tile");
     static_assert(PM >= 0 && PM <= 2 && PL >= 1 && D >= 2, "pieces in the MFMA part; at least three stages");
+    static_assert(!TS || (!BFG && PM == BG && D <= 3), "tap-shift form: A pieces in the L part, B pieces in the M part");
     extern __shared__ __attribute__((aligned(1024))) unsigned char smem[];
     unsigned char* As = smem;
     unsigned char* Bs = smem + NST * BM * RB;
@@ -109,6 +117,20 @@
             __builtin_amdgcn_raw_ptr_buffer_load_lds(wsrc, (lds_ptr_t)dst, 16, (int)dma_off[i], 0, 0, 0);
         }
     };
+    auto stage_addr_ts = [&](auto posc, const int tap, const int cc, const bool valid) {
+        constexpr int pos = decltype(posc)::value;
+        const unsigned sel = valid ? 0u : 0xFFFFFFFFu;
+        if constexpr (pos == 0) {
+            const int ct = tap + 1;
+            const int dy = (int)((a.dy_pack >> (4 * ct)) & 15ull) - 8, dx = (int)((a.dx_pack >> (4 * ct)) & 15ull) - 8;
+            const unsigned toff = (unsigned)((dy * d.W + dx) * (int)px_bytes + cc * RB);
+#pragma unroll
+            for (int i = 0; i < AG; ++i) dma_off[i] = (a_base[i] + toff) | (((a_mask[i] >> ct) & 1u) - 1u) | sel;
+        }
+        const unsigned wk = (unsigned)tap * (unsigned)d.Cin * 4u + (unsigned)cc * (unsigned)RB;
+#pragma unroll
+        for (int i = 0; i < BG; ++i) dma_off[AG + i] = (w_off[i] + wk) | sel;
+    };
     auto stage_pieces = [&](auto firstc, auto lastc, const int st) {
         constexpr int first = decltype(firstc)::value, last = decltype(lastc)::value;
         if constexpr (first + 0 < last) stage_piece(ic<first + 0>{}, st);
@@ -167,6 +189,7 @@
 
     const int half = lane >> 5;
     u32x4 fa[TM][4], fb[BFG ? 3 * TN : TN][4];
+    [[maybe_unused]] u32x4 fs[TS ? TM : 1][4];
     const unsigned wf_lane = (unsigned)lane * 16u;
     const unsigned wf_n32 = (unsigned)(n0 + wn * WTN) / 32u;
     auto load_bfrags = [&](auto slotc, const int tap, const int cc, const bool valid) {
@@ -182,14 +205,16 @@
             }
         }
     };
-    auto read_frags = [&](const int st) {
-#pragma unroll
-        for (int i = 0; i < TM; ++i) {
-            const int R = wm * WTM + i * 32 + frow;
-            const int sw = (R >> 1) & 7;
-            const unsigned char* q = As + ((st * BM) + R) * RB;
-#pragma unroll
-            for (int j = 0; j < 4; ++j) fa[i][j] = *reinterpret_cast<const u32x4*>(q + (((2 * j + half) ^ sw) << 4));
+    auto read_frags = [&](const int st, auto withAc) {
+        if constexpr (decltype(withAc)::value != 0) {
+#pragma unroll
+            for (int i = 0; i < TM; ++i) {
+                const int R = wm * WTM + i * 32 + frow;
+                const int sw = (R >> 1) & 7;
+                const unsigned char* q = As + ((st * BM) + R) * RB;
+#pragma unroll
+                for (int j = 0; j < 4; ++j) fa[i][j] = *reinterpret_cast<const u32x4*>(q + (((2 * j + half) ^ sw) << 4));
+            }
         }
         if constexpr (!BFG) {
 #pragma unroll
@@ -203,6 +228,25 @@
         }
     };
 
+    const int ts_ox = frow % (TS ? d.W : 32);
+    const bool ts_first = ts_ox == 0, ts_last = ts_ox == (TS ? d.W : 32) - 1;
+    auto shift_frags = [&](auto dirc) {
+        constexpr int dir = decltype(dirc)::value;
+        if constexpr (TS) {
+#pragma unroll
+            for (int i = 0; i < TM; ++i)
+#pragma unroll
+                for (int j = 0; j < 4; ++j)
+#pragma unroll
+                    for (int e = 0; e < 4; ++e) {
+                        const int v = (int)fa[i][j][e];
+                        const int sh = dir < 0 ? __builtin_amdgcn_update_dpp(0, v, 0x138 , 0xf, 0xf, false)
+                                               : __builtin_amdgcn_update_dpp(0, v, 0x130 , 0xf, 0xf, false);
+                        fs[i][j][e] = (dir < 0 ? ts_first : ts_last) ? 0u : (unsigned)sh;
+                    }
+        }
+    };
+
     f32x16 acc[TM][TN];
 #pragma unroll
     for (int i = 0; i < TM; ++i)
@@ -213,11 +257,15 @@
 
     auto mma_group = [&](auto prc, auto slotc) {
         constexpr int pr = decltype(prc)::value, slot = decltype(slotc)::value;
+        constexpr int bs = TS ? 0 : slot;
         H2_PAIRS;
 #pragma unroll
         for (int i = 0; i < TM; ++i)
 #pragma unroll
-            for (int jn = 0; jn < TN; ++jn) acc[i][jn] = h2_mfma(fa[i][H2_PA[pr]], fb[slot * TN + jn][H2_PB[pr]], acc[i][jn]);
+            for (int jn = 0; jn < TN; ++jn) {
+                if constexpr (TS && slot != 1) acc[i][jn] = h2_mfma(fs[i][H2_PA[pr]], fb[bs * TN + jn][H2_PB[pr]], acc[i][jn]);
+                else acc[i][jn] = h2_mfma(fa[i][H2_PA[pr]], fb[bs * TN + jn][H2_PB[pr]], acc[i][jn]);
+            }
     };
 
     int lb_cc = 0, lb_tap = 0, lb_idx = 0;
@@ -232,7 +280,12 @@
 
     auto pro_step = [&](auto cc_) {
         constexpr int c = decltype(cc_)::value;
-        if constexpr (c < D) {
+        if constexpr (TS && c < D) {
+            stage_addr_ts(ic<c>{}, ld_tap, ld_cc, ld_idx < nk);
+            if constexpr (c == 0) stage_pieces(ic<0>{}, ic<AG>{}, c);
+            stage_pieces(ic<AG>{}, ic<P>{}, c);
+            next_chunk();
+        } else if constexpr (c < D) {
             stage_addr(ld_tap, ld_cc, ld_idx < nk);
             stage_pieces(ic<0>{}, ic<PL>{}, c);
             if constexpr (BFG && c - D + 2 >= 0) {
@@ -248,8 +301,9 @@
     pro_step(ic<2>{});
     pro_step(ic<3>{});
     static_assert(D <= 4, "prologue steps");
-    stage_addr(ld_tap, ld_cc, ld_idx < nk);
-    asm volatile("s_waitcnt vmcnt(%0)" ::"n"((D - 1) * Q) : "memory");
+    if constexpr (TS) stage_addr_ts(ic<D % 3>{}, ld_tap, ld_cc, ld_idx < nk);
+    else stage_addr(ld_tap, ld_cc, ld_idx < nk);
+    asm volatile("s_waitcnt vmcnt(%0)" ::"n"(TS ? (D - 1) * BG : (D - 1) * Q) : "memory");
     __builtin_amdgcn_s_barrier();
     asm volatile("" ::: "memory");
     if (grp == 1) __builtin_amdgcn_s_barrier();
@@ -265,7 +319,7 @@
         constexpr int slot = decltype(slotc)::value;
         __builtin_amdgcn_sched_barrier(0);
         PP_T(0);
-        read_frags(st_rd);
+        read_frags(st_rd, ic<1>{});
         __builtin_amdgcn_sched_barrier(0);
         stage_pieces(ic<0>{}, ic<PL>{}, st_wr);
         if constexpr (BFG) {
@@ -312,7 +366,67 @@
         PP_ACC(4, 4, 5);
         PP_ACC(5, 5, 6);
     };
-    if constexpr (BFG) {
+    auto step_ts = [&](auto posc) {
+        constexpr int pos = decltype(posc)::value;
+        constexpr int wpos = (pos + D) % 3;
+        constexpr int SHL_POS = (1 + D) % 3 == 0 ? 2 : 1;
+        constexpr int T1 = pp_ts_sum(pos + 2 - D, pos - 1, AG, BG, D) + (wpos == 0 ? AG : 0), T3 = pp_ts_sum(pos + 2 - D, pos, AG, BG, D);
+        static_assert(T1 <= 63 && T3 <= 63, "vmcnt is a 6-bit counter");
+        __builtin_amdgcn_sched_barrier(0);
+        PP_T(0);
+        read_frags(st_rd, ic<pos == 0 ? 1 : 0>{});
+        __builtin_amdgcn_sched_barrier(0);
+        if constexpr (wpos == 0) stage_pieces(ic<0>{}, ic<AG>{}, st_wr);
+        __builtin_amdgcn_sched_barrier(0);
+        if constexpr (pos == 0) shift_frags(ic<-1>{});
+        else if constexpr (pos == SHL_POS) shift_frags(ic<1>{});
+        __builtin_amdgcn_sched_barrier(0);
+        PP_T(1);
+        asm volatile("s_waitcnt vmcnt(%0) lgkmcnt(0)" ::"n"(T1) : "memory");
+        PP_T(2);
+        __builtin_amdgcn_s_barrier();
+        asm volatile("" ::: "memory");
+        __builtin_amdgcn_sched_barrier(0);
+        PP_T(3);
+        __builtin_amdgcn_s_setprio(1);
+        mma_group(ic<0>{}, posc);
+        mma_group(ic<1>{}, posc);
+        __builtin_amdgcn_sched_barrier(0);
+        stage_piece(ic<AG>{}, st_wr);
+        __builtin_amdgcn_sched_barrier(0);
+        mma_group(ic<2>{}, posc);
+        mma_group(ic<3>{}, posc);
+        __builtin_amdgcn_sched_barrier(0);
+        if constexpr (BG >= 2) stage_piece(ic<AG + 1>{}, st_wr);
+        __builtin_amdgcn_sched_barrier(0);
+        next_chunk();
+        stage_addr_ts(ic<(wpos + 1) % 3>{}, ld_tap, ld_cc, ld_idx < nk);
+        mma_group(ic<4>{}, posc);
+        mma_group(ic<5>{}, posc);
+        __builtin_amdgcn_s_setprio(0);
+        __builtin_amdgcn_sched_barrier(0);
+        PP_T(4);
+        st_rd = st_rd == NST - 1 ? 0 : st_rd + 1;
+        st_wr = st_wr == NST - 1 ? 0 : st_wr + 1;
+        asm volatile("s_waitcnt vmcnt(%0)" ::"n"(T3) : "memory");
+        PP_T(5);
+        __builtin_amdgcn_s_barrier();
+        asm volatile("" ::: "memory");
+        PP_T(6);
+        PP_ACC(0, 0, 1);
+        PP_ACC(1, 1, 2);
+        PP_ACC(2, 2, 3);
+        PP_ACC(3, 3, 4);
+        PP_ACC(4, 4, 5);
+        PP_ACC(5, 5, 6);
+    };
+    if constexpr (TS) {
+        for (int k = 0; k < nk; k += 3) {
+            step_ts(ic<0>{});
+            step_ts(ic<1>{});
+            step_ts(ic<2>{});
+        }
+    } else if constexpr (BFG) {
         int k = 0;
         for (; k + 3 <= nk; k += 3) {
             step(ic<0>{});
@@ -379,14 +493,14 @@
 #endif
 }
 
-template <int BM, int BN, int WM, int WN, int NST, int PM, bool BFG = false>
+template <int BM, int BN, int WM, int WN, int NST, int PM, bool BFG = false, bool TS = false>
 int launch_pp(const ConvH2Args& ax, hipStream_t s)
 {
     constexpr int lds_stage = NST * (BM + (BFG ? 0 : BN)) * 128;
     constexpr int lds_epi = 8 * 32 * (BN / WN + 8) * 4;
     constexpr int lds = lds_stage > lds_epi ? lds_stage : lds_epi;
     static_assert(lds <= 160 * 1024, "LDS");
-    auto kern = conv_h2_pp_kernel<BM, BN, WM, WN, NST, PM, BFG>;
+    auto kern = conv_h2_pp_kernel<BM, BN, WM, WN, NST, PM, BFG, TS>;
     RD_LDS_OPT_IN(kern, lds);
     hipLaunchKernelGGL(kern, dim3((unsigned)(ax.b.mtiles * ax.b.ntiles)), dim3(512), lds, s, ax);
     return RDPN6D_OK;
@@ -394,8 +508,12 @@
 
 }
 
-int conv_h2_launch_pp(ConvH2Args& ax, int shape, hipStream_t s)
+int conv_h2_launch_pp(ConvH2Args& ax, int shape, bool tapshift, hipStream_t s)
 {
+    if (tapshift && !ax.w_frag) {
+        if (shape == 0) return launch_pp<128, 128, 2, 4, 4, 2, false, true>(ax, s);
+        if (shape == 2) return launch_pp<256, 128, 2, 4, 3, 2, false, true>(ax, s);
+    }
     static const int pm = getenv("RDPN6D_H2_PP_PM") ? atoi(getenv("RDPN6D_H2_PP_PM")) : 2;
     if (ax.w_frag) {
         static const int bpm = getenv("RDPN6D_H2_BFG_PM") ? atoi(getenv("RDPN6D_H2_BFG_PM")) : 1;
diff --git a/rdpn6d_amd/gdrn.py b/rdpn6d_amd/gdrn.py
--- a/rdpn6d_amd/gdrn.py
+++ b/rdpn6d_amd/gdrn.py
@@ -320,6 +320,8 @@
         self.h2_wfrag = bool(cfg.get("TEST", {}).get("H2_WFRAG", False))
         if self.h2_wfrag:
             self.lib.rdpn6d_conv_h2_set_wfrag(1)
+        self.h2_tapshift = 1 if cfg.get("TEST", {}).get("H2_TAPSHIFT", True) else 0
+        self.lib.rdpn6d_conv_h2_set_tapshift(self.h2_tapshift)
         self.R = int(cfg.MODEL.CDPN.BACKBONE.INPUT_RES)
         self.K = int(cfg.MODEL.CDPN.ROT_HEAD.NUM_REGIONS)
         self.mask_attention = cfg.MODEL.CDPN.PNP_NET.MASK_ATTENTION
@@ -1025,6 +1027,7 @@
         lib = self.lib
         st = ctypes.c_void_p(torch.cuda.current_stream().cuda_stream)
         B = self.B
+        lib.rdpn6d_conv_h2_set_tapshift(self.h2_tapshift)
         _lib.check(self.stem_fn(_ptr(x), self.stem_args[0], x.shape[1], *self.stem_args[2:], st), "stem")
         _lib.check(self.xyz_fn(_ptr(x), self.xyz_args[0], x.shape[1], *self.xyz_args[2:], st), "xyz")
         probe = self._probe
diff --git a/rdpn6d_amd/ops.py b/rdpn6d_amd/ops.py
--- a/rdpn6d_amd/ops.py
+++ b/rdpn6d_amd/ops.py
@@ -131,7 +131,7 @@
 
 
 def conv2d_nhwc_h2(x, weight, scale=None, shift=None, stride=1, pad=0, residual=None, act=0, slope=0.0, want_h2=False, residual_h2=None,
-                   split_k=True, wfrag=False):
+                   split_k=True, wfrag=False, tapshift=None):
     from .gdrn import pack_h2_weight
 
     lib = _lib.load()
@@ -173,6 +173,14 @@
     if not lib.rdpn6d_conv_h2_kernel_for(ctypes.byref(d)):
         raise ValueError("layer not eligible for the h2 kernels (Cin % 32, N % 8, aligned slices)")
     ws_bytes = int(lib.rdpn6d_conv_h2_workspace_bytes(ctypes.byref(d))) if split_k else 0
+    if tapshift is not None:
+        lib.rdpn6d_conv_h2_set_tapshift(1 if tapshift else 0)
+        try:
+            if tapshift and (wfrag or ws_bytes or not lib.rdpn6d_conv_h2_tapshift_wanted(ctypes.byref(d))):
+                raise ValueError("this launch has no tap-shift form (3x3 / stride 1 / pad 1, W | 32, ping-pong or un-split 64x64 tile kernel)")
+            return conv2d_nhwc_h2(x, weight, scale, shift, stride, pad, residual, act, slope, want_h2, residual_h2, split_k, wfrag)
+        finally:
+            lib.rdpn6d_conv_h2_set_tapshift(1)
     if wfrag:
         if not lib.rdpn6d_conv_h2_wfrag_wanted(ctypes.byref(d)):
             raise ValueError("this layer's kernel has no weights-from-L2 form")
```
